# ksahlin/IsoCon

Hardware: AMD Instinct MI355X
Metric: read x candidate alignments/sec (NN-graph build, 50k x 2.5kb reads) (higher is better)
Workload: dtype u64; 1 GPU; C3: 50000 synthetic CCS reads (50000 unique), ~2500 bp, 10 isoforms, seed 30001; 1-set NN graph; edges=78526, graph_digest=65944c838d76a6c9, parallelism=single GPU

## Files before the change

isocon_amd/csrc/isocon_hip.hip:

```cpp
#include <algorithm>
#include <chrono>
#include <cstdio>
#include <cstdlib>
#include <cstring>
#include <numeric>
#include <string>
#include <memory>
#include <mutex>
#include <thread>
#include <vector>

#include "common.hpp"
#include "ed_band.hpp"
#include "ed_full.hpp"
#include "qgram_mm.hpp"
#include "nn.hpp"
#include "nn_list.hpp"
#include "nn_filter.hpp"
#include "nn_finalize.hpp"
#include "nn_finalize_host.hpp"
#include "partition_host.hpp"
#include "sg.hpp"
#include "msa.hpp"
#include "hw.hpp"
#include "hw_tiles.hpp"
#include "hw_full.hpp"
#include "nw_path.hpp"
#include "ed_lanes.hpp"
#include "ed_bytes.hpp"
#include "nn2_depth.hpp"
#include "readtab.hpp"
#include "edgevar.hpp"

namespace isocon {
thread_local std::string g_last_error;
}

using namespace isocon;

static bool variant_lookup(const char *name, std::string *value)
{
    const char *e = getenv("ISOCON_DEBUG_VARIANT");
    if (!e) return false;
    const size_t ln = strlen(name);
    for (const char *p = e; *p;) {
        const char *q = strchr(p, ',');
        const size_t len = q ? (size_t)(q - p) : strlen(p);
        if (len >= ln && strncmp(p, name, ln) == 0 && (len == ln || p[ln] == '=')) {
            if (value) *value = len > ln ? std::string(p + ln + 1, len - ln - 1) : std::string();
            return true;
        }
        p += len + (q ? 1 : 0);
    }
    return false;
}
static bool variant(const char *name) { return variant_lookup(name, nullptr); }
static const char *variant_value(const char *name)
{
    thread_local std::string ring[8];
    thread_local unsigned at = 0;
    std::string &slot = ring[at++ % 8];
    return variant_lookup(name, &slot) ? slot.c_str() : nullptr;
}

struct BoundTag {
    bool valid = false, has_order = false;
    uint64_t serial = 0;
    QMap map = {0, 0, 0, 0};
    uint32_t depth = 0;
    int32_t kcap = 0;
    unsigned long long lb_total = 0;
};
struct MsaBuilt {
    enum By { NONE, SINGLE, BATCH } by = NONE;
    uint64_t serial = 0;
    uint32_t n_parts = 0, n_rows = 0;
    std::vector<uint32_t> ncols, col_base, first_row;
    std::vector<unsigned long long> m_off;
};
struct HeldHits { uint64_t store_serial = 0; uint64_t rows = 0; };

struct ScratchPool {
    struct Slot { void *p = nullptr; size_t cap = 0; };
    Slot slots[160];
    BoundTag bound_tag;
    HeldHits held_hits;
    MsaBuilt msa;
    void *get(int idx, size_t bytes)
    {
        Slot &s = slots[idx];
        if (bytes == 0) bytes = 16;
        if (s.cap < bytes) {
            if (s.p) (void)hipFree(s.p);
            s.p = nullptr; s.cap = 0;
            const size_t want = bytes + bytes / 8;
            if (hipMalloc(&s.p, want) == hipSuccess) s.cap = want;
            else if (hipMalloc(&s.p, bytes) == hipSuccess) s.cap = bytes;
            else { s.p = nullptr; (void)hipGetLastError(); }
        }
        return s.p;
    }
    void release()
    {
        for (Slot &s : slots) { if (s.p) (void)hipFree(s.p); s.p = nullptr; s.cap = 0; }
        bound_tag = BoundTag();
        held_hits = HeldHits();
        msa = MsaBuilt();
    }
};

enum {
    SLOT_ED_TS = 0, SLOT_ED_IDS, SLOT_ED_K, SLOT_ED_OUT, SLOT_FULL_A, SLOT_FULL_B, SLOT_FULL_K, SLOT_FULL_OUT,
    SLOT_NN_BEST, SLOT_NN_QF, SLOT_NN_TF, SLOT_NN_HITS, SLOT_NN_HITCOUNT, SLOT_NN_STATS, SLOT_NN_TS, SLOT_NN_IDS, SLOT_NN_PLANES2, SLOT_NN_PERM, SLOT_NN_IL, SLOT_NN_IL2, SLOT_NN_HITS2, SLOT_NN_HITCOUNT2, SLOT_NN_QPROF, SLOT_NN_QSUM, SLOT_NN_LB, SLOT_NN_LBROW, SLOT_NN_LBLEN, SLOT_NN_SLOTORDER, SLOT_NN_LBCHUNKS, SLOT_NN_ROWMIN, SLOT_NN_COLMIN, SLOT_NN_SEED_A, SLOT_NN_SEED_B, SLOT_NN_SEED_N, SLOT_NN_LBT, SLOT_NN_LBT_OFF, SLOT_NN_LBT_SLO, SLOT_NN_LBT_LEN, SLOT_NN_LBT_PAD, SLOT_NN_SCORE, SLOT_NN_LDEST, SLOT_NN_FIN_HITS, SLOT_NN_FIN_CNT, SLOT_NN_FIN_START, SLOT_NN_FIN_CUR, SLOT_NN_FIN_NB, SLOT_NN_FIN_LEN2, SLOT_NN_FIN_OUT, SLOT_NN_FIN_FLAG, SLOT_NN_FIN_BEST, SLOT_NN_ACC_HITS, SLOT_NN_LTOT, SLOT_NN_LCHUNKS, SLOT_NN_LIST, SLOT_NN_LPA, SLOT_NN_LPB, SLOT_NN_TEXT2, SLOT_NN_LTASKS, SLOT_NN_RECORD,
    SLOT_NN2_STATE, SLOT_NN2_TPOS, SLOT_NN2_EXC, SLOT_NN2_CTR, SLOT_NN2_PAIRS, SLOT_NN2_WIDE,
    SLOT_SG_PAIRS, SLOT_SG_R, SLOT_SG_TRACE, SLOT_SG_END, SLOT_SG_OPS, SLOT_SG_CNT, SLOT_SG_RES, SLOT_SG_OFF, SLOT_SG_DENSE, SLOT_SG_BOUND, SLOT_SG_AOFF, SLOT_SG_ALNA, SLOT_SG_ALNB,
    SLOT_MSA_IN, SLOT_MSA_OUT, SLOT_MSA_DEG, SLOT_MSA_COUNTS, SLOT_MSA_MAJ, SLOT_MSA_FLAGS, SLOT_MSA_TOT, SLOT_MSA_NCAND, SLOT_MSA_LEN, SLOT_MSA_OFF, SLOT_MSA_PACKED, SLOT_MSA_ROWS, SLOT_MSA_OPS, SLOT_MSA_OPTR, SLOT_MSA_LONGEST, SLOT_MSA_WIDTH, SLOT_MSA_CSLOT, SLOT_MSA_LTOT, SLOT_MSA_WIDE, SLOT_MSA_PROW, SLOT_MSA_PCOL, SLOT_MSA_PPTR, SLOT_MSA_PBYTES, SLOT_MSA_PART, SLOT_MSA_FIRST, SLOT_MSA_LM, SLOT_MSA_SBASE, SLOT_MSA_NCOLS, SLOT_MSA_MOFF, SLOT_MSA_CBASE, SLOT_MSA_CBP, SLOT_MSA_CBC, SLOT_MSA_CBR,
    SLOT_HW_Q, SLOT_HW_T, SLOT_HW_K, SLOT_HW_OUT, SLOT_HW_TRACE, SLOT_HW_CTR, SLOT_HW_TILEQ, SLOT_HW_LANES, SLOT_HW_PQ, SLOT_HW_KEY, SLOT_HW_HIST, SLOT_HW_CURSOR, SLOT_HW_TBASE, SLOT_HW_CLS,
    SLOT_PACK_ASCII, SLOT_PACK_OFF, SLOT_PACK_BAD, SLOT_PACK_HIST, SLOT_PACK_FLAGS, SLOT_EB_A, SLOT_EB_B, SLOT_EB_K, SLOT_EB_OUT, SLOT_EB_ROWS, SLOT_SCAN_TMP, SLOT_SCAN_SUMS,
    SLOT_RT_REF, SLOT_RT_IN, SLOT_RT_OUT,
    SLOT_EV_IN, SLOT_EV_OUT, SLOT_EV_SNIP,
    SLOT_NWP_Q, SLOT_NWP_T, SLOT_NWP_ED, SLOT_NWP_TOFF, SLOT_NWP_ROFF, SLOT_NWP_REV, SLOT_NWP_RUNS, SLOT_NWP_FOFF, SLOT_NWP_OPS, SLOT_NWP_START, SLOT_NWP_COLS,
    SLOT_COUNT
};
static_assert(SLOT_COUNT <= 160, "ScratchPool::slots too small");

static ScratchPool g_scratch;

static uint64_t g_store_serial = 0;

struct isocon_store {
    uint64_t serial = ++g_store_serial;
    DevStore dev;
    explicit isocon_store(bool private_scratch = false) : own_pool(private_scratch ? new ScratchPool() : nullptr), pool(own_pool ? *own_pool : g_scratch) {}
    std::unique_ptr<ScratchPool> own_pool;
    ScratchPool &pool;
    std::vector<int32_t> lens;
    uint64_t device_bytes = 0;
    uint64_t *d_planes = nullptr;
    char alphabet[4] = {'A', 'C', 'G', 'T'};
    bool acgt = true;
    uint8_t *d_bytes = nullptr;
    uint64_t *d_boff = nullptr;
    uint64_t bytes_base = 0;
    std::vector<uint8_t> exc;
    std::vector<uint32_t> exc_count;
    uint32_t n_exc = 0;
    bool is_exc(uint32_t i) const { return n_exc != 0 && exc[i] != 0; }
    int32_t *d_lens = nullptr;
    int32_t maxlen = 0;
    uint64_t last_host_waits = 0;
};

namespace {

struct PinnedStage {
    void *p = nullptr;
    size_t cap = 0;
    void *get(size_t bytes)
    {
        if (cap < bytes) {
            if (p) (void)hipHostFree(p);
            p = nullptr; cap = 0;
            if (hipHostMalloc(&p, bytes, hipHostMallocDefault) == hipSuccess) cap = bytes;
            else { p = nullptr; (void)hipGetLastError(); }
        }
        return p;
    }
    void release() { if (p) (void)hipHostFree(p); p = nullptr; cap = 0; }
};
static PinnedStage g_stage;
static constexpr size_t kStageBytes = (size_t)32 << 20;
static constexpr uint64_t kPackWaves = (uint64_t)1 << 25;
static constexpr size_t kStageMin = (size_t)32 << 10;

static std::vector<std::pair<const char *, size_t>> g_pinned;
static bool is_pinned(const void *p, size_t bytes)
{
    for (const auto &r : g_pinned)
        if ((const char *)p >= r.first && (const char *)p + bytes <= r.first + r.second) return true;
    return false;
}

static thread_local uint64_t g_host_waits = 0;
static hipError_t memcpy_wait(void *dst, const void *src, size_t bytes, hipMemcpyKind kind) { ++g_host_waits; return hipMemcpy(dst, src, bytes, kind); }
static hipError_t memset_wait(void *dst, int value, size_t bytes) { ++g_host_waits; return hipMemset(dst, value, bytes); }
static hipError_t device_wait() { ++g_host_waits; return hipDeviceSynchronize(); }

static hipError_t copy_d2h(void *dst, const void *dsrc, size_t bytes)
{
    if (bytes < kStageMin || is_pinned(dst, bytes)) return memcpy_wait(dst, dsrc, bytes, hipMemcpyDeviceToHost);
    char *st = static_cast<char *>(g_stage.get(kStageBytes));
    if (!st) return memcpy_wait(dst, dsrc, bytes, hipMemcpyDeviceToHost);
    for (size_t off = 0; off < bytes; off += kStageBytes) {
        const size_t len = std::min(kStageBytes, bytes - off);
        const hipError_t e = memcpy_wait(st, static_cast<const char *>(dsrc) + off, len, hipMemcpyDeviceToHost);
        if (e != hipSuccess) return e;
        memcpy(static_cast<char *>(dst) + off, st, len);
    }
    return hipSuccess;
}

static hipError_t copy_h2d(void *ddst, const void *src, size_t bytes)
{
    if (bytes < kStageMin || is_pinned(src, bytes)) return memcpy_wait(ddst, src, bytes, hipMemcpyHostToDevice);
    char *st = static_cast<char *>(g_stage.get(kStageBytes));
    if (!st) return memcpy_wait(ddst, src, bytes, hipMemcpyHostToDevice);
    for (size_t off = 0; off < bytes; off += kStageBytes) {
        const size_t len = std::min(kStageBytes, bytes - off);
        memcpy(st, static_cast<const char *>(src) + off, len);
        const hipError_t e = memcpy_wait(static_cast<char *>(ddst) + off, st, len, hipMemcpyHostToDevice);
        if (e != hipSuccess) return e;
    }
    return hipSuccess;
}

struct SideUpload {
    hipStream_t stream = nullptr;
    hipEvent_t before = nullptr, done = nullptr;
    PinnedStage pinned;
    bool in_flight = false;
    bool ready()
    {
        if (stream) return true;
        if (hipStreamCreateWithFlags(&stream, hipStreamNonBlocking) != hipSuccess) { stream = nullptr; (void)hipGetLastError(); return false; }
        if (hipEventCreateWithFlags(&before, hipEventDisableTiming) != hipSuccess || hipEventCreateWithFlags(&done, hipEventDisableTiming) != hipSuccess) {
            (void)hipGetLastError();
            release();
            return false;
        }
        return true;
    }
    void settle()
    {
        if (!in_flight) return;
        if (hipEventQuery(done) != hipSuccess || hipStreamQuery(stream) != hipSuccess) { (void)hipGetLastError(); ++g_host_waits; (void)hipStreamSynchronize(stream); }
        in_flight = false;
    }
    void release()
    {
        if (stream) { (void)hipStreamSynchronize(stream); (void)hipStreamDestroy(stream); }
        if (before) (void)hipEventDestroy(before);
        if (done) (void)hipEventDestroy(done);
        stream = nullptr; before = done = nullptr; in_flight = false;
        pinned.release();
    }
};
static SideUpload g_side;

struct DevBuf {
    void *p = nullptr;
    ScratchPool *pool = nullptr;
    int slot = -1;
    DevBuf() {}
    DevBuf(ScratchPool *pl, int sl) : pool(pl), slot(sl) {}
    DevBuf(const DevBuf &) = delete;
    DevBuf &operator=(const DevBuf &) = delete;
    ~DevBuf() { if (p && !pool) (void)hipFree(p); }
    template <class T> T *as() { return static_cast<T *>(p); }
    int alloc(size_t bytes)
    {
        if (pool) {
            p = pool->get(slot, bytes);
            if (!p) { g_last_error = "hipMalloc(scratch slot " + std::to_string(slot) + ", " + std::to_string(bytes) + " B) failed"; return ISOCON_E_HIP; }
            return ISOCON_OK;
        }
        if (p) { (void)hipFree(p); p = nullptr; }
        ISO_HIP_CHECK(hipMalloc(&p, bytes ? bytes : 16));
        return ISOCON_OK;
    }
};

template <int SHIFT, class OUT>
static int device_exscan(ScratchPool *pl, const uint32_t *d_in, uint32_t n, OUT *d_out)
{
    DevBuf d_tmp(pl, SLOT_SCAN_TMP), d_sums(pl, SLOT_SCAN_SUMS);
    const uint32_t tiles = std::max<uint32_t>(1, (n + SCAN_TILE - 1) / SCAN_TILE);
    int rc;
    if ((rc = d_tmp.alloc((size_t)std::max<uint32_t>(n, 1) * 4)) || (rc = d_sums.alloc((size_t)tiles * 8))) return rc;
    hipLaunchKernelGGL((k_scan_tiles<SHIFT>), dim3(tiles), dim3(256), 0, 0, d_in, n, d_tmp.as<uint32_t>(), d_sums.as<unsigned long long>());
    hipLaunchKernelGGL((k_scan_finish<OUT>), dim3(tiles), dim3(256), 0, 0, d_tmp.as<uint32_t>(), n, d_sums.as<unsigned long long>(), tiles, d_out, (unsigned long long *)nullptr);
    ISO_HIP_CHECK(hipGetLastError());
    return ISOCON_OK;
}

struct EventPool {
    std::mutex mu;
    std::vector<hipEvent_t> idle;
    hipEvent_t get()
    {
        {
            std::lock_guard<std::mutex> g(mu);
            if (!idle.empty()) { hipEvent_t e = idle.back(); idle.pop_back(); return e; }
        }
        hipEvent_t e = nullptr;
        if (hipEventCreate(&e) != hipSuccess) { (void)hipGetLastError(); return nullptr; }
        return e;
    }
    void put(hipEvent_t e)
    {
        if (!e) return;
        std::lock_guard<std::mutex> g(mu);
        idle.push_back(e);
    }
    void release()
    {
        std::lock_guard<std::mutex> g(mu);
        for (hipEvent_t e : idle) (void)hipEventDestroy(e);
        idle.clear();
    }
};
static EventPool g_events;

struct EventTimer {
    struct Interval { hipEvent_t e0, em, e1; float *acc, *marked_acc; };
    std::vector<Interval> pending;
    hipEvent_t e0 = nullptr, em = nullptr;
    float total = 0.f;
    float marked_total = 0.f;
    const bool sync_phases = variant("nn_sync_phases");
    EventTimer() {}
    EventTimer(const EventTimer &) = delete;
    EventTimer &operator=(const EventTimer &) = delete;
    ~EventTimer()
    {
        g_events.put(e0); g_events.put(em);
        for (const Interval &iv : pending) { g_events.put(iv.e0); g_events.put(iv.em); g_events.put(iv.e1); }
    }
    void start()
    {
        g_events.put(em); em = nullptr;
        if (!e0) e0 = g_events.get();
        if (e0) (void)hipEventRecord(e0, 0);
    }
    void mark()
    {
        if (!e0) return;
        if (!em) em = g_events.get();
        if (em) (void)hipEventRecord(em, 0);
    }
    void stop_later(float *acc, float *marked_acc = nullptr)
    {
        if (!e0) return;
        hipEvent_t e1 = g_events.get();
        if (!e1) { g_events.put(e0); g_events.put(em); e0 = em = nullptr; return; }
        (void)hipEventRecord(e1, 0);
        pending.push_back(Interval{e0, em, e1, acc, marked_acc});
        e0 = em = nullptr;
        if (sync_phases) resolve(true);
    }
    void resolve(bool wait_counts = false)
    {
        if (pending.empty()) return;
        hipEvent_t last = pending.back().e1;
        if (wait_counts || hipEventQuery(last) != hipSuccess) { (void)hipGetLastError(); ++g_host_waits; (void)hipEventSynchronize(last); }
        for (const Interval &iv : pending) {
            float ms = 0.f, part = 0.f;
            if (hipEventElapsedTime(&ms, iv.e0, iv.e1) != hipSuccess) { (void)hipGetLastError(); ms = 0.f; }
            total += ms;
            if (iv.acc) *iv.acc += ms;
            if (iv.em) {
                if (hipEventElapsedTime(&part, iv.em, iv.e1) != hipSuccess) { (void)hipGetLastError(); part = 0.f; }
                if (iv.marked_acc) *iv.marked_acc += part; else marked_total += part;
            }
            g_events.put(iv.e0); g_events.put(iv.em); g_events.put(iv.e1);
        }
        pending.clear();
    }
    float stop()
    {
        float ms = 0.f;
        stop_later(&ms);
        resolve(true);
        return ms;
    }
};

struct PackMap { uint8_t sym[4]; };

__global__ __launch_bounds__(256) void k_byte_histogram(const uint8_t *__restrict__ ascii, uint64_t total, unsigned long long *__restrict__ hist)
{
    __shared__ uint32_t h[256];
    h[threadIdx.x] = 0;
    __syncthreads();
    for (uint64_t i = (uint64_t)blockIdx.x * 256 + threadIdx.x; i < total; i += (uint64_t)gridDim.x * 256) atomicAdd(&h[ascii[i]], 1u);
    __syncthreads();
    if (h[threadIdx.x]) atomicAdd(hist + threadIdx.x, (unsigned long long)h[threadIdx.x]);
}

__global__ __launch_bounds__(256) void k_pack_planes(const uint8_t *__restrict__ ascii, const uint64_t *__restrict__ offsets, uint64_t base, uint32_t n,
                                                      uint32_t nchunks, uint64_t *__restrict__ planes, unsigned long long *__restrict__ first_bad, PackMap map,
                                                      uint32_t fold, uint64_t w0)
{
    const uint64_t w = w0 + (uint64_t)blockIdx.x * 4 + (threadIdx.x >> 6);
    if (w >= (uint64_t)nchunks * n) return;
    const uint32_t lane = threadIdx.x & 63;
    const uint32_t chunk = (uint32_t)(w / n), seq = (uint32_t)(w % n);
    const uint64_t off = offsets[seq] - base, len = offsets[seq + 1] - offsets[seq];
    const uint64_t pos = (uint64_t)chunk * 64 + lane;
    int cd = 0;
    bool bad = false;
    if (pos < len) {
        uint8_t ch = ascii[off + pos];
        if (fold && ch >= 'a' && ch <= 'z') ch = (uint8_t)(ch - 32);
        cd = ch == map.sym[0] ? 0 : ch == map.sym[1] ? 1 : ch == map.sym[2] ? 2 : ch == map.sym[3] ? 3 : -1;
        bad = cd < 0 && !fold;
    }
    const unsigned long long lo = __ballot(!bad && (cd & 1)), hi = __ballot(!bad && (cd & 2)), bm = __ballot(bad);
    if (lane == 0) {
        planes[((size_t)chunk * n + seq) * 2] = lo;
        planes[((size_t)chunk * n + seq) * 2 + 1] = hi;
        if (bm) atomicMin(first_bad, ((unsigned long long)seq << 32) | ((unsigned long long)chunk * 64 + (unsigned long long)(__ffsll((long long)bm) - 1)));
    }
}

}

extern "C" {

const char *isocon_strerror(int status)
{
    switch (status) {
    case ISOCON_OK: return "ok";
    case ISOCON_E_ARG: return "bad argument";
    case ISOCON_E_ALPHABET: return "sequence contains a symbol outside ACGT";
    case ISOCON_E_HIP: return "HIP runtime error";
    case ISOCON_E_CAPACITY: return "output buffer too small";
    case ISOCON_E_NODEVICE: return "no usable GPU";
    case ISOCON_E_UNSUPPORTED: return "unsupported request";
    default: return "unknown status";
    }
}

const char *isocon_last_error(void) { return g_last_error.c_str(); }

int isocon_device_count(void)
{
    int n = 0;
    if (hipGetDeviceCount(&n) != hipSuccess) return 0;
    return n;
}

void isocon_release_scratch(void) { g_scratch.release(); g_stage.release(); g_events.release(); g_side.release(); }

int isocon_init(int device_ordinal)
{
    int n = 0;
    if (hipGetDeviceCount(&n) != hipSuccess || n <= 0) { g_last_error = "hipGetDeviceCount: no device"; return ISOCON_E_NODEVICE; }
    if (device_ordinal < 0 || device_ordinal >= n) return ISOCON_E_ARG;
    ISO_HIP_CHECK(hipSetDevice(device_ordinal));
    return ISOCON_OK;
}

static int store_create_impl(const uint8_t *ascii, const uint8_t *const *seq_ptrs, const uint64_t *offsets, uint32_t n, isocon_store **out, bool private_scratch = false)
{
    *out = nullptr;
    int32_t maxlen = 0;
    for (uint32_t i = 0; i < n; ++i) {
        if (offsets[i + 1] < offsets[i] || offsets[i + 1] - offsets[i] > 0x3fffffff) return ISOCON_E_ARG;
        maxlen = std::max<int32_t>(maxlen, (int32_t)(offsets[i + 1] - offsets[i]));
    }
    const uint32_t nchunks = (uint32_t)((maxlen + 63) / 64 + 1);
    const uint32_t nn = std::max<uint32_t>(n, 1);
    std::vector<int32_t> lens(nn, 0);
    for (uint32_t i = 0; i < n; ++i) lens[i] = (int32_t)(offsets[i + 1] - offsets[i]);
    const uint64_t base = n ? offsets[0] : 0, total = n ? offsets[n] - offsets[0] : 0;
    isocon_store *st = new isocon_store(private_scratch);
    st->lens = lens;
    st->maxlen = maxlen;
    const size_t pbytes = (size_t)nchunks * nn * 2 * sizeof(uint64_t), lbytes = lens.size() * sizeof(int32_t);
    if (hipMalloc((void **)&st->d_planes, pbytes) != hipSuccess || hipMalloc((void **)&st->d_lens, lbytes) != hipSuccess) {
        g_last_error = "hipMalloc(store) failed";
        isocon_store_destroy(st);
        return ISOCON_E_HIP;
    }
    {
        DevBuf d_ascii(&g_scratch, SLOT_PACK_ASCII), d_off(&g_scratch, SLOT_PACK_OFF), d_bad(&g_scratch, SLOT_PACK_BAD);
        uint64_t pack_waves = kPackWaves;
        if (const char *e = variant_value("pack_waves")) pack_waves = std::max<uint64_t>(4, strtoull(e, nullptr, 10)) & ~(uint64_t)3;
        const unsigned long long none = ~0ull;
        int rc = ISOCON_OK;
        if ((rc = d_ascii.alloc(total ? total : 16)) || (rc = d_off.alloc((size_t)(nn + 1) * 8)) || (rc = d_bad.alloc(8))) { isocon_store_destroy(st); return rc; }
        bool up = true;
        if (total && ascii) up = copy_h2d(d_ascii.p, ascii + base, total) == hipSuccess;
        else if (total) {
            char *stg = static_cast<char *>(g_stage.get(kStageBytes));
            hipEvent_t ev[2] = {nullptr, nullptr};
            up = stg != nullptr && hipEventCreateWithFlags(&ev[0], hipEventDisableTiming) == hipSuccess && hipEventCreateWithFlags(&ev[1], hipEventDisableTiming) == hipSuccess;
            const size_t half = kStageBytes / 2;
            uint64_t done = 0;
            bool busy[2] = {false, false};
            auto gather = [&](char *dst, uint64_t b0, uint64_t b1) {
                uint32_t i = (uint32_t)(std::upper_bound(offsets, offsets + n + 1, base + b0) - offsets) - 1;
                uint64_t in_seq = base + b0 - offsets[i];
                while (b0 < b1 && i < n) {
                    const uint64_t len = offsets[i + 1] - offsets[i];
                    const size_t take = (size_t)std::min<uint64_t>(len - in_seq, b1 - b0);
                    if (take) memcpy(dst, seq_ptrs[i] + in_seq, take);
                    dst += take; b0 += take; in_seq += take;
                    if (in_seq == len) { ++i; in_seq = 0; }
                }
            };
            const unsigned hc = std::thread::hardware_concurrency();
            const unsigned n_thr = total >= ((uint64_t)8 << 20) ? std::min(4u, hc ? hc : 1u) : 1u;
            for (int h = 0; up && done < total; h ^= 1) {
                if (busy[h]) up = hipEventSynchronize(ev[h]) == hipSuccess;
                const size_t fill = (size_t)std::min<uint64_t>(half, total - done);
                if (n_thr <= 1) gather(stg + h * half, done, done + fill);
                else {
                    std::thread th[4];
                    const size_t part = (fill + n_thr - 1) / n_thr;
                    for (unsigned t = 0; t < n_thr; ++t) {
                        const size_t a = std::min(fill, t * part), b = std::min(fill, (t + 1) * part);
                        th[t] = std::thread([&, a, b, h] { if (b > a) gather(stg + h * half + a, done + a, done + b); });
                    }
                    for (unsigned t = 0; t < n_thr; ++t) th[t].join();
                }
                up = up && hipMemcpyAsync(static_cast<char *>(d_ascii.p) + done, stg + h * half, fill, hipMemcpyHostToDevice, 0) == hipSuccess &&
                     hipEventRecord(ev[h], 0) == hipSuccess;
                busy[h] = true;
                done += fill;
            }
            up = up && hipStreamSynchronize(0) == hipSuccess;
            if (ev[0]) (void)hipEventDestroy(ev[0]);
            if (ev[1]) (void)hipEventDestroy(ev[1]);
        }
        bool ok = up &&
                  (n == 0 || copy_h2d(d_off.p, offsets, (size_t)(n + 1) * 8) == hipSuccess) &&
                  hipMemcpy(d_bad.p, &none, 8, hipMemcpyHostToDevice) == hipSuccess && copy_h2d(st->d_lens, lens.data(), lbytes) == hipSuccess;
        unsigned long long bad = none;
        if (ok) {
            if (n) {
                const uint64_t waves = (uint64_t)nchunks * n;
                for (uint64_t w0 = 0; w0 < waves; w0 += pack_waves)
                    hipLaunchKernelGGL(k_pack_planes, dim3((unsigned)((std::min<uint64_t>(pack_waves, waves - w0) + 3) / 4)), dim3(256), 0, 0, d_ascii.as<uint8_t>(), d_off.as<uint64_t>(), base, n, nchunks,
                                       st->d_planes, d_bad.as<unsigned long long>(), PackMap{{'A', 'C', 'G', 'T'}}, 0u, w0);
            } else {
                ok = hipMemset(st->d_planes, 0, pbytes) == hipSuccess;
            }
            ok = ok && hipGetLastError() == hipSuccess && hipMemcpy(&bad, d_bad.p, 8, hipMemcpyDeviceToHost) == hipSuccess;
        }
        if (!ok) {
            g_last_error = "isocon_store_create: device copy / packing failed";
            (void)hipGetLastError();
            isocon_store_destroy(st);
            return ISOCON_E_HIP;
        }
        if (bad != none) {
            DevBuf d_hist(&g_scratch, SLOT_PACK_HIST);
            unsigned long long hist[256];
            bool hok = d_hist.alloc(256 * 8) == ISOCON_OK && hipMemset(d_hist.p, 0, 256 * 8) == hipSuccess;
            if (hok) {
                hipLaunchKernelGGL(k_byte_histogram, dim3(1024), dim3(256), 0, 0, d_ascii.as<uint8_t>(), (uint64_t)total, d_hist.as<unsigned long long>());
                hok = hipGetLastError() == hipSuccess && hipMemcpy(hist, d_hist.p, sizeof(hist), hipMemcpyDeviceToHost) == hipSuccess;
            }
            int distinct = 0;
            for (int c = 0; hok && c < 256; ++c) distinct += hist[c] != 0;
            if (!hok) {
                g_last_error = "isocon_store_create: symbol histogram failed";
                (void)hipGetLastError();
                isocon_store_destroy(st);
                return ISOCON_E_HIP;
            }
            if (distinct > 4) {
                DevBuf d_flags(&g_scratch, SLOT_PACK_FLAGS);
                st->exc.assign(nn, 0);
                st->exc_count.assign(nn, 0);
                bool eok = d_flags.alloc((size_t)nn * 4) == ISOCON_OK && hipMemset(d_flags.p, 0, (size_t)nn * 4) == hipSuccess &&
                           hipMalloc((void **)&st->d_bytes, total ? total : 16) == hipSuccess && hipMalloc((void **)&st->d_boff, (size_t)(nn + 1) * 8) == hipSuccess;
                if (eok) {
                    const uint64_t waves = (uint64_t)nchunks * n;
                    for (uint64_t w0 = 0; w0 < waves; w0 += pack_waves)
                    hipLaunchKernelGGL(k_pack_planes, dim3((unsigned)((std::min<uint64_t>(pack_waves, waves - w0) + 3) / 4)), dim3(256), 0, 0, d_ascii.as<uint8_t>(), d_off.as<uint64_t>(), base, n, nchunks,
                                       st->d_planes, d_bad.as<unsigned long long>(), PackMap{{'A', 'C', 'G', 'T'}}, 1u, w0);
                    for (uint64_t w0 = 0; w0 < waves; w0 += pack_waves)
                        hipLaunchKernelGGL(k_exception_flags, dim3((unsigned)((std::min<uint64_t>(pack_waves, waves - w0) + 3) / 4)), dim3(256), 0, 0, d_ascii.as<uint8_t>(), d_off.as<uint64_t>(), base, n,
                                           nchunks, d_flags.as<uint32_t>(), (uint32_t)'A' | ((uint32_t)'C' << 8) | ((uint32_t)'G' << 16) | ((uint32_t)'T' << 24), w0);
                    eok = hipGetLastError() == hipSuccess && hipMemcpy(st->exc_count.data(), d_flags.p, (size_t)n * 4, hipMemcpyDeviceToHost) == hipSuccess &&
                          hipMemcpy(st->d_bytes, d_ascii.p, total, hipMemcpyDeviceToDevice) == hipSuccess &&
                          hipMemcpy(st->d_boff, d_off.p, (size_t)(n + 1) * 8, hipMemcpyDeviceToDevice) == hipSuccess;
                }
                if (!eok) {
                    g_last_error = "isocon_store_create: keeping the bytes of a set with more than four symbols failed";
                    (void)hipGetLastError();
                    isocon_store_destroy(st);
                    return ISOCON_E_HIP;
                }
                st->bytes_base = base;
                for (uint32_t i = 0; i < n; ++i) { st->exc[i] = st->exc_count[i] != 0; st->n_exc += st->exc[i]; }
                st->acgt = false;
                st->device_bytes += total + (size_t)(nn + 1) * 8;
            } else {
            PackMap map{{0, 0, 0, 0}};
            bool used[4] = {false, false, false, false};
            const char acgt_sym[4] = {'A', 'C', 'G', 'T'};
            for (int k = 0; k < 4; ++k) if (hist[(uint8_t)acgt_sym[k]]) { map.sym[k] = (uint8_t)acgt_sym[k]; used[k] = true; }
            for (int c = 0; c < 256; ++c) {
                if (!hist[c] || c == 'A' || c == 'C' || c == 'G' || c == 'T') continue;
                for (int k = 0; k < 4; ++k) if (!used[k]) { map.sym[k] = (uint8_t)c; used[k] = true; break; }
            }
            for (int k = 0; k < 4; ++k) if (!used[k]) { for (int c = 1; c < 256; ++c) if (!hist[c] && c != map.sym[0] && c != map.sym[1] && c != map.sym[2] && c != map.sym[3]) { map.sym[k] = (uint8_t)c; break; } }
            bool rok = hipMemcpy(d_bad.p, &none, 8, hipMemcpyHostToDevice) == hipSuccess;
            if (rok) {
                const uint64_t waves = (uint64_t)nchunks * n;
                for (uint64_t w0 = 0; w0 < waves; w0 += pack_waves)
                    hipLaunchKernelGGL(k_pack_planes, dim3((unsigned)((std::min<uint64_t>(pack_waves, waves - w0) + 3) / 4)), dim3(256), 0, 0, d_ascii.as<uint8_t>(), d_off.as<uint64_t>(), base, n, nchunks,
                                       st->d_planes, d_bad.as<unsigned long long>(), map, 0u, w0);
                rok = hipGetLastError() == hipSuccess && hipMemcpy(&bad, d_bad.p, 8, hipMemcpyDeviceToHost) == hipSuccess && bad == none;
            }
            if (!rok) {
                g_last_error = "isocon_store_create: packing under the set's own alphabet failed";
                (void)hipGetLastError();
                isocon_store_destroy(st);
                return ISOCON_E_HIP;
            }
            for (int k = 0; k < 4; ++k) st->alphabet[k] = (char)map.sym[k];
            st->acgt = false;
            }
        }
    }
    st->device_bytes += pbytes + lbytes;
    st->dev.planes = st->d_planes;
    st->dev.il = nullptr;
    st->dev.lens = st->d_lens;
    st->dev.n = n;
    st->dev.nchunks = nchunks;
    st->lens.resize(n);
    *out = st;
    return ISOCON_OK;
}

int isocon_store_create(const uint8_t *ascii, const uint64_t *offsets, uint32_t n, isocon_store **out)
{
    if (!out || (!ascii && n) || !offsets) return ISOCON_E_ARG;
    return store_create_impl(ascii, nullptr, offsets, n, out);
}

int isocon_store_create_ptrs(const uint8_t *const *seq_ptrs, const uint64_t *seq_lens, uint32_t n, isocon_store **out)
{
    if (!out || (n && (!seq_ptrs || !seq_lens))) return ISOCON_E_ARG;
    std::vector<uint64_t> offsets((size_t)n + 1, 0);
    for (uint32_t i = 0; i < n; ++i) {
        if (seq_lens[i] && !seq_ptrs[i]) return ISOCON_E_ARG;
        offsets[i + 1] = offsets[i] + seq_lens[i];
    }
    return store_create_impl(nullptr, seq_ptrs, offsets.data(), n, out);
}

int isocon_store_create_ptrs_ex(const uint8_t *const *seq_ptrs, const uint64_t *seq_lens, uint32_t n, uint32_t flags, isocon_store **out)
{
    if (!out || (n && (!seq_ptrs || !seq_lens)) || (flags & ~(uint32_t)ISOCON_STORE_PRIVATE_SCRATCH)) return ISOCON_E_ARG;
    std::vector<uint64_t> offsets((size_t)n + 1, 0);
    for (uint32_t i = 0; i < n; ++i) {
        if (seq_lens[i] && !seq_ptrs[i]) return ISOCON_E_ARG;
        offsets[i + 1] = offsets[i] + seq_lens[i];
    }
    return store_create_impl(nullptr, seq_ptrs, offsets.data(), n, out, (flags & ISOCON_STORE_PRIVATE_SCRATCH) != 0);
}

void *isocon_host_alloc(uint64_t bytes)
{
    void *p = nullptr;
    if (hipHostMalloc(&p, bytes ? bytes : 16, hipHostMallocDefault) != hipSuccess) { (void)hipGetLastError(); return nullptr; }
    g_pinned.emplace_back((const char *)p, (size_t)(bytes ? bytes : 16));
    return p;
}

void isocon_host_free(void *p)
{
    if (!p) return;
    for (size_t i = 0; i < g_pinned.size(); ++i)
        if (g_pinned[i].first == (const char *)p) { g_pinned.erase(g_pinned.begin() + (long)i); break; }
    (void)hipHostFree(p);
}

void isocon_store_destroy(isocon_store *s)
{
    if (!s) return;
    if (s->d_planes) (void)hipFree(s->d_planes);
    if (s->d_lens) (void)hipFree(s->d_lens);
    if (s->d_bytes) (void)hipFree(s->d_bytes);
    if (s->d_boff) (void)hipFree(s->d_boff);
    if (s->own_pool) s->own_pool->release();
    delete s;
}

uint32_t isocon_store_size(const isocon_store *s) { return s ? s->dev.n : 0; }
uint64_t isocon_nn_last_host_waits(const isocon_store *s) { return s ? s->last_host_waits : 0; }
uint64_t isocon_store_device_bytes(const isocon_store *s) { return s ? s->device_bytes : 0; }

}

namespace {

template <int W>
int launch_band_tiles(isocon_store *st, const DevStore &S, const std::vector<uint32_t> &tile_shared, const std::vector<uint32_t> &lane_ids,
                      const std::vector<int32_t> &lane_k, std::vector<int32_t> &out, EventTimer &tm)
{
    const size_t nt = tile_shared.size();
    out.assign(nt * 64, -1);
    if (!nt) return ISOCON_OK;
    DevBuf d_ts(&st->pool, SLOT_ED_TS), d_ids(&st->pool, SLOT_ED_IDS), d_k(&st->pool, SLOT_ED_K), d_out(&st->pool, SLOT_ED_OUT);
    int rc;
    if ((rc = d_ts.alloc(nt * 4)) || (rc = d_ids.alloc(nt * 64 * 4)) || (rc = d_k.alloc(nt * 64 * 4)) || (rc = d_out.alloc(nt * 64 * 4))) return rc;
    ISO_HIP_CHECK(copy_h2d(d_ts.p, tile_shared.data(), nt * 4));
    ISO_HIP_CHECK(copy_h2d(d_ids.p, lane_ids.data(), nt * 64 * 4));
    ISO_HIP_CHECK(copy_h2d(d_k.p, lane_k.data(), nt * 64 * 4));
    tm.start();
    hipLaunchKernelGGL(k_ed_band_tiles<W>, dim3((unsigned)((nt + 3) / 4)), dim3(256), 0, 0, S, d_ts.as<uint32_t>(),
                       d_ids.as<uint32_t>(), d_k.as<int32_t>(), d_out.as<int32_t>(), (uint32_t)nt);
    ISO_HIP_CHECK(hipGetLastError());
    tm.stop();
    ISO_HIP_CHECK(copy_d2h(out.data(), d_out.p, nt * 64 * 4));
    return ISOCON_OK;
}

int run_band_stage(int W, isocon_store *st, const DevStore &S, const std::vector<uint32_t> &ts, const std::vector<uint32_t> &ids,
                   const std::vector<int32_t> &ks, std::vector<int32_t> &out, EventTimer &tm)
{
    switch (W) {
    case 1: return launch_band_tiles<1>(st, S, ts, ids, ks, out, tm);
    case 2: return launch_band_tiles<2>(st, S, ts, ids, ks, out, tm);
    case 4: return launch_band_tiles<4>(st, S, ts, ids, ks, out, tm);
    case 8: return launch_band_tiles<8>(st, S, ts, ids, ks, out, tm);
    default: return ISOCON_E_ARG;
    }
}

int run_full(isocon_store *st, const std::vector<uint32_t> &a, const std::vector<uint32_t> &b,
             const std::vector<int32_t> &k, std::vector<int32_t> &out, EventTimer &tm)
{
    const size_t np = a.size();
    out.assign(np, -1);
    if (!np) return ISOCON_OK;
    DevBuf d_a(&st->pool, SLOT_FULL_A), d_b(&st->pool, SLOT_FULL_B), d_k(&st->pool, SLOT_FULL_K), d_out(&st->pool, SLOT_FULL_OUT);
    int rc;
    if ((rc = d_a.alloc(np * 4)) || (rc = d_b.alloc(np * 4)) || (rc = d_k.alloc(np * 4)) || (rc = d_out.alloc(np * 4))) return rc;
    ISO_HIP_CHECK(copy_h2d(d_a.p, a.data(), np * 4));
    ISO_HIP_CHECK(copy_h2d(d_b.p, b.data(), np * 4));
    ISO_HIP_CHECK(copy_h2d(d_k.p, k.data(), np * 4));
    bool multipass = false;
    int32_t maxtext = 0;
    for (size_t p = 0; p < np; ++p) {
        const int32_t la = st->lens[a[p]], lb = st->lens[b[p]];
        if (std::min(la, lb) > 4096) multipass = true;
        maxtext = std::max(maxtext, std::max(la, lb));
    }
    const size_t lds = multipass ? (size_t)((maxtext + 15) & ~15) : 0;
    if (lds > 160 * 1024) { g_last_error = "sequence longer than 163840 bases in the un-banded kernel"; return ISOCON_E_UNSUPPORTED; }
    if (lds > 64 * 1024)
        ISO_HIP_CHECK(hipFuncSetAttribute((const void *)k_ed_full, hipFuncAttributeMaxDynamicSharedMemorySize, (int)lds));
    tm.start();
    hipLaunchKernelGGL(k_ed_full, dim3((unsigned)np), dim3(64), lds, 0, st->dev, d_a.as<uint32_t>(), d_b.as<uint32_t>(),
                       d_k.as<int32_t>(), d_out.as<int32_t>(), (uint32_t)np);
    ISO_HIP_CHECK(hipGetLastError());
    tm.stop();
    ISO_HIP_CHECK(copy_d2h(out.data(), d_out.p, np * 4));
    return ISOCON_OK;
}

int run_bytes(isocon_store *st, const std::vector<uint32_t> &a, const std::vector<uint32_t> &b, const std::vector<int32_t> &k, std::vector<int32_t> &out, EventTimer &tm)
{
    const size_t np = a.size();
    out.assign(np, -1);
    if (!np) return ISOCON_OK;
    if (!st->d_bytes) { g_last_error = "internal: byte-wise distances on a store that kept no bytes"; return ISOCON_E_HIP; }
    if (st->maxlen >= (int32_t)EB_INF - 1) { g_last_error = "byte-wise distances: sequences of 8 388 606 bases and more are not supported"; return ISOCON_E_UNSUPPORTED; }
    const uint32_t row_stride = (uint32_t)st->maxlen + 130u;
    size_t waves = std::min<size_t>(np, 8192);
    while (waves > 256 && waves * row_stride * 4 > ((size_t)2 << 30)) waves /= 2;
    DevBuf d_a(&st->pool, SLOT_EB_A), d_b(&st->pool, SLOT_EB_B), d_k(&st->pool, SLOT_EB_K), d_out(&st->pool, SLOT_EB_OUT), d_rows(&st->pool, SLOT_EB_ROWS);
    int rc;
    if ((rc = d_a.alloc(np * 4)) || (rc = d_b.alloc(np * 4)) || (rc = d_k.alloc(np * 4)) || (rc = d_out.alloc(np * 4)) || (rc = d_rows.alloc(waves * row_stride * 4))) return rc;
    ISO_HIP_CHECK(copy_h2d(d_a.p, a.data(), np * 4));
    ISO_HIP_CHECK(copy_h2d(d_b.p, b.data(), np * 4));
    ISO_HIP_CHECK(copy_h2d(d_k.p, k.data(), np * 4));
    tm.start();
    hipLaunchKernelGGL(k_ed_bytes, dim3((unsigned)waves), dim3(64), 0, 0, ByteStore{st->d_bytes, st->d_boff, st->bytes_base, st->d_lens}, d_a.as<uint32_t>(), d_b.as<uint32_t>(),
                       d_k.as<int32_t>(), (unsigned long long)np, d_rows.as<uint32_t>(), row_stride, d_out.as<int32_t>());
    ISO_HIP_CHECK(hipGetLastError());
    tm.stop();
    ISO_HIP_CHECK(copy_d2h(out.data(), d_out.p, np * 4));
    return ISOCON_OK;
}

}

namespace isocon {

int ed_pairs_impl(isocon_store *st, const uint32_t *a, const uint32_t *b, const int32_t *k, uint64_t n_pairs,
                  int32_t *out_ed, float *kernel_ms, uint64_t *full_pairs, bool images)
{
    EventTimer tm;
    const uint32_t n = st->dev.n;
    for (uint64_t p = 0; p < n_pairs; ++p)
        if (a[p] >= n || b[p] >= n) return ISOCON_E_ARG;
    bool swap_roles = false;
    {
        std::vector<uint8_t> seen_a(n, 0), seen_b(n, 0);
        size_t da = 0, db = 0;
        for (uint64_t p = 0; p < n_pairs; ++p) {
            if (!seen_a[a[p]]) { seen_a[a[p]] = 1; ++da; }
            if (!seen_b[b[p]]) { seen_b[b[p]] = 1; ++db; }
        }
        swap_roles = db < da;
    }
    std::vector<uint64_t> pending;
    pending.reserve(n_pairs);
    if (st->n_exc && !images) {
        std::vector<uint64_t> xp;
        for (uint64_t p = 0; p < n_pairs; ++p) (st->exc[a[p]] || st->exc[b[p]] ? xp : pending).push_back(p);
        if (!xp.empty()) {
            std::vector<uint32_t> xa(xp.size()), xb(xp.size());
            std::vector<int32_t> xk(xp.size()), res;
            for (size_t i = 0; i < xp.size(); ++i) { xa[i] = a[xp[i]]; xb[i] = b[xp[i]]; xk[i] = k ? k[xp[i]] : -1; }
            int rc = run_bytes(st, xa, xb, xk, res, tm);
            if (rc) return rc;
            for (size_t i = 0; i < xp.size(); ++i) out_ed[xp[i]] = res[i];
        }
    } else {
        pending.resize(n_pairs);
        std::iota(pending.begin(), pending.end(), 0);
    }
    static const int stages[4] = {1, 2, 4, 8};
    for (int si = 0; si < 4 && !pending.empty(); ++si) {
        const int W = stages[si];
        const int32_t kcap = 64 * W - 1;
        auto sh = [&](uint64_t p) { return swap_roles ? b[p] : a[p]; };
        auto ln = [&](uint64_t p) { return swap_roles ? a[p] : b[p]; };
        std::sort(pending.begin(), pending.end(), [&](uint64_t x, uint64_t y) {
            if (sh(x) != sh(y)) return sh(x) < sh(y);
            const int32_t lx = st->lens[ln(x)], ly = st->lens[ln(y)];
            if (lx != ly) return lx < ly;
            return x < y;
        });
        std::vector<uint64_t> todo = pending, next;
        if (W == 1) {
            const char *e = variant_value("ed_lanes");
            const size_t min_group = e ? (atoi(e) ? (size_t)-1 : 0) : 16;
            std::vector<uint64_t> lanes_p, tiles_p;
            for (size_t i = 0; i < todo.size();) {
                size_t j = i;
                while (j < todo.size() && sh(todo[j]) == sh(todo[i])) ++j;
                std::vector<uint64_t> &dst = (j - i) < min_group ? lanes_p : tiles_p;
                dst.insert(dst.end(), todo.begin() + i, todo.begin() + j);
                i = j;
            }
            if (!lanes_p.empty()) {
                const size_t np = lanes_p.size();
                std::vector<uint32_t> la(np), lb2(np);
                std::vector<int32_t> lk(np), res(np, -1);
                for (size_t i = 0; i < np; ++i) {
                    const uint64_t p = lanes_p[i];
                    la[i] = a[p]; lb2[i] = b[p];
                    const int32_t kr = k ? k[p] : -1;
                    lk[i] = kr < 0 ? kcap : std::min(kr, kcap);
                }
                DevBuf d_a(&st->pool, SLOT_ED_TS), d_b(&st->pool, SLOT_ED_IDS), d_k(&st->pool, SLOT_ED_K), d_out(&st->pool, SLOT_ED_OUT);
                int rc;
                if ((rc = d_a.alloc(np * 4)) || (rc = d_b.alloc(np * 4)) || (rc = d_k.alloc(np * 4)) || (rc = d_out.alloc(np * 4))) return rc;
                ISO_HIP_CHECK(copy_h2d(d_a.p, la.data(), np * 4));
                ISO_HIP_CHECK(copy_h2d(d_b.p, lb2.data(), np * 4));
                ISO_HIP_CHECK(copy_h2d(d_k.p, lk.data(), np * 4));
                NNParams none;
                memset(&none, 0, sizeof(none));
                tm.start();
                hipLaunchKernelGGL(k_ed_lanes<false>, dim3((unsigned)((np + 255) / 256)), dim3(256), 0, 0, st->dev, none, d_a.as<uint32_t>(), d_b.as<uint32_t>(),
                                   d_k.as<int32_t>(), (uint64_t)np, d_out.as<int32_t>());
                ISO_HIP_CHECK(hipGetLastError());
                tm.stop();
                ISO_HIP_CHECK(copy_d2h(res.data(), d_out.p, np * 4));
                for (size_t i = 0; i < np; ++i) {
                    const uint64_t p = lanes_p[i];
                    const int32_t kr = k ? k[p] : -1;
                    if (res[i] >= 0) out_ed[p] = res[i];
                    else if (kr >= 0 && kr <= kcap) out_ed[p] = -1;
                    else next.push_back(p);
                }
            }
            todo.swap(tiles_p);
        }
        for (int round = 0; round < 2 && !todo.empty(); ++round) {
            std::vector<uint32_t> ts, ids;
            std::vector<int32_t> ks;
            std::vector<uint64_t> slot_pair;
            size_t i = 0;
            while (i < todo.size()) {
                size_t j = i;
                const uint32_t s0 = sh(todo[i]);
                const size_t lim = round == 0 ? 64 : 1;
                while (j < todo.size() && j - i < lim && sh(todo[j]) == s0) ++j;
                ts.push_back(s0);
                for (size_t l = 0; l < 64; ++l) {
                    if (i + l < j) {
                        const uint64_t p = todo[i + l];
                        ids.push_back(ln(p));
                        const int32_t kr = k ? k[p] : -1;
                        ks.push_back(kr < 0 ? kcap : std::min(kr, kcap));
                        slot_pair.push_back(p);
                    } else {
                        ids.push_back(0xffffffffu);
                        ks.push_back(-1);
                        slot_pair.push_back(~(uint64_t)0);
                    }
                }
                i = j;
            }
            std::vector<int32_t> res;
            int rc = run_band_stage(W, st, st->dev, ts, ids, ks, res, tm);
            if (rc) return rc;
            std::vector<uint64_t> retry;
            for (size_t sidx = 0; sidx < slot_pair.size(); ++sidx) {
                const uint64_t p = slot_pair[sidx];
                if (p == ~(uint64_t)0) continue;
                const int32_t r = res[sidx];
                const int32_t kr = k ? k[p] : -1;
                if (r >= 0) out_ed[p] = r;
                else if (r == -2) retry.push_back(p);
                else if (kr >= 0 && kr <= kcap) out_ed[p] = -1;
                else next.push_back(p);
            }
            todo.swap(retry);
        }
        if (!todo.empty()) { g_last_error = "internal: single-lane tile undetermined"; return ISOCON_E_HIP; }
        pending.swap(next);
    }
    if (full_pairs) *full_pairs = pending.size();
    if (!pending.empty()) {
        std::vector<uint32_t> fa, fb;
        std::vector<int32_t> fk, res;
        for (uint64_t p : pending) { fa.push_back(a[p]); fb.push_back(b[p]); fk.push_back(k ? k[p] : -1); }
        int rc = run_full(st, fa, fb, fk, res, tm);
        if (rc) return rc;
        for (size_t i = 0; i < pending.size(); ++i) out_ed[pending[i]] = res[i];
    }
    if (kernel_ms) *kernel_ms = tm.total;
    return ISOCON_OK;
}

}

__global__ __launch_bounds__(256) void k_store_digest(const uint64_t *__restrict__ planes, size_t n_words, const int32_t *__restrict__ lens, uint32_t n,
                                                      unsigned long long *__restrict__ out)
{
    unsigned long long acc = 0;
    const size_t stride = (size_t)gridDim.x * blockDim.x;
    for (size_t i = (size_t)blockIdx.x * blockDim.x + threadIdx.x; i < n_words + n; i += stride) {
        unsigned long long v = i < n_words ? planes[i] : (unsigned long long)(uint32_t)lens[i - n_words];
        v ^= (unsigned long long)i * 0xD6E8FEB86659FD93ull;
        v ^= v >> 32; v *= 0x9E3779B97F4A7C15ull; v ^= v >> 29; v *= 0xBF58476D1CE4E5B9ull; v ^= v >> 32;
        acc += v;
    }
    for (int o = 32; o > 0; o >>= 1) acc += __shfl_xor(acc, o, 64);
    if ((threadIdx.x & 63) == 0 && acc) atomicAdd(out, acc);
}

extern "C" int isocon_store_digest(const isocon_store *s, uint64_t *out)
{
    if (!s || !out) return ISOCON_E_ARG;
    DevBuf d_acc;
    int rc;
    if ((rc = d_acc.alloc(8))) return rc;
    ISO_HIP_CHECK(hipMemset(d_acc.p, 0, 8));
    const size_t n_words = (size_t)s->dev.nchunks * std::max<uint32_t>(s->dev.n, 1) * 2;
    hipLaunchKernelGGL(k_store_digest, dim3(1024), dim3(256), 0, 0, s->d_planes, n_words, s->d_lens, s->dev.n, d_acc.as<unsigned long long>());
    ISO_HIP_CHECK(hipGetLastError());
    ISO_HIP_CHECK(hipMemcpy(out, d_acc.p, 8, hipMemcpyDeviceToHost));
    return ISOCON_OK;
}

extern "C" int isocon_ed_pairs(isocon_store *s, const uint32_t *a, const uint32_t *b, const int32_t *k, uint64_t n_pairs,
                               int32_t *out_ed, float *kernel_ms)
{
    if (!s || (n_pairs && (!a || !b || !out_ed))) return ISOCON_E_ARG;
    if (kernel_ms) *kernel_ms = 0.f;
    if (!n_pairs) return ISOCON_OK;
    return ed_pairs_impl(s, a, b, k, n_pairs, out_ed, kernel_ms, nullptr, false);
}

extern "C" int isocon_qgram_params(int32_t *out)
{
    if (out) { out[0] = QG_Q; out[1] = QG_B0; out[2] = QG_B1; out[3] = QG_CAP; }
    return QM_K;
}

namespace isocon {
int qgram_bounds_for_pairs(isocon_store *s, const uint32_t *a, const uint32_t *b, uint64_t n_pairs, int32_t *out_bound, float *kernel_ms)
{
    const uint32_t n = s->dev.n;
    const uint32_t n_pad = std::max<uint32_t>(QM_TILE, ((n + QM_TILE - 1) / QM_TILE) * QM_TILE);
    DevBuf d_prof(&s->pool, SLOT_NN_QPROF), d_sum(&s->pool, SLOT_NN_QSUM), d_a(&s->pool, SLOT_ED_TS), d_b(&s->pool, SLOT_ED_IDS), d_out(&s->pool, SLOT_ED_OUT);
    int rc;
    if ((rc = d_prof.alloc((size_t)n_pad * (QM_K / 2))) || (rc = d_sum.alloc((size_t)n * 4)) || (rc = d_a.alloc(n_pairs * 4)) || (rc = d_b.alloc(n_pairs * 4)) ||
        (rc = d_out.alloc(n_pairs * 4)))
        return rc;
    s->pool.bound_tag.valid = false;
    ISO_HIP_CHECK(copy_h2d(d_a.p, a, n_pairs * 4));
    ISO_HIP_CHECK(copy_h2d(d_b.p, b, n_pairs * 4));
    EventTimer tm;
    tm.start();
    hipLaunchKernelGGL(k_qgram_profile4, dim3((n + QP_SEQS - 1) / QP_SEQS), dim3(256), 0, 0, s->dev, d_prof.as<uint8_t>(), d_sum.as<uint32_t>(), n_pad);
    ISO_HIP_CHECK(hipGetLastError());
    for (uint64_t at = 0; at < n_pairs; at += (uint64_t)1 << 24) {
        const uint64_t cnt = std::min<uint64_t>((uint64_t)1 << 24, n_pairs - at);
        hipLaunchKernelGGL(k_qgram_lb_pairs, dim3((unsigned)((cnt + 3) / 4)), dim3(256), 0, 0, d_prof.as<uint8_t>(), d_sum.as<uint32_t>(), n_pad, d_a.as<uint32_t>() + at,
                           d_b.as<uint32_t>() + at, cnt, d_out.as<int32_t>() + at);
        ISO_HIP_CHECK(hipGetLastError());
    }
    const float ms = tm.stop();
    if (kernel_ms) *kernel_ms = ms;
    ISO_HIP_CHECK(copy_d2h(out_bound, d_out.p, n_pairs * 4));
    return ISOCON_OK;
}
}

extern "C" int isocon_qgram_bound_pairs(isocon_store *s, const uint32_t *a, const uint32_t *b, uint64_t n_pairs, int32_t *out_bound)
{
    if (!s || (n_pairs && (!a || !b || !out_bound))) return ISOCON_E_ARG;
    if (!n_pairs) return ISOCON_OK;
    if (s->n_exc) { g_last_error = "q-gram bounds are defined on the 2-bit planes: the set holds more than four distinct symbols"; return ISOCON_E_ALPHABET; }
    const uint32_t n = s->dev.n;
    for (uint64_t i = 0; i < n_pairs; ++i)
        if (a[i] >= n || b[i] >= n) { g_last_error = "pair index out of range"; return ISOCON_E_ARG; }
    return qgram_bounds_for_pairs(s, a, b, n_pairs, out_bound, nullptr);
}

extern "C" int isocon_block_bound_pairs(isocon_store *s, const uint32_t *owner, const uint32_t *partner, uint64_t n_pairs, int32_t probe_stride, int32_t *out_count)
{
    if (probe_stride != 4 && probe_stride != 2) return ISOCON_E_ARG;
    if (!s || (n_pairs && (!owner || !partner || !out_count))) return ISOCON_E_ARG;
    if (!n_pairs) return ISOCON_OK;
    if (s->n_exc) { g_last_error = "block bounds are defined on the 2-bit planes: the set holds more than four distinct symbols"; return ISOCON_E_ALPHABET; }
    const uint32_t n = s->dev.n;
    if (n_pairs >= ((uint64_t)1 << 31)) return ISOCON_E_ARG;
    for (uint64_t i = 0; i < n_pairs; ++i)
        if (owner[i] >= n || partner[i] >= n) { g_last_error = "pair index out of range"; return ISOCON_E_ARG; }
    const uint32_t stride = nnf_text2_stride(s->maxlen);
    DevBuf d_text(&s->pool, SLOT_NN_TEXT2), d_a(&s->pool, SLOT_ED_TS), d_b(&s->pool, SLOT_ED_IDS), d_out(&s->pool, SLOT_ED_OUT);
    int rc;
    if ((rc = d_text.alloc((size_t)n * stride * 4)) || (rc = d_a.alloc(n_pairs * 4)) || (rc = d_b.alloc(n_pairs * 4)) || (rc = d_out.alloc(n_pairs * 4))) return rc;
    ISO_HIP_CHECK(copy_h2d(d_a.p, owner, n_pairs * 4));
    ISO_HIP_CHECK(copy_h2d(d_b.p, partner, n_pairs * 4));
    hipLaunchKernelGGL(k_build_text2, dim3(n), dim3(256), 0, 0, s->dev, d_text.as<uint32_t>(), stride);
    hipLaunchKernelGGL(k_nn_block_count_pairs, dim3((unsigned)n_pairs), dim3(256), 0, 0, d_text.as<uint32_t>(), stride, s->dev.lens, d_a.as<uint32_t>(), d_b.as<uint32_t>(), d_out.as<int32_t>(), probe_stride);
    ISO_HIP_CHECK(hipGetLastError());
    ISO_HIP_CHECK(copy_d2h(out_count, d_out.p, n_pairs * 4));
    return ISOCON_OK;
}

#include "nn_context.inc"
#include "nn_bounds.inc"
#include "nn_lists.inc"
#include "nn_main.inc"
#include "nn_wide.inc"
#include "nn_images.inc"
#include "nn_entry.inc"
#include "nn2_depth.inc"
#include "sg_host.inc"
#include "msa_host.inc"
#include "hw_host.inc"
#include "hw_full_host.inc"
#include "nw_path_host.inc"
#include "hw_path_host.inc"
#include "readtab_host.inc"
#include "edgevar_host.inc"

extern "C" int isocon_partition_ids(uint32_t n, const int32_t *degree, uint64_t n_edges, const uint32_t *edge_a, const uint32_t *edge_b,
                                    const uint32_t *rank, int32_t nbr_tiebreak, uint32_t *out_centre, int64_t *out_weight,
                                    uint64_t *out_member_ptr, uint32_t *out_members, uint32_t *n_parts)
{
    if (!out_member_ptr || !n_parts || (n && (!degree || !rank || !out_centre || !out_weight || !out_members)) || (n_edges && (!edge_a || !edge_b))) return ISOCON_E_ARG;
    return partition_ids_impl(n, degree, n_edges, edge_a, edge_b, rank, nbr_tiebreak, out_centre, out_weight, out_member_ptr, out_members, n_parts);
}
```

isocon_amd/csrc/nn_bounds.inc:

```

namespace {

int NNContext::build_bounds(const QMap &Q, int32_t kcap, NNParams &P, bool want_seeds)
{
    const uint32_t q_begin = Q.begin, q_end = Q.end;
    P.lb = nullptr;
    P.lb_row = nullptr;
    P.slot_order = nullptr;
    if (variant("nn_no_qgram") || n < 2 || n >= (1u << 30) || q_begin >= q_end) return ISOCON_OK;
    if (!want_seeds && st->pool.bound_tag.valid && st->pool.bound_tag.serial == st->serial && st->pool.bound_tag.map.same(Q) &&
        st->pool.bound_tag.depth == depth && st->pool.bound_tag.kcap == kcap) {
        P.lb = static_cast<const uint8_t *>(st->pool.slots[SLOT_NN_LB].p);
        P.lb_row = static_cast<const unsigned long long *>(st->pool.slots[SLOT_NN_LBROW].p);
        if (st->pool.bound_tag.has_order && use_slot_order(Q.count())) P.slot_order = static_cast<const uint32_t *>(st->pool.slots[SLOT_NN_SLOTORDER].p);
        lb_total = st->pool.bound_tag.lb_total;
        return ISOCON_OK;
    }
    st->pool.bound_tag.valid = false;
    const uint32_t nq = Q.count();
    const std::vector<int32_t> &lens = st->lens;
    const uint32_t n_pad = std::max<uint32_t>(QM_TILE, ((n + QM_TILE - 1) / QM_TILE) * QM_TILE);
    const size_t prof_bytes = (size_t)n_pad * (QM_K / 2);
    d_qprof.pool = d_qsum.pool = &st->pool;
    d_qprof.slot = SLOT_NN_QPROF; d_qsum.slot = SLOT_NN_QSUM;
    HostClock bclk;
    {
        size_t free_b = 0;
        if (!free_mem(free_b) || prof_bytes > free_b / 2 + st->pool.slots[SLOT_NN_QPROF].cap) return ISOCON_OK;
        if (d_qprof.alloc(prof_bytes) || d_qsum.alloc((size_t)n * 4)) return ISOCON_OK;
    }
    bclk.lap("bounds: memory check + profile buffers");
    const bool side = !variant("nn_sync_uploads") && g_side.ready() && hipEventRecord(g_side.before, 0) == hipSuccess;
    tm.start();
    hipLaunchKernelGGL(k_qgram_profile4, dim3((n + QP_SEQS - 1) / QP_SEQS), dim3(256), 0, 0, st->dev, d_qprof.as<uint8_t>(), d_qsum.as<uint32_t>(), n_pad);
    ISO_HIP_CHECK(hipGetLastError());
    struct StopTimer { NNContext &c; bool armed = true; ~StopTimer() { if (armed) c.tm.stop_later(&c.stats.bound_kernel_ms); } } stop_timer{*this};
    std::vector<unsigned long long> &off = lb_off_host;
    std::vector<uint32_t> &rlen = lb_len_host;
    off.assign(nq, 0);
    rlen.assign(nq, 0);
    unsigned long long total = 0, sum_rlen = 0;
    uint64_t hi = 0;
    const uint32_t nrb = (nq + QM_TILE - 1) / QM_TILE;
    std::vector<uint64_t> rb_lo(nrb, ~(uint64_t)0), rb_hi(nrb, 0);
    for (uint32_t s = 0; s < nq; ++s) {
        const uint64_t q = Q.entry(s);
        if (hi < q + 1) hi = q + 1;
        while (hi < n && lens[hi] - lens[q] <= kcap) ++hi;
        uint64_t len = hi - q - 1;
        if (len > depth) len = depth;
        const uint64_t pal = (q + 1) & ~(uint64_t)15;
        off[s] = total + (q + 1 - pal);
        rlen[s] = (uint32_t)len;
        sum_rlen += len;
        if (len) {
            total += ((q + 1 + len + 15) & ~(uint64_t)15) - pal;
            rb_lo[s / QM_TILE] = std::min<uint64_t>(rb_lo[s / QM_TILE], q + 1);
            rb_hi[s / QM_TILE] = std::max<uint64_t>(rb_hi[s / QM_TILE], q + len);
        }
    }
    if (total == 0) return ISOCON_OK;
    bclk.lap("bounds: profile launch + rows (host)");
    const unsigned long long totalT = sum_rlen + 30ull * n;
    bclk.lap("bounds: transposed rows (host)");
    size_t free_b = 0;
    const size_t need = (size_t)total + (size_t)totalT + prof_bytes + (size_t)n * 24 + (size_t)nq * 12;
    if (!free_mem(free_b) || need > free_b / 2 + st->pool.slots[SLOT_NN_LB].cap + st->pool.slots[SLOT_NN_QPROF].cap) return ISOCON_OK;
    bclk.lap("bounds: memory check 2");
    std::vector<uint2> tiles;
    for (uint32_t g = 0; g * 4 < nrb; ++g) {
        uint64_t jmin = ~(uint64_t)0, jmax = 0;
        bool any = false;
        for (uint32_t I = g * 4; I < std::min(nrb, g * 4 + 4); ++I)
            if (rb_lo[I] != ~(uint64_t)0) { any = true; jmin = std::min(jmin, rb_lo[I] / QM_TILE); jmax = std::max(jmax, rb_hi[I] / QM_TILE); }
        if (!any) continue;
        for (uint64_t j0 = jmin; j0 <= jmax; j0 += 8)
            for (uint32_t ri = 0; ri < 4; ++ri)
                for (uint32_t cj = 0; cj < 8; ++cj) {
                    const uint32_t I = g * 4 + ri;
                    const uint64_t J = j0 + cj;
                    const bool have = I < nrb && rb_lo[I] != ~(uint64_t)0 && J >= rb_lo[I] / QM_TILE && J <= rb_hi[I] / QM_TILE;
                    tiles.push_back(have ? make_uint2(I, (uint32_t)J) : make_uint2(0xffffffffu, 0xffffffffu));
                }
    }
    while (tiles.size() % 256) tiles.push_back(make_uint2(0xffffffffu, 0xffffffffu));
    if (tiles.size() > 0x7fffffffull) return ISOCON_OK;
    bclk.lap("bounds: tile table (host)");
    d_lb.pool = d_lbrow.pool = d_lblen.pool = &st->pool;
    d_lb.slot = SLOT_NN_LB; d_lbrow.slot = SLOT_NN_LBROW; d_lblen.slot = SLOT_NN_LBLEN;
    int rc;
    if ((rc = d_lb.alloc((size_t)total + 16)) ||
        (rc = d_lbrow.alloc((size_t)nq * 8)) || (rc = d_lblen.alloc((size_t)nq * 4)))
        return ISOCON_OK;
    d_lbt.pool = d_offT.pool = d_sloT.pool = d_lenT.pool = d_score.pool = &st->pool;
    d_lbt.slot = SLOT_NN_LBT; d_offT.slot = SLOT_NN_LBT_OFF; d_sloT.slot = SLOT_NN_LBT_SLO; d_lenT.slot = SLOT_NN_LBT_LEN; d_score.slot = SLOT_NN_SCORE;
    DevBuf d_padT(&st->pool, SLOT_NN_LBT_PAD);
    if (d_lbt.alloc((size_t)totalT + 16) || d_offT.alloc(((size_t)n + 1) * 8) || d_sloT.alloc((size_t)n * 4) || d_lenT.alloc((size_t)n * 4) || d_score.alloc((size_t)n * 4) ||
        d_padT.alloc((size_t)n * 4))
        return ISOCON_OK;
    ISO_HIP_CHECK(hipMemsetAsync(d_score.p, 0, (size_t)n * 4, 0));
    d_chunks.pool = &st->pool;
    d_chunks.slot = SLOT_NN_LBCHUNKS;
    if (d_chunks.alloc(tiles.size() * sizeof(uint2))) return ISOCON_OK;
    const size_t b_tiles = (tiles.size() * sizeof(uint2) + 15) & ~(size_t)15, b_off = ((size_t)nq * 8 + 15) & ~(size_t)15, b_len = (size_t)nq * 4;
    char *pin = nullptr;
    if (side) { g_side.settle(); pin = static_cast<char *>(g_side.pinned.get(b_tiles + b_off + b_len)); }
    if (pin) {
        memcpy(pin, tiles.data(), tiles.size() * sizeof(uint2));
        memcpy(pin + b_tiles, off.data(), (size_t)nq * 8);
        memcpy(pin + b_tiles + b_off, rlen.data(), (size_t)nq * 4);
        g_side.in_flight = true;
        ISO_HIP_CHECK(hipStreamWaitEvent(g_side.stream, g_side.before, 0));
        ISO_HIP_CHECK(hipMemcpyAsync(d_chunks.p, pin, tiles.size() * sizeof(uint2), hipMemcpyHostToDevice, g_side.stream));
        ISO_HIP_CHECK(hipMemcpyAsync(d_lbrow.p, pin + b_tiles, (size_t)nq * 8, hipMemcpyHostToDevice, g_side.stream));
        ISO_HIP_CHECK(hipMemcpyAsync(d_lblen.p, pin + b_tiles + b_off, (size_t)nq * 4, hipMemcpyHostToDevice, g_side.stream));
        ISO_HIP_CHECK(hipEventRecord(g_side.done, g_side.stream));
        ISO_HIP_CHECK(hipStreamWaitEvent(0, g_side.done, 0));
    } else {
        ISO_HIP_CHECK(copy_h2d(d_chunks.p, tiles.data(), tiles.size() * sizeof(uint2)));
        ISO_HIP_CHECK(copy_h2d(d_lbrow.p, off.data(), (size_t)nq * 8));
        ISO_HIP_CHECK(copy_h2d(d_lblen.p, rlen.data(), (size_t)nq * 4));
    }
    hipLaunchKernelGGL(k_lbt_rows, dim3((n + 255) / 256), dim3(256), 0, 0, Q, nq, d_lblen.as<uint32_t>(), n, d_sloT.as<uint32_t>(), d_lenT.as<uint32_t>(), d_padT.as<uint32_t>());
    if ((rc = device_exscan<0, unsigned long long>(&st->pool, d_padT.as<uint32_t>(), n, d_offT.as<unsigned long long>()))) return ISOCON_OK;
    hipLaunchKernelGGL(k_lbt_offsets, dim3((n + 255) / 256), dim3(256), 0, 0, n, d_sloT.as<uint32_t>(), d_offT.as<unsigned long long>());
    ISO_HIP_CHECK(hipGetLastError());
    bclk.lap("bounds: alloc + uploads");
    if (use_slot_order(nq)) {
        std::vector<uint32_t> order(nq);
        std::iota(order.begin(), order.end(), 0u);
        std::stable_sort(order.begin(), order.end(), [&](uint32_t x, uint32_t y) { return rlen[x] > rlen[y]; });
        d_order.pool = &st->pool;
        d_order.slot = SLOT_NN_SLOTORDER;
        if (d_order.alloc((size_t)nq * 4)) return ISOCON_OK;
        ISO_HIP_CHECK(copy_h2d(d_order.p, order.data(), (size_t)nq * 4));
    }
    unsigned long long *rowmin = nullptr, *colmin = nullptr;
    if (want_seeds) {
        d_rowmin.pool = d_colmin.pool = d_seed_a.pool = d_seed_b.pool = &st->pool;
        d_rowmin.slot = SLOT_NN_ROWMIN; d_colmin.slot = SLOT_NN_COLMIN; d_seed_a.slot = SLOT_NN_SEED_A; d_seed_b.slot = SLOT_NN_SEED_B;
        if (!(d_rowmin.alloc((size_t)nq * 8 * QM_SEEDS) || d_colmin.alloc((size_t)n_pad * 8 * QM_SEEDS) || d_seed_a.alloc((size_t)n * 8 * QM_SEEDS) || d_seed_b.alloc((size_t)n * 8 * QM_SEEDS))) {
            ISO_HIP_CHECK(hipMemsetAsync(d_rowmin.p, 0xff, (size_t)nq * 8 * QM_SEEDS, 0));
            ISO_HIP_CHECK(hipMemsetAsync(d_colmin.p, 0xff, (size_t)n_pad * 8 * QM_SEEDS, 0));
            rowmin = d_rowmin.as<unsigned long long>();
            colmin = d_colmin.as<unsigned long long>();
        }
    }
    bclk.lap("bounds: slot order + seed buffers");
    static bool lds_attr_set = false;
    if (!lds_attr_set) {
        ISO_HIP_CHECK(hipFuncSetAttribute((const void *)k_qgram_mm, hipFuncAttributeMaxDynamicSharedMemorySize, (int)QM_LDS_BYTES));
        lds_attr_set = true;
    }
    tm.mark();
    hipLaunchKernelGGL(k_qgram_mm, dim3((unsigned)tiles.size()), dim3(512), QM_LDS_BYTES, 0, d_qprof.as<uint8_t>(), d_qsum.as<uint32_t>(), n, n_pad,
                       d_chunks.as<uint2>(), d_lbrow.as<unsigned long long>(), d_lblen.as<uint32_t>(), d_lb.as<uint8_t>(), Q, nq,
                       d_qf.as<uint8_t>(), d_tf.as<uint8_t>(), rowmin, colmin, d_offT.as<unsigned long long>(), d_sloT.as<uint32_t>(), d_lenT.as<uint32_t>(),
                       d_lbt.as<uint8_t>(), d_score.as<uint32_t>());
    ISO_HIP_CHECK(hipGetLastError());
    stop_timer.armed = false;
    tm.stop_later(&stats.bound_kernel_ms, &stats.mm_kernel_ms);
    bclk.lap("bounds: k_qgram_mm (enqueued)");
#ifdef ISOCON_QM_TIMELINE
    {
        const size_t nt = std::min<size_t>(tiles.size(), 16384);
        std::vector<unsigned long long> tl(nt * 8);
        ISO_HIP_CHECK(hipMemcpyFromSymbol(tl.data(), HIP_SYMBOL(g_qm_timeline), nt * 64));
        double sum[5] = {0, 0, 0, 0, 0};
        unsigned long long t_min = ~0ull, t_max = 0;
        size_t cnt = 0;
        for (size_t b = 0; b < nt; ++b) {
            if (tiles[b].x == 0xffffffffu) continue;
            const unsigned long long *t = tl.data() + b * 8;
            for (int k = 0; k < 5; ++k) sum[k] += (double)(t[k + 1] - t[k]);
            t_min = std::min(t_min, t[0]); t_max = std::max(t_max, t[5]);
            ++cnt;
        }
        fprintf(stderr, "[qm timeline] %zu tiles: prologue %.2f us, K loop %.2f us, E1 %.2f us, E2 %.2f us, E3 %.2f us per tile; first start to last end %.3f ms\n", cnt,
                sum[0] / cnt / 100.0, sum[1] / cnt / 100.0, sum[2] / cnt / 100.0, sum[3] / cnt / 100.0, sum[4] / cnt / 100.0, (double)(t_max - t_min) / 1e5);
    }
#endif
    for (const uint2 &t : tiles) stats.bound_tiles += t.x != 0xffffffffu;
    P.lb = d_lb.as<uint8_t>();
    P.lb_row = d_lbrow.as<unsigned long long>();
    if (use_slot_order(nq)) P.slot_order = d_order.as<uint32_t>();
    seeds_ready = rowmin != nullptr;
    seed_nq = nq;
    lb_total = total;
    st->pool.bound_tag.valid = true;
    st->pool.bound_tag.lb_total = total;
    st->pool.bound_tag.has_order = use_slot_order(nq);
    st->pool.bound_tag.serial = st->serial;
    st->pool.bound_tag.map = Q; st->pool.bound_tag.depth = depth; st->pool.bound_tag.kcap = kcap;
    return ISOCON_OK;
}

int NNContext::run_bound_seeds(const QMap &Q)
{
    if (!seeds_ready) return ISOCON_OK;
    tm.start();
    const uint64_t np = (uint64_t)2 * QM_SEEDS * n;
    const uint32_t ranks = std::max<uint32_t>(1u, Q.stride >> Q.block_log2);
    uint32_t col_classes = QM_SEEDS;
    while (col_classes > 1 && col_classes * ranks > (uint32_t)QM_SEEDS) col_classes >>= 1;
    if (const char *e = variant_value("nn_seed_classes")) { const int v = atoi(e); if (v == 1 || v == 2 || v == QM_SEEDS) col_classes = (uint32_t)v; }
    DevBuf d_seed_n(&st->pool, SLOT_NN_SEED_N);
    int rc;
    if ((rc = d_seed_n.alloc(8))) return rc;
    ISO_HIP_CHECK(hipMemsetAsync(d_seed_n.p, 0, 8, 0));
    ISO_HIP_CHECK(hipMemsetAsync(d_seed_a.p, 0xff, (size_t)np * 4, 0));
    ISO_HIP_CHECK(hipMemsetAsync(d_seed_b.p, 0xff, (size_t)np * 4, 0));
    hipLaunchKernelGGL(k_qgram_seed_pairs, dim3((n + 255) / 256), dim3(256), 0, 0, d_rowmin.as<unsigned long long>(), d_colmin.as<unsigned long long>(),
                       n, Q, seed_nq, col_classes, d_seed_a.as<uint32_t>(), d_seed_b.as<uint32_t>(), d_seed_n.as<unsigned long long>());
    ISO_HIP_CHECK(hipGetLastError());
    hipLaunchKernelGGL(k_ed_lanes<true>, dim3((unsigned)((np + 255) / 256)), dim3(256), 0, 0, st->dev, params(63), d_seed_a.as<uint32_t>(), d_seed_b.as<uint32_t>(),
                       (const int32_t *)nullptr, np, (int32_t *)nullptr);
    ISO_HIP_CHECK(hipGetLastError());
    tm.stop_later(&stats.seed_kernel_ms);
    return ISOCON_OK;
}

}
```

isocon_amd/csrc/nn_context.inc:

```

namespace {

struct HostClock {
    std::chrono::steady_clock::time_point t0 = std::chrono::steady_clock::now();
    const bool on = getenv("ISOCON_DEBUG") != nullptr;
    void lap(const char *what)
    {
        if (!on) return;
        const auto t1 = std::chrono::steady_clock::now();
        fprintf(stderr, "[isocon] %-28s %8.2f ms\n", what, std::chrono::duration<double, std::milli>(t1 - t0).count());
        t0 = t1;
    }
};

struct NNContext {
    isocon_store *st = nullptr;
    uint32_t n = 0;
    std::vector<uint8_t> qflag, tflag;
    bool two_set = false;
    bool depth_binds = false;
    std::vector<uint8_t> wide_mask;
    int32_t min_d = 1;
    uint32_t depth = 0x7fffffffu;
    DevBuf d_best, d_qf, d_tf, d_hits, d_hit_count, d_stats;
    DevBuf d_text;
    uint32_t text_stride = 0;
    bool text_ready = false;
    DevBuf d_qprof, d_qsum, d_lb, d_lbrow, d_lblen;
    DevBuf d_chunks;
    DevBuf d_lbt, d_offT, d_sloT, d_lenT, d_score;
    DevBuf d_order;
    DevBuf d_rowmin, d_colmin, d_seed_a, d_seed_b;
    uint64_t hits_cap = 0;
    std::vector<int32_t> best;
    std::vector<int32_t> hits;
    isocon_nn_stats stats;
    EventTimer tm;

    size_t free_bytes = 0;
    int free_state = 0;
    bool free_mem(size_t &free_b)
    {
        if (free_state == 0) {
            size_t total_b = 0;
            free_state = hipMemGetInfo(&free_bytes, &total_b) == hipSuccess ? 1 : -1;
            if (free_state < 0) (void)hipGetLastError();
        }
        free_b = free_bytes;
        return free_state > 0;
    }
    bool text_room = false;
    bool text_affordable()
    {
        if (text_ready || text_room) return true;
        text_stride = (uint32_t)NN_TEXT_PAD_FRONT + (uint32_t)((st->maxlen + 7) / 8) + (uint32_t)NN_TEXT_PAD_BACK;
        size_t free_b = 0;
        if (!free_mem(free_b) || (size_t)n * text_stride * 4 > free_b / 2) return false;
        d_text.pool = &st->pool;
        d_text.slot = SLOT_NN_IL;
        if (d_text.alloc((size_t)std::max<uint32_t>(n, 1) * text_stride * 4) != ISOCON_OK) return false;
        text_room = true;
        return true;
    }
    bool build_text()
    {
        if (text_ready) return true;
        if (!text_room) return false;
        hipLaunchKernelGGL(k_build_nibble_text, dim3(std::max<uint32_t>(n, 1)), dim3(256), 0, 0, st->dev, d_text.as<uint32_t>(), text_stride);
        if (hipGetLastError() != hipSuccess) { g_last_error = "k_build_nibble_text: launch failed"; return false; }
        text_ready = true;
        return true;
    }
    bool ensure_text() { return text_affordable() && build_text(); }
    DevBuf d_text2;
    uint32_t text2_stride = 0;
    bool text2_ready = false;
    bool ensure_text2()
    {
        if (text2_ready) return true;
        text2_stride = nnf_text2_stride(st->maxlen);
        size_t free_b = 0;
        if (!free_mem(free_b) || (size_t)n * text2_stride * 4 > free_b / 2 + st->pool.slots[SLOT_NN_TEXT2].cap) return false;
        d_text2.pool = &st->pool;
        d_text2.slot = SLOT_NN_TEXT2;
        if (d_text2.alloc((size_t)std::max<uint32_t>(n, 1) * text2_stride * 4) != ISOCON_OK) return false;
        hipLaunchKernelGGL(k_build_text2, dim3(std::max<uint32_t>(n, 1)), dim3(256), 0, 0, st->dev, d_text2.as<uint32_t>(), text2_stride);
        if (hipGetLastError() != hipSuccess) return false;
        text2_ready = true;
        return true;
    }
    static bool use_slot_order(uint32_t nq)
    {
        if (const char *e = variant_value("nn_order")) return atoi(e) != 0;
        return nq <= 16384;
    }
    int build_bounds(const QMap &Q, int32_t kcap, NNParams &P, bool want_seeds = false);
    std::vector<unsigned long long> lb_off_host;
    std::vector<uint32_t> lb_len_host;
    unsigned long long lb_total = 0;
    bool seeds_ready = false;
    uint32_t seed_nq = 0;
    int run_bound_seeds(const QMap &Q);
    DevBuf d_ltot, d_lchunks, d_list, d_lpa, d_lpb, d_lmeta, d_ltasks;
    struct ListPlan {
        bool listed = false;
        unsigned long long n_chunks = 0, n_chunks_narrow = 0, n_small = 0;
        unsigned long long conv_a = 0, conv_b = 0, conv_pairs = 0;
        NNChunk *a = nullptr, *b = nullptr, *sorted_a = nullptr, *sorted_b = nullptr;
    };
    int plan_lists(const QMap &Q, uint32_t nq, const NNParams &PR, ListPlan &L);
    NNParams params(int32_t kcap)
    {
        NNParams P;
        P.best = d_best.as<int32_t>();
        P.qflag = d_qf.as<uint8_t>();
        P.tflag = d_tf.as<uint8_t>();
        P.hits = d_hits.as<int32_t>();
        P.hit_count = d_hit_count.as<unsigned long long>();
        P.stats = d_stats.as<unsigned long long>();
        P.hits_cap = hits_cap;
        P.kcap = kcap;
        P.min_d = image_pass ? 0 : min_d;
        P.depth = depth;
        P.fixed = fixed ? 1 : 0;
        P.q_list = nullptr;
        P.own = QMap{0u, n, 1u, 0u};
        P.lb = nullptr;
        P.lb_row = nullptr;
        P.slot_order = nullptr;
        P.wg_base = 0;
        P.chunks = nullptr;
        P.list = nullptr;
        return P;
    }

    bool fill_best = false;
    bool best_on_host = true;
    int upload_best()
    {
        if (fill_best) {
            fill_best = false;
            if (n) ISO_HIP_CHECK(hipMemsetD32Async((hipDeviceptr_t)d_best.p, NN_INF, n, 0));
            return ISOCON_OK;
        }
        ISO_HIP_CHECK(copy_h2d(d_best.p, best.data(), (size_t)n * 4));
        return ISOCON_OK;
    }
    int download_best() { ISO_HIP_CHECK(copy_d2h(best.data(), d_best.p, (size_t)n * 4)); best_on_host = true; return ISOCON_OK; }
    static constexpr uint32_t N_COUNTERS = 2 * (NN_COUNTER_SLOTS * 4 + 1);
    int reset_counters()
    {
        ISO_HIP_CHECK(hipMemsetAsync(d_hit_count.p, 0, 8, 0));
        ISO_HIP_CHECK(hipMemsetAsync(d_stats.p, 0, N_COUNTERS * 8, 0));
        return ISOCON_OK;
    }
    void add_counters(const unsigned long long *sc2)
    {
        for (int blk = 0; blk < 2; ++blk) {
            const unsigned long long *sc = sc2 + blk * (NN_COUNTER_SLOTS * 4 + 1);
            stats.pairs_prefiltered += sc[NN_COUNTER_SLOTS * 4];
            for (int i = 0; i < NN_COUNTER_SLOTS; ++i) {
                stats.pairs_evaluated += sc[i * 4 + 0];
                stats.cells_columns += sc[i * 4 + 1];
                stats.tiles += sc[i * 4 + 2];
                stats.live_columns += sc[i * 4 + 3];
                if (blk == 1) stats.narrow_columns += sc[i * 4 + 1];
            }
        }
    }
    bool keep_dev = false;
    const int32_t *dev_hits = nullptr;
    uint64_t dev_hit_count = 0;
    int collect(std::vector<int32_t> &out, uint64_t *needed, bool filter = false, bool to_device = false)
    {
        unsigned long long cnt = 0;
        ISO_HIP_CHECK(memcpy_wait(&cnt, d_hit_count.p, 8, hipMemcpyDeviceToHost));
        unsigned long long sc2[N_COUNTERS];
        ISO_HIP_CHECK(memcpy_wait(sc2, d_stats.p, sizeof(sc2), hipMemcpyDeviceToHost));
        add_counters(sc2);
        if (needed) *needed = cnt;
        if (cnt > hits_cap) return ISOCON_E_CAPACITY;
        stats.hits += cnt;
        const void *src = d_hits.p;
        if (filter && cnt > 4096 && dev_hit_count == 0) {
            DevBuf d_h2(&st->pool, SLOT_NN_HITS2), d_c2(&st->pool, SLOT_NN_HITCOUNT2);
            int rc;
            if ((rc = d_h2.alloc((size_t)cnt * 12)) || (rc = d_c2.alloc(8))) return rc;
            ISO_HIP_CHECK(hipMemsetAsync(d_c2.p, 0, 8, 0));
            const unsigned blocks = (unsigned)std::min<unsigned long long>((cnt + 255) / 256, 4096);
            hipLaunchKernelGGL(k_filter_hits, dim3(blocks), dim3(256), 0, 0, d_hits.as<int32_t>(), cnt, d_best.as<int32_t>(), d_h2.as<int32_t>(),
                               d_c2.as<unsigned long long>());
            ISO_HIP_CHECK(hipGetLastError());
            ISO_HIP_CHECK(memcpy_wait(&cnt, d_c2.p, 8, hipMemcpyDeviceToHost));
            src = d_h2.p;
        }
        if (to_device) {
            dev_hits = static_cast<const int32_t *>(src);
            dev_hit_count = cnt;
            return ISOCON_OK;
        }
        const size_t base = out.size();
        out.resize(base + (size_t)cnt * 3);
        if (cnt) ISO_HIP_CHECK(copy_d2h(out.data() + base, src, (size_t)cnt * 12));
        return ISOCON_OK;
    }
    bool csr_follows = false;
    bool wide_needed = false;
    int collect_record(uint64_t *needed)
    {
        DevBuf d_rec(&st->pool, SLOT_NN_RECORD);
        int rc;
        if ((rc = d_rec.alloc((2 + N_COUNTERS) * 8))) return rc;
        ISO_HIP_CHECK(hipMemsetAsync(d_rec.p, 0, 16, 0));
        hipLaunchKernelGGL(k_nn_step_record, dim3(std::max<uint32_t>(1, (n + 255) / 256)), dim3(256), 0, 0, d_hit_count.as<unsigned long long>(), d_stats.as<unsigned long long>(),
                           N_COUNTERS, d_best.as<int32_t>(), d_qf.as<uint8_t>(), st->dev.lens, n, d_rec.as<unsigned long long>());
        ISO_HIP_CHECK(hipGetLastError());
        unsigned long long rec[2 + N_COUNTERS];
        ISO_HIP_CHECK(memcpy_wait(rec, d_rec.p, sizeof(rec), hipMemcpyDeviceToHost));
        add_counters(rec + 2);
        if (needed) *needed = rec[0];
        if (rec[0] > hits_cap) return ISOCON_E_CAPACITY;
        stats.hits += rec[0];
        wide_needed = rec[1] != 0;
        dev_hits = d_hits.as<int32_t>();
        dev_hit_count = rec[0];
        best_on_host = false;
        return ISOCON_OK;
    }
    int pull_dev_hits()
    {
        if (dev_hit_count) {
            const size_t base = hits.size();
            hits.resize(base + (size_t)dev_hit_count * 3);
            ISO_HIP_CHECK(copy_d2h(hits.data() + base, dev_hits, (size_t)dev_hit_count * 12));
        }
        dev_hits = nullptr;
        dev_hit_count = 0;
        return ISOCON_OK;
    }
    bool is_exc(uint32_t q) const { return st->n_exc != 0 && st->exc[q] != 0; }
    bool mask_exc = true;
    bool image_pass = false;
    bool fixed = false;
    bool dev_excluded(uint32_t q) const { return mask_exc && is_exc(q); }
    bool flags_dirty = false;
    bool roles_uniform = false;
    int upload_flags(bool fresh = false)
    {
        if (!n) return ISOCON_OK;
        if (fresh && roles_uniform && !st->n_exc) {
            ISO_HIP_CHECK(hipMemsetAsync(d_qf.p, 1, n, 0));
            ISO_HIP_CHECK(hipMemsetAsync(d_tf.p, 1, n, 0));
            return ISOCON_OK;
        }
        if (!st->n_exc || !mask_exc) {
            ISO_HIP_CHECK(copy_h2d(d_qf.p, qflag.data(), n));
            ISO_HIP_CHECK(copy_h2d(d_tf.p, tflag.data(), n));
            return ISOCON_OK;
        }
        std::vector<uint8_t> q2(qflag), t2(tflag);
        for (uint32_t i = 0; i < n; ++i)
            if (st->exc[i]) q2[i] = t2[i] = 0;
        ISO_HIP_CHECK(copy_h2d(d_qf.p, q2.data(), n));
        ISO_HIP_CHECK(copy_h2d(d_tf.p, t2.data(), n));
        return ISOCON_OK;
    }
    bool admissible(uint32_t x, uint32_t y) const { return qflag[x] && tflag[y]; }
    void apply(uint32_t s, uint32_t p, int32_t d)
    {
        if (d < min_d) return;
        const int32_t ls = st->lens[s], lp = st->lens[p];
        if (admissible(s, p) && d <= ls && d <= best[s]) { if (!fixed) best[s] = d; hits.push_back((int32_t)s); hits.push_back((int32_t)p); hits.push_back(d); }
        if (admissible(p, s) && d <= lp && d <= best[p]) { if (!fixed) best[p] = d; hits.push_back((int32_t)p); hits.push_back((int32_t)s); hits.push_back(d); }
    }
};

template <int W>
int launch_nn_tiles(NNContext &C, const std::vector<uint32_t> &ts, const std::vector<uint32_t> &ids, int32_t kcap, float *ms_out)
{
    const size_t nt = ts.size();
    if (!nt) return ISOCON_OK;
    DevBuf d_ts(&C.st->pool, SLOT_NN_TS), d_ids(&C.st->pool, SLOT_NN_IDS);
    int rc;
    if ((rc = d_ts.alloc(nt * 4)) || (rc = d_ids.alloc(nt * 64 * 4))) return rc;
    ISO_HIP_CHECK(copy_h2d(d_ts.p, ts.data(), nt * 4));
    ISO_HIP_CHECK(copy_h2d(d_ids.p, ids.data(), nt * 64 * 4));
    C.tm.start();
    hipLaunchKernelGGL(k_nn_tiles<W>, dim3((unsigned)((nt + 3) / 4)), dim3(256), 0, 0, C.st->dev, C.params(kcap),
                       d_ts.as<uint32_t>(), d_ids.as<uint32_t>(), (uint32_t)nt);
    ISO_HIP_CHECK(hipGetLastError());
    const float ms = C.tm.stop();
    if (ms_out) *ms_out += ms;
    return ISOCON_OK;
}

int run_nn_tiles(int W, NNContext &C, const std::vector<uint32_t> &ts, const std::vector<uint32_t> &ids, float *ms_out)
{
    switch (W) {
    case 1: return launch_nn_tiles<1>(C, ts, ids, 63, ms_out);
    case 2: return launch_nn_tiles<2>(C, ts, ids, 127, ms_out);
    case 4: return launch_nn_tiles<4>(C, ts, ids, 255, ms_out);
    case 8: return launch_nn_tiles<8>(C, ts, ids, 511, ms_out);
    default: return ISOCON_E_ARG;
    }
}

void push_tiles(std::vector<uint32_t> &ts, std::vector<uint32_t> &ids, uint32_t shared, const std::vector<uint32_t> &lanes)
{
    for (size_t i = 0; i < lanes.size(); i += 64) {
        ts.push_back(shared);
        for (size_t l = 0; l < 64; ++l) ids.push_back(i + l < lanes.size() ? lanes[i + l] : 0xffffffffu);
    }
}

void length_window(const std::vector<int32_t> &lens, uint32_t x, int32_t w, uint32_t &lo, uint32_t &hi)
{
    const int32_t L = lens[x];
    lo = (uint32_t)(std::lower_bound(lens.begin(), lens.end(), L - w) - lens.begin());
    hi = (uint32_t)(std::upper_bound(lens.begin(), lens.end(), L + w) - lens.begin());
}

int nn_setup(NNContext &C, isocon_store *s, const uint8_t *is_converged, const uint8_t *is_target, uint64_t depth,
             const int32_t *best_in, bool depth_walk = false)
{
    C.st = s;
    C.n = s->dev.n;
    C.d_best.pool = C.d_qf.pool = C.d_tf.pool = C.d_hits.pool = C.d_hit_count.pool = C.d_stats.pool = &s->pool;
    C.d_best.slot = SLOT_NN_BEST; C.d_qf.slot = SLOT_NN_QF; C.d_tf.slot = SLOT_NN_TF; C.d_hits.slot = SLOT_NN_HITS;
    C.d_hit_count.slot = SLOT_NN_HITCOUNT; C.d_stats.slot = SLOT_NN_STATS;
    const uint32_t n = C.n;
    for (uint32_t i = 1; i < n; ++i)
        if (s->lens[i] < s->lens[i - 1]) { g_last_error = "nearest-neighbour entry points need a length-sorted store"; return ISOCON_E_ARG; }
    C.two_set = is_target != nullptr;
    C.roles_uniform = !C.two_set && !is_converged;
    C.min_d = C.two_set ? 0 : 1;
    C.qflag.assign(n, 0);
    C.tflag.assign(n, 0);
    uint64_t n_targets = 0;
    for (uint32_t i = 0; i < n; ++i) {
        if (C.two_set) { C.tflag[i] = is_target[i] ? 1 : 0; C.qflag[i] = is_target[i] ? 0 : 1; n_targets += C.tflag[i]; }
        else { C.tflag[i] = 1; C.qflag[i] = (is_converged && is_converged[i]) ? 0 : 1; }
    }
    if (C.two_set) {
        C.depth_binds = depth < n_targets;
        if (C.depth_binds && !depth_walk) { g_last_error = "2-set search with neighbor_search_depth < number of targets is not supported"; return ISOCON_E_UNSUPPORTED; }
        C.depth = 0x7fffffffu;
    } else {
        if (depth == 0) { g_last_error = "neighbor_search_depth must be >= 1"; return ISOCON_E_ARG; }
        C.depth = depth > 0x7fffffffull ? 0x7fffffffu : (uint32_t)depth;
    }
    HostClock clk;
    C.best.assign(std::max<uint32_t>(n, 1), NN_INF);
    if (best_in) std::copy(best_in, best_in + n, C.best.begin());
    clk.lap("setup: host arrays");
    memset(&C.stats, 0, sizeof(C.stats));
    C.hits_cap = ((uint64_t)1 << 20) + (uint64_t)n * 48;
    if (const char *e = variant_value("hits_cap")) C.hits_cap = std::max<uint64_t>(16, strtoull(e, nullptr, 10));
    int rc;
    if ((rc = C.d_best.alloc((size_t)std::max<uint32_t>(n, 1) * 4)) || (rc = C.d_qf.alloc(std::max<uint32_t>(n, 1))) ||
        (rc = C.d_tf.alloc(std::max<uint32_t>(n, 1))) || (rc = C.d_hits.alloc(C.hits_cap * 12)) || (rc = C.d_hit_count.alloc(8)) ||
        (rc = C.d_stats.alloc(2 * (NN_COUNTER_SLOTS * 4 + 1) * 8)))
        return rc;
    clk.lap("setup: pool");
    if ((rc = C.upload_flags(true))) return rc;
    clk.lap("setup: role flags");
    return ISOCON_OK;
}

bool qmap_args_ok(uint32_t q_stride, uint32_t q_block) { return q_stride != 0 && q_block != 0 && (q_block & (q_block - 1)) == 0 && q_block <= q_stride; }
QMap qmap_of(uint32_t q_begin, uint32_t q_end, uint32_t q_stride, uint32_t q_block)
{
    uint32_t lg = 0;
    while ((1u << lg) < q_block) ++lg;
    return QMap{q_begin, q_end, q_stride, lg};
}

}
```

isocon_amd/csrc/nn_entry.inc:

```

namespace {

int nn_phase_a(NNContext &C, const QMap &Q, bool allow_regroup = false, bool do_seed = true, bool do_main = true, bool seeded_before = false)
{
    if (!C.st->n_exc || !do_main) return nn_phase_a_planes(C, Q, allow_regroup, do_seed, do_main, seeded_before);
    return nn_phase_a_images(C, Q, allow_regroup, do_seed, seeded_before);
}

int nn_phase_b(NNContext &C, const QMap &Q)
{
    return C.st->n_exc ? nn_phase_b_images(C, Q) : nn_phase_b_planes(C, Q);
}


struct WaitScope {
    isocon_store *s;
    explicit WaitScope(isocon_store *st) : s(st) { g_host_waits = 0; }
    ~WaitScope() { if (s) s->last_host_waits = g_host_waits; }
};

int nn_finalize_device_core(ScratchPool *pl, uint32_t n, const int32_t *d_best, const int32_t *best_host, const int32_t *d_hits, uint64_t n_hits,
                            int32_t *out_best, uint64_t *out_row_ptr, uint32_t *out_cols, uint64_t cols_cap, uint64_t *n_cols_needed)
{
    DevBuf d_cnt(pl, SLOT_NN_FIN_CNT), d_start(pl, SLOT_NN_FIN_START), d_cur(pl, SLOT_NN_FIN_CUR), d_nb(pl, SLOT_NN_FIN_NB),
        d_len2(pl, SLOT_NN_FIN_LEN2), d_out(pl, SLOT_NN_FIN_OUT), d_rec(pl, SLOT_NN_FIN_FLAG);
    static_assert(sizeof(unsigned long long) == sizeof(uint64_t), "row pointers travel as they are");
    const size_t rp_bytes = (((size_t)n + 1) * 8 + 15) & ~(size_t)15, best_bytes = best_host ? 0 : ((size_t)n * 4 + 15) & ~(size_t)15;
    const size_t cols_off = rp_bytes + best_bytes;
    int rc;
    if ((rc = d_cnt.alloc((size_t)n * 4)) || (rc = d_start.alloc(((size_t)n + 1) * 8)) || (rc = d_cur.alloc((size_t)n * 4)) ||
        (rc = d_nb.alloc((size_t)n_hits * 4 + 16)) || (rc = d_len2.alloc((size_t)n * 4)) || (rc = d_out.alloc(cols_off + (size_t)n_hits * 4 + 16)) ||
        (rc = d_rec.alloc(16)))
        return rc;
    unsigned long long *d_rowptr = d_out.as<unsigned long long>();
    int32_t *d_best_out = best_host ? nullptr : reinterpret_cast<int32_t *>(d_out.as<char>() + rp_bytes);
    uint32_t *d_cols = reinterpret_cast<uint32_t *>(d_out.as<char>() + cols_off);
    ISO_HIP_CHECK(hipMemsetAsync(d_cnt.p, 0, (size_t)n * 4, 0));
    ISO_HIP_CHECK(hipMemsetAsync(d_cur.p, 0, (size_t)n * 4, 0));
    ISO_HIP_CHECK(hipMemsetAsync(d_rec.p, 0, 16, 0));
    const unsigned hb = (unsigned)std::max<uint64_t>(1, (n_hits + 255) / 256), nb_ = (n + 255) / 256;
    hipLaunchKernelGGL(k_fin_count, dim3(hb), dim3(256), 0, 0, d_hits, (unsigned long long)n_hits, d_best, n, d_cnt.as<uint32_t>());
    if ((rc = device_exscan<0, unsigned long long>(pl, d_cnt.as<uint32_t>(), n, d_start.as<unsigned long long>()))) return rc;
    hipLaunchKernelGGL(k_fin_scatter, dim3(hb), dim3(256), 0, 0, d_hits, (unsigned long long)n_hits, d_best, n,
                       d_start.as<unsigned long long>(), d_cur.as<uint32_t>(), d_nb.as<uint32_t>());
    hipLaunchKernelGGL(k_fin_rows, dim3(nb_), dim3(256), 0, 0, n, d_start.as<unsigned long long>(), d_nb.as<uint32_t>(), d_len2.as<uint32_t>(), d_rec.as<uint32_t>());
    if ((rc = device_exscan<0, unsigned long long>(pl, d_len2.as<uint32_t>(), n, d_rowptr))) return rc;
    hipLaunchKernelGGL(k_fin_gather, dim3(nb_), dim3(256), 0, 0, n, d_start.as<unsigned long long>(), d_nb.as<uint32_t>(), d_rowptr, d_cols);
    hipLaunchKernelGGL(k_fin_pack, dim3(std::max(1u, nb_)), dim3(256), 0, 0, n, d_rowptr, d_rec.as<unsigned long long>(), d_best, d_best_out);
    ISO_HIP_CHECK(hipGetLastError());
    unsigned long long rec[2] = {0, 0};
    ISO_HIP_CHECK(memcpy_wait(rec, d_rec.p, sizeof(rec), hipMemcpyDeviceToHost));
    if (rec[0]) return ISOCON_E_UNSUPPORTED;
    const uint64_t total = rec[1];
    if (n_cols_needed) *n_cols_needed = total;
    if (total > cols_cap) return ISOCON_E_CAPACITY;
    const size_t bytes = cols_off + (size_t)total * 4;
    char *stg = bytes <= kStageBytes ? static_cast<char *>(g_stage.get(kStageBytes)) : nullptr;
    const int32_t *best_src = best_host;
    std::vector<int32_t> best_tmp;
    if (stg) {
        ISO_HIP_CHECK(memcpy_wait(stg, d_out.p, bytes, hipMemcpyDeviceToHost));
        memcpy(out_row_ptr, stg, ((size_t)n + 1) * 8);
        if (total) memcpy(out_cols, stg + cols_off, (size_t)total * 4);
        if (!best_src) best_src = reinterpret_cast<const int32_t *>(stg + rp_bytes);
    } else {
        ISO_HIP_CHECK(copy_d2h(out_row_ptr, d_rowptr, ((size_t)n + 1) * 8));
        if (total) ISO_HIP_CHECK(copy_d2h(out_cols, d_cols, (size_t)total * 4));
        if (!best_src) {
            best_tmp.resize(std::max<uint32_t>(n, 1));
            if (n) ISO_HIP_CHECK(copy_d2h(best_tmp.data(), d_best_out, (size_t)n * 4));
            best_src = best_tmp.data();
        }
    }
    for (uint32_t i = 0; i < n; ++i) out_best[i] = out_row_ptr[i + 1] > out_row_ptr[i] ? best_src[i] : -1;
    return ISOCON_OK;
}

int nn_finalize_device(isocon_store *st, uint32_t n, const int32_t *best, const int32_t *hits, uint64_t n_hits, int32_t *out_best,
                       uint64_t *out_row_ptr, uint32_t *out_cols, uint64_t cols_cap, uint64_t *n_cols_needed)
{
    ScratchPool *pl = &st->pool;
    DevBuf d_hits(pl, SLOT_NN_FIN_HITS), d_best(pl, SLOT_NN_FIN_BEST);
    int rc;
    if ((rc = d_hits.alloc((size_t)n_hits * 12)) || (rc = d_best.alloc((size_t)n * 4))) return rc;
    ISO_HIP_CHECK(copy_h2d(d_hits.p, hits, (size_t)n_hits * 12));
    ISO_HIP_CHECK(copy_h2d(d_best.p, best, (size_t)n * 4));
    return nn_finalize_device_core(pl, n, d_best.as<int32_t>(), best, d_hits.as<int32_t>(), n_hits, out_best, out_row_ptr, out_cols, cols_cap, n_cols_needed);
}

int nn2_depth_graph(NNContext &C, uint64_t depth, int32_t *out_best, uint64_t *out_row_ptr, uint32_t *out_cols, uint64_t cols_cap,
                    uint64_t *n_cols_needed, isocon_nn_stats *stats);


}

extern "C" int isocon_nn_partial(isocon_store *s, const uint8_t *is_converged, const uint8_t *is_target, uint64_t depth,
                                 uint32_t q_begin, uint32_t q_end, uint32_t q_stride, uint32_t q_block, int32_t phase, int32_t *best_inout,
                                 int32_t *out_hits, uint64_t hits_cap, uint64_t *n_hits, isocon_nn_stats *stats, const uint8_t *wide_queries)
{
    if (!s || !best_inout || !n_hits || (hits_cap && !out_hits) || phase < 0 || phase > 3 || !qmap_args_ok(q_stride, q_block)) return ISOCON_E_ARG;
    const uint32_t n = s->dev.n;
    if (q_end > n) q_end = n;
    const QMap Q = qmap_of(q_begin, q_end, q_stride, q_block);
    WaitScope waits(s);
    NNContext C;
    int rc = nn_setup(C, s, is_converged, is_target, depth, best_inout);
    if (rc) return rc;
    if (phase == 2 && wide_queries) C.wide_mask.assign(wide_queries, wide_queries + n);
    rc = phase == 2 ? nn_phase_b(C, Q) : nn_phase_a(C, Q, false, phase == 0 || phase == 3, phase == 1 || phase == 3, phase == 1);
    if (rc) return rc;
    C.tm.resolve();
    C.stats.kernel_ms = C.tm.total; C.stats.narrow_kernel_ms = C.tm.marked_total;
    if (stats) *stats = C.stats;
    std::copy(C.best.begin(), C.best.begin() + n, best_inout);
    *n_hits = C.hits.size() / 3;
    if (*n_hits > hits_cap) return ISOCON_E_CAPACITY;
    if (!C.hits.empty()) memcpy(out_hits, C.hits.data(), C.hits.size() * 4);
    return ISOCON_OK;
}

extern "C" int isocon_nn_finalize(uint32_t n, const int32_t *best, const int32_t *hits, uint64_t n_hits,
                                  int32_t *out_best, uint64_t *out_row_ptr, uint32_t *out_cols, uint64_t cols_cap,
                                  uint64_t *n_cols_needed)
{
    if ((n && (!best || !out_best)) || !out_row_ptr || (n_hits && !hits) || (cols_cap && !out_cols)) return ISOCON_E_ARG;
    return nn_finalize_impl(n, best, hits, n_hits, out_best, out_row_ptr, out_cols, cols_cap, n_cols_needed);
}

extern "C" int isocon_nn_partial_dev(isocon_store *s, const uint8_t *is_converged, const uint8_t *is_target, uint64_t depth,
                                     uint32_t q_begin, uint32_t q_end, uint32_t q_stride, uint32_t q_block, int32_t phase, int32_t *best_inout_dev,
                                     int32_t keep_hits, uint64_t *n_hits_held, isocon_nn_stats *stats, const uint8_t *wide_queries)
{
    if (!s || !best_inout_dev || !n_hits_held || phase < 0 || phase > 3 || !qmap_args_ok(q_stride, q_block)) return ISOCON_E_ARG;
    const uint32_t n = s->dev.n;
    if (q_end > n) q_end = n;
    const QMap Q = qmap_of(q_begin, q_end, q_stride, q_block);
    WaitScope waits(s);
    std::vector<int32_t> best(std::max<uint32_t>(n, 1), NN_INF);
    if (n) ISO_HIP_CHECK(copy_d2h(best.data(), best_inout_dev, (size_t)n * 4));
    NNContext C;
    int rc = nn_setup(C, s, is_converged, is_target, depth, best.data());
    if (rc) return rc;
    if (phase == 2 && wide_queries) C.wide_mask.assign(wide_queries, wide_queries + n);
    C.keep_dev = phase != 2;
    rc = phase == 2 ? nn_phase_b(C, Q) : nn_phase_a(C, Q, false, phase == 0 || phase == 3, phase == 1 || phase == 3, phase == 1);
    if (rc) return rc;
    C.tm.resolve();
    C.stats.kernel_ms = C.tm.total; C.stats.narrow_kernel_ms = C.tm.marked_total;
    if (stats) *stats = C.stats;
    if (n) ISO_HIP_CHECK(copy_h2d(best_inout_dev, C.best.data(), (size_t)n * 4));
    if (!keep_hits || s->pool.held_hits.store_serial != s->serial) s->pool.held_hits = HeldHits{s->serial, 0};
    const uint64_t add_host = C.hits.size() / 3, add = add_host + C.dev_hit_count, have = s->pool.held_hits.rows;
    ScratchPool::Slot &slot = s->pool.slots[SLOT_NN_ACC_HITS];
    if ((have + add) * 12 > slot.cap) {
        void *bigger = nullptr;
        const size_t want = (size_t)(have + add) * 12 * 2 + ((size_t)1 << 20);
        ISO_HIP_CHECK(hipMalloc(&bigger, want));
        if (have) ISO_HIP_CHECK(memcpy_wait(bigger, slot.p, (size_t)have * 12, hipMemcpyDeviceToDevice));
        if (slot.p) (void)hipFree(slot.p);
        slot.p = bigger; slot.cap = want;
    }
    if (add_host) ISO_HIP_CHECK(copy_h2d(static_cast<char *>(slot.p) + (size_t)have * 12, C.hits.data(), (size_t)add_host * 12));
    if (C.dev_hit_count)
        ISO_HIP_CHECK(memcpy_wait(static_cast<char *>(slot.p) + (size_t)(have + add_host) * 12, C.dev_hits, (size_t)C.dev_hit_count * 12, hipMemcpyDeviceToDevice));
    s->pool.held_hits.rows = have + add;
    *n_hits_held = s->pool.held_hits.rows;
    return ISOCON_OK;
}

extern "C" int isocon_nn_hits_dev(isocon_store *s, const int32_t *best_dev, int32_t *out_hits_dev, uint64_t cap_rows, uint64_t *n_kept)
{
    if (!s || !best_dev || (cap_rows && !out_hits_dev)) return ISOCON_E_ARG;
    uint64_t rows = s->pool.held_hits.store_serial == s->serial ? s->pool.held_hits.rows : 0;
    if (s->pool.slots[SLOT_NN_ACC_HITS].cap < rows * 12) rows = 0;
    if (rows > cap_rows) return ISOCON_E_CAPACITY;
    if (cap_rows) ISO_HIP_CHECK(hipMemsetAsync(out_hits_dev, 0xff, (size_t)cap_rows * 12, 0));
    unsigned long long kept = 0;
    if (rows) {
        DevBuf d_c(&s->pool, SLOT_NN_HITCOUNT2);
        int rc;
        if ((rc = d_c.alloc(8))) return rc;
        ISO_HIP_CHECK(hipMemsetAsync(d_c.p, 0, 8, 0));
        const unsigned blocks = (unsigned)std::min<unsigned long long>((rows + 255) / 256, 4096);
        hipLaunchKernelGGL(k_filter_hits, dim3(blocks), dim3(256), 0, 0, static_cast<const int32_t *>(s->pool.slots[SLOT_NN_ACC_HITS].p), (unsigned long long)rows,
                           best_dev, out_hits_dev, d_c.as<unsigned long long>());
        ISO_HIP_CHECK(hipGetLastError());
        if (n_kept) ISO_HIP_CHECK(memcpy_wait(&kept, d_c.p, 8, hipMemcpyDeviceToHost));
    }
    if (n_kept) *n_kept = kept;
    return ISOCON_OK;
}

extern "C" int isocon_nn_finalize_dev(isocon_store *s, const int32_t *best_dev, const int32_t *hits_dev, uint64_t n_rows,
                                      int32_t *out_best, uint64_t *out_row_ptr, uint32_t *out_cols, uint64_t cols_cap, uint64_t *n_cols_needed)
{
    if (!s || !out_row_ptr || (n_rows && !hits_dev) || (cols_cap && !out_cols)) return ISOCON_E_ARG;
    const uint32_t n = s->dev.n;
    if (n && (!best_dev || !out_best)) return ISOCON_E_ARG;
    std::vector<int32_t> best(std::max<uint32_t>(n, 1));
    if (n) ISO_HIP_CHECK(copy_d2h(best.data(), best_dev, (size_t)n * 4));
    int rc = nn_finalize_device_core(&s->pool, n, best_dev, best.data(), hits_dev, n_rows, out_best, out_row_ptr, out_cols, cols_cap, n_cols_needed);
    if (rc != ISOCON_E_UNSUPPORTED) return rc;
    std::vector<int32_t> hits((size_t)n_rows * 3);
    if (n_rows) ISO_HIP_CHECK(copy_d2h(hits.data(), hits_dev, (size_t)n_rows * 12));
    return nn_finalize_impl(n, best.data(), hits.data(), n_rows, out_best, out_row_ptr, out_cols, cols_cap, n_cols_needed);
}

extern "C" int isocon_nn_graph(isocon_store *s, const uint8_t *is_converged, const uint8_t *is_target, uint64_t depth,
                               int32_t *out_best, uint64_t *out_row_ptr, uint32_t *out_cols, uint64_t cols_cap,
                               uint64_t *n_cols_needed, isocon_nn_stats *stats)
{
    if (!s || !out_best || !out_row_ptr || (cols_cap && !out_cols)) return ISOCON_E_ARG;
    const uint32_t n = s->dev.n;
    HostClock clk0;
    if (getenv("ISOCON_DEBUG")) { (void)hipDeviceSynchronize(); clk0.lap("sync at entry"); }
    struct Total { std::chrono::steady_clock::time_point t = std::chrono::steady_clock::now();
                   ~Total() { if (getenv("ISOCON_DEBUG")) fprintf(stderr, "[isocon] %-28s %8.2f ms\n", "isocon_nn_graph total", std::chrono::duration<double, std::milli>(std::chrono::steady_clock::now() - t).count()); } } total;
    WaitScope waits(s);
    NNContext C;
    int rc = nn_setup(C, s, is_converged, is_target, depth, nullptr, true);
    if (rc) return rc;
    clk0.lap("setup");
    if (getenv("ISOCON_DEBUG")) { (void)hipDeviceSynchronize(); clk0.lap("sync after setup"); }
    if (C.two_set && (C.depth_binds || variant("nn_2set_walk"))) return nn2_depth_graph(C, depth, out_best, out_row_ptr, out_cols, cols_cap, n_cols_needed, stats);
    C.keep_dev = n >= 1024 && !variant("nn_host_finalize");
    C.csr_follows = C.keep_dev;
    C.fill_best = !s->n_exc;
    if ((rc = nn_phase_a(C, QMap{0u, n, 1u, 0u}, true, true, true))) return rc;
    HostClock clk;
    C.keep_dev = C.csr_follows = C.fill_best = false;
    bool run_b = true;
    if (!C.best_on_host) {
        if (C.wide_needed || !C.dev_hit_count) {
            if ((rc = C.download_best()) || (rc = C.pull_dev_hits())) return rc;
        } else run_b = false;
    }
    if (run_b && (rc = nn_phase_b(C, QMap{0u, n, 1u, 0u}))) return rc;
    clk.lap("phaseB");
    C.tm.resolve();
    if (C.dev_hit_count) {
        if (C.hits.empty()) {
            C.stats.kernel_ms = C.tm.total; C.stats.narrow_kernel_ms = C.tm.marked_total;
            if (stats) *stats = C.stats;
            rc = nn_finalize_device_core(&s->pool, n, C.d_best.as<int32_t>(), C.best_on_host ? C.best.data() : nullptr, C.dev_hits, C.dev_hit_count, out_best, out_row_ptr, out_cols, cols_cap, n_cols_needed);
            clk.lap("finalize (device hits)");
            if (rc != ISOCON_E_UNSUPPORTED && rc != ISOCON_E_HIP) return rc;
        }
        if (!C.best_on_host && (rc = C.download_best())) return rc;
        if ((rc = C.pull_dev_hits())) return rc;
    }
    C.stats.kernel_ms = C.tm.total; C.stats.narrow_kernel_ms = C.tm.marked_total;
    if (stats) *stats = C.stats;
    struct Lap { HostClock &c; ~Lap() { c.lap("finalize"); } } lap{clk};
    if (C.hits.size() / 3 >= 4096 && n >= 1024 && !variant("nn_host_finalize")) {
        rc = nn_finalize_device(s, n, C.best.data(), C.hits.data(), C.hits.size() / 3, out_best, out_row_ptr, out_cols, cols_cap, n_cols_needed);
        if (rc != ISOCON_E_UNSUPPORTED && rc != ISOCON_E_HIP) return rc;
    }
    return nn_finalize_impl(n, C.best.data(), C.hits.data(), C.hits.size() / 3, out_best, out_row_ptr, out_cols, cols_cap, n_cols_needed);
}

extern "C" int isocon_qgram_bound_matrix(isocon_store *s, uint32_t q_begin, uint32_t q_end, uint32_t q_stride, uint32_t q_block, uint64_t depth,
                                         uint64_t *out_row_ptr, uint8_t *out_bounds, uint64_t bounds_cap, uint64_t *n_bounds_needed)
{
    if (!s || !out_row_ptr || !qmap_args_ok(q_stride, q_block) || (bounds_cap && !out_bounds)) return ISOCON_E_ARG;
    if (s->n_exc) { g_last_error = "q-gram bounds are defined on the 2-bit planes: the set holds more than four distinct symbols"; return ISOCON_E_ALPHABET; }
    const uint32_t n = s->dev.n;
    if (q_end > n) q_end = n;
    NNContext C;
    int rc = nn_setup(C, s, nullptr, nullptr, depth, nullptr);
    if (rc) return rc;
    NNParams P = C.params(63);
    s->pool.bound_tag.valid = false;
    const QMap Q = qmap_of(q_begin, q_end, q_stride, q_block);
    const uint32_t nq = Q.count();
    if ((rc = C.build_bounds(Q, 63, P))) return rc;
    ISO_HIP_CHECK(device_wait());
    C.tm.resolve();
    s->pool.bound_tag.valid = false;
    uint64_t total = 0;
    if (P.lb == nullptr) {
        for (uint32_t r = 0; r <= nq; ++r) out_row_ptr[r] = 0;
        if (n_bounds_needed) *n_bounds_needed = 0;
        bool any = false;
        for (uint32_t r = 0; r < C.lb_len_host.size(); ++r) any = any || C.lb_len_host[r] != 0;
        if (any) { g_last_error = "bound matrix not built (memory)"; return ISOCON_E_UNSUPPORTED; }
        return ISOCON_OK;
    }
    for (uint32_t r = 0; r < nq; ++r) { out_row_ptr[r] = total; total += C.lb_len_host[r]; }
    out_row_ptr[nq] = total;
    if (n_bounds_needed) *n_bounds_needed = total;
    if (total > bounds_cap) return ISOCON_E_CAPACITY;
    std::vector<uint8_t> raw((size_t)C.lb_total);
    ISO_HIP_CHECK(copy_d2h(raw.data(), P.lb, (size_t)C.lb_total));
    for (uint32_t r = 0; r < nq; ++r)
        if (C.lb_len_host[r]) memcpy(out_bounds + out_row_ptr[r], raw.data() + C.lb_off_host[r], C.lb_len_host[r]);
    if (C.d_lbt.p != nullptr) {
        std::vector<unsigned long long> offT(n);
        std::vector<uint32_t> sloT(n), lenT(n);
        ISO_HIP_CHECK(copy_d2h(offT.data(), C.d_offT.p, (size_t)n * 8));
        ISO_HIP_CHECK(copy_d2h(sloT.data(), C.d_sloT.p, (size_t)n * 4));
        ISO_HIP_CHECK(copy_d2h(lenT.data(), C.d_lenT.p, (size_t)n * 4));
        unsigned long long endT = 0, cells = 0;
        for (uint32_t p = 0; p < n; ++p) if (lenT[p]) endT = std::max(endT, offT[p] + lenT[p]);
        std::vector<uint8_t> rawT((size_t)endT + 1);
        if (endT) ISO_HIP_CHECK(copy_d2h(rawT.data(), C.d_lbt.p, (size_t)endT));
        for (uint32_t p = 0; p < n; ++p)
            for (uint32_t i = 0; i < lenT[p]; ++i) {
                const uint32_t r = sloT[p] + i;
                const uint64_t q = Q.entry(r);
                if (r >= nq || q >= p || p - q - 1 >= C.lb_len_host[r] || rawT[offT[p] + i] != raw[C.lb_off_host[r] + (p - q - 1)]) {
                    g_last_error = "transposed bound matrix differs from the matrix at entry " + std::to_string(p) + ", slot " + std::to_string(r);
                    return ISOCON_E_HIP;
                }
                ++cells;
            }
        if (cells != total) { g_last_error = "transposed bound matrix holds " + std::to_string(cells) + " cells, the matrix " + std::to_string(total); return ISOCON_E_HIP; }
    }
    return ISOCON_OK;
}
```

isocon_amd/csrc/nn_finalize.hpp:

```cpp
#pragma once
#include "nn_list.hpp"

namespace isocon {

static constexpr uint32_t NN_FIN_MAX_ROW = 256;

__device__ __forceinline__ bool nn_fin_valid(const int32_t *__restrict__ hits, unsigned long long h, const int32_t *__restrict__ best, uint32_t n,
                                             uint32_t &e, uint32_t &o)
{
    const int32_t a = hits[h * 3], b = hits[h * 3 + 1], d = hits[h * 3 + 2];
    if (a < 0 || b < 0 || (uint32_t)a >= n || (uint32_t)b >= n || d < 0 || d != best[a]) return false;
    e = (uint32_t)a; o = (uint32_t)b;
    return true;
}

__global__ __launch_bounds__(256) void k_fin_count(const int32_t *__restrict__ hits, unsigned long long n_hits, const int32_t *__restrict__ best, uint32_t n,
                                                    uint32_t *__restrict__ cnt)
{
    const unsigned long long h = (unsigned long long)blockIdx.x * 256u + threadIdx.x;
    uint32_t e, o;
    if (h < n_hits && nn_fin_valid(hits, h, best, n, e, o)) atomicAdd(cnt + e, 1u);
}

__global__ __launch_bounds__(256) void k_fin_scatter(const int32_t *__restrict__ hits, unsigned long long n_hits, const int32_t *__restrict__ best, uint32_t n,
                                                      const unsigned long long *__restrict__ start, uint32_t *__restrict__ cursor, uint32_t *__restrict__ nb)
{
    const unsigned long long h = (unsigned long long)blockIdx.x * 256u + threadIdx.x;
    uint32_t e, o;
    if (h < n_hits && nn_fin_valid(hits, h, best, n, e, o)) nb[start[e] + atomicAdd(cursor + e, 1u)] = o;
}

__global__ __launch_bounds__(256) void k_fin_rows(uint32_t n, const unsigned long long *__restrict__ start, uint32_t *__restrict__ nb, uint32_t *__restrict__ len2,
                                                   uint32_t *__restrict__ too_long)
{
    const uint32_t i = blockIdx.x * 256u + threadIdx.x;
    if (i >= n) return;
    uint32_t *b = nb + start[i];
    const uint32_t len = (uint32_t)(start[i + 1] - start[i]);
    if (len > NN_FIN_MAX_ROW) { atomicOr(too_long, 1u); len2[i] = len; return; }
    auto before = [i](uint32_t x, uint32_t y) {
        const uint32_t ox = x > i ? x - i : i - x, oy = y > i ? y - i : i - y;
        return ox != oy ? ox < oy : x < y;
    };
    for (uint32_t a = 1; a < len; ++a) {
        const uint32_t v = b[a];
        uint32_t c = a;
        while (c > 0 && before(v, b[c - 1])) { b[c] = b[c - 1]; --c; }
        b[c] = v;
    }
    uint32_t w = 0;
    for (uint32_t a = 0; a < len; ++a)
        if (a == 0 || b[a] != b[a - 1]) b[w++] = b[a];
    len2[i] = w;
}

__global__ __launch_bounds__(256) void k_fin_gather(uint32_t n, const unsigned long long *__restrict__ start, const uint32_t *__restrict__ nb,
                                                     const unsigned long long *__restrict__ row_ptr, uint32_t *__restrict__ cols)
{
    const uint32_t i = blockIdx.x * 256u + threadIdx.x;
    if (i >= n) return;
    const uint32_t len = (uint32_t)(row_ptr[i + 1] - row_ptr[i]);
    const uint32_t *src = nb + start[i];
    uint32_t *dst = cols + row_ptr[i];
    for (uint32_t a = 0; a < len; ++a) dst[a] = src[a];
}

__global__ __launch_bounds__(256) void k_fin_pack(uint32_t n, const unsigned long long *__restrict__ row_ptr, unsigned long long *__restrict__ rec,
                                                   const int32_t *__restrict__ best, int32_t *__restrict__ best_out)
{
    const uint32_t i = blockIdx.x * 256u + threadIdx.x;
    if (i == 0) rec[1] = row_ptr[n];
    if (best_out != nullptr && i < n) best_out[i] = best[i];
}

__global__ __launch_bounds__(256) void k_nn_step_record(const unsigned long long *__restrict__ hit_count, const unsigned long long *__restrict__ stats, uint32_t n_stats,
                                                         const int32_t *__restrict__ best, const uint8_t *__restrict__ qflag, const int32_t *__restrict__ lens,
                                                         uint32_t n, unsigned long long *__restrict__ rec)
{
    const uint32_t i = blockIdx.x * 256u + threadIdx.x;
    if (blockIdx.x == 0) {
        if (threadIdx.x == 0) rec[0] = *hit_count;
        for (uint32_t k = threadIdx.x; k < n_stats; k += 256u) rec[2 + k] = stats[k];
    }
    const bool wide = i < n && qflag[i] != 0 && best[i] == NN_INF && lens[i] > 63;
    if (__ballot(wide) != 0 && (threadIdx.x & 63u) == 0) atomicOr(rec + 1, 1ull);
}

}
```

isocon_amd/csrc/nn_lists.inc:

```

namespace {

int NNContext::plan_lists(const QMap &Q, uint32_t nq, const NNParams &PR, ListPlan &L)
{
    L = ListPlan();
    if (PR.lb == nullptr || nq == 0 || variant("nn_no_list") || st->pool.slots[SLOT_NN_LBT].p == nullptr || st->maxlen >= 16384) return ISOCON_OK;
    unsigned long long pairs_cap = std::min<unsigned long long>(lb_total, std::max<unsigned long long>(1ull << 22, lb_total / 8));
    if (const char *e = variant_value("nn_list_cap")) pairs_cap = std::max<unsigned long long>(1, strtoull(e, nullptr, 10));
    const bool filter = !variant("nn_no_block_filter") && ensure_text2();
    uint32_t list_min = NN_LIST_MIN;
    if (const char *e = variant_value("nn_list_min")) list_min = (uint32_t)std::max(1, atoi(e));
    const uint32_t build_min = filter ? std::min<uint32_t>(list_min, NNF_LIST_MIN) : list_min;
    const unsigned long long cap_in = pairs_cap / build_min + 1, cap_out = filter ? pairs_cap / list_min + 1 : cap_in;
    size_t free_b = 0;
    if (!free_mem(free_b) || pairs_cap * 12 > free_b / 2 + st->pool.slots[SLOT_NN_LIST].cap * 3) return ISOCON_OK;
    DevBuf *bufs[] = {&d_ltot, &d_lchunks, &d_list, &d_lpa, &d_lpb, &d_lmeta, &d_ltasks};
    const int slots[] = {SLOT_NN_LTOT, SLOT_NN_LCHUNKS, SLOT_NN_LIST, SLOT_NN_LPA, SLOT_NN_LPB, SLOT_NN_LDEST, SLOT_NN_LTASKS};
    for (int i = 0; i < 7; ++i) { bufs[i]->pool = &st->pool; bufs[i]->slot = slots[i]; }
    const bool second = filter && !variant("nn_filter_one_pass");
    const unsigned long long tasks_cap = second ? 2 * cap_in + pairs_cap / 64 + 1 : 0;
    if (second && d_ltasks.alloc((size_t)tasks_cap * sizeof(NNFTask))) return ISOCON_OK;
    const size_t n_records = (size_t)(filter ? 2 * cap_in : 0) + 4 * (size_t)cap_out;
    if (d_lmeta.alloc(((size_t)n + NN_META_PAD) * 4) || d_ltot.alloc(sizeof(NNPlanTotals)) || d_lchunks.alloc(n_records * sizeof(NNChunk)) || d_list.alloc((size_t)pairs_cap * 4) ||
        d_lpa.alloc((size_t)pairs_cap * 4) || d_lpb.alloc((size_t)pairs_cap * 4))
        return ISOCON_OK;
    NNChunk *built = d_lchunks.as<NNChunk>();
    L.a = built + (filter ? 2 * cap_in : 0);
    L.b = L.a + cap_out;
    L.sorted_a = L.b + cap_out;
    L.sorted_b = L.sorted_a + cap_out;
    ISO_HIP_CHECK(hipMemsetAsync(d_ltot.p, 0, sizeof(NNPlanTotals), 0));
    NNBoundRows B;
    B.lb = PR.lb; B.row_off = PR.lb_row; B.row_len = static_cast<const uint32_t *>(st->pool.slots[SLOT_NN_LBLEN].p);
    B.lbT = static_cast<const uint8_t *>(st->pool.slots[SLOT_NN_LBT].p);
    B.offT = static_cast<const unsigned long long *>(st->pool.slots[SLOT_NN_LBT_OFF].p);
    B.sloT = static_cast<const uint32_t *>(st->pool.slots[SLOT_NN_LBT_SLO].p);
    B.lenT = static_cast<const uint32_t *>(st->pool.slots[SLOT_NN_LBT_LEN].p);
    B.score = static_cast<const uint32_t *>(st->pool.slots[SLOT_NN_SCORE].p);
    tm.start();
    int32_t class_mode = 0;
    if (const char *e = variant_value("nn_narrow")) class_mode = atoi(e) > 0 ? 1 : -1;
    hipLaunchKernelGGL(k_nn_entry_meta, dim3((n + NN_META_PAD + 255) / 256), dim3(256), 0, 0, st->dev, PR, B.score, d_lmeta.as<uint32_t>(), d_ltot.as<NNPlanTotals>());
    ISO_HIP_CHECK(hipGetLastError());
    hipLaunchKernelGGL(k_nn_survivors, dim3((n + NN_SURV_WAVES - 1) / NN_SURV_WAVES), dim3(64 * NN_SURV_WAVES), 0, 0, st->dev, PR, B, d_lmeta.as<uint32_t>(), Q, nq, d_list.as<uint32_t>(), pairs_cap,
                       filter ? built : L.a, cap_in, d_lpa.as<uint32_t>(), d_lpb.as<uint32_t>(), pairs_cap, d_ltot.as<NNPlanTotals>(), build_min, class_mode);
    ISO_HIP_CHECK(hipGetLastError());
    if (filter) {
        tm.mark();
        hipLaunchKernelGGL(k_nn_block_filter, dim3(NNF_GRID), dim3(256), 0, 0, d_text2.as<uint32_t>(), text2_stride, st->dev.lens, d_lmeta.as<uint32_t>(), PR.kcap, d_list.as<uint32_t>(),
                           built, cap_in, L.a, cap_out, d_lpa.as<uint32_t>(), d_lpb.as<uint32_t>(), pairs_cap, d_ltot.as<NNPlanTotals>(), list_min,
                           second ? d_ltasks.as<NNFTask>() : (NNFTask *)nullptr, tasks_cap);
        ISO_HIP_CHECK(hipGetLastError());
        if (second) {
            hipLaunchKernelGGL(k_nn_block_filter2, dim3(NNF_GRID2), dim3(256), 0, 0, d_text2.as<uint32_t>(), text2_stride, st->dev.lens, d_lmeta.as<uint32_t>(), PR.kcap,
                               d_list.as<uint32_t>(), d_ltasks.as<NNFTask>(), tasks_cap, d_lpa.as<uint32_t>(), d_lpb.as<uint32_t>(), pairs_cap, d_ltot.as<NNPlanTotals>());
            ISO_HIP_CHECK(hipGetLastError());
        }
    }
    tm.stop_later(&stats.list_kernel_ms, &stats.filter_kernel_ms);
    NNPlanTotals tot;
    ISO_HIP_CHECK(memcpy_wait(&tot, d_ltot.p, sizeof(tot), hipMemcpyDeviceToHost));
    if (tot.overflow) return ISOCON_OK;
    stats.pairs_prefiltered += tot.n_filtered;
    stats.pairs_block_rejected += tot.f_rejected + tot.f_rejected2;
    L.listed = true;
    L.n_chunks = filter ? tot.f_chunks : tot.n_chunks;
    L.n_chunks_narrow = filter ? tot.f_chunks_narrow : tot.n_chunks_narrow;
    L.n_small = tot.n_small;
    stats.pairs_wide_to_lanes += tot.n_wide_pairs;
    unsigned long long table_chunks = NNF_TABLE_CHUNKS;
    if (const char *e = variant_value("nn_table_chunks")) table_chunks = strtoull(e, nullptr, 10);
    if (filter && L.n_chunks + L.n_chunks_narrow > 0 && L.n_chunks + L.n_chunks_narrow < table_chunks) {
        if (tot.n_small + tot.f_listed > pairs_cap) return ISOCON_OK;
        L.conv_a = L.n_chunks; L.conv_b = L.n_chunks_narrow; L.conv_pairs = tot.f_listed;
        L.n_chunks = L.n_chunks_narrow = 0;
        return ISOCON_OK;
    }
    stats.pairs_narrow += filter ? tot.f_narrow_listed : tot.n_narrow_listed;
    return ISOCON_OK;
}

}
```

isocon_amd/csrc/nn_main.inc:

```

namespace {

template <int NW, bool HALF>
int launch_refill_as(NNContext &C, const NNRefillShape &sh, unsigned grid, const NNParams &P, const QMap &Q, int32_t first_tile)
{
    if (sh.raise_limit) ISO_HIP_CHECK(hipFuncSetAttribute((const void *)k_nn_scan_refill<NW, 1, HALF>, hipFuncAttributeMaxDynamicSharedMemorySize, (int)sh.lds));
    hipLaunchKernelGGL((k_nn_scan_refill<NW, 1, HALF>), dim3(grid), dim3(NW * 64), sh.lds, 0, C.st->dev, P, C.d_text.as<uint32_t>(), C.text_stride, Q, first_tile);
    ISO_HIP_CHECK(hipGetLastError());
    return ISOCON_OK;
}

int launch_refill(NNContext &C, const NNRefillShape &sh, bool half, unsigned grid, const NNParams &P, const QMap &Q, int32_t first_tile)
{
    switch (sh.waves) {
    case 4: return half ? launch_refill_as<4, true>(C, sh, grid, P, Q, first_tile) : launch_refill_as<4, false>(C, sh, grid, P, Q, first_tile);
    case 8: return half ? launch_refill_as<8, true>(C, sh, grid, P, Q, first_tile) : launch_refill_as<8, false>(C, sh, grid, P, Q, first_tile);
    default: return half ? launch_refill_as<16, true>(C, sh, grid, P, Q, first_tile) : launch_refill_as<16, false>(C, sh, grid, P, Q, first_tile);
    }
}

struct Regrouped {
    std::vector<uint32_t> perm;
    std::vector<int32_t> seed_got;
    bool seed_collected = false;
    const std::vector<int32_t> *best_at_entry = nullptr;
    const uint64_t *planes = nullptr;

    int unpermute(NNContext &C, std::vector<int32_t> &got) const
    {
        std::vector<int32_t> b(C.n);
        for (uint32_t i = 0; i < C.n; ++i) b[perm[i]] = C.best[i];
        std::copy(b.begin(), b.end(), C.best.begin());
        for (size_t i = 0; i + 2 < got.size(); i += 3) { got[i] = (int32_t)perm[got[i]]; got[i + 1] = (int32_t)perm[got[i + 1]]; }
        return C.upload_flags();
    }
};

struct PhaseAPass {
    bool do_seed, do_main, seeded_before;
    bool refill_main = false;
    bool bounds_wanted = false;
    NNParams PR;
    bool bound_seeded = false, bounds_built = false;
    bool seeds_clean;
    bool no_markers = false;
    Regrouped G;
    PhaseAPass(bool seed, bool main_, bool before) : do_seed(seed), do_main(main_), seeded_before(before), seeds_clean(!seed) {}
};

int phase_a_seeds(NNContext &C, const QMap &Q, PhaseAPass &P, HostClock &clk)
{
    int rc;
    if (P.bounds_wanted && !variant("nn_old_seed")) {
        if ((rc = C.build_bounds(Q, 63, P.PR, true))) return rc;
        P.bounds_built = true;
        clk.lap("phaseA: q-gram bounds");
        if (C.seeds_ready) {
            if ((rc = C.run_bound_seeds(Q))) return rc;
            P.bound_seeded = P.seeds_clean = true;
            clk.lap("phaseA: seed pairs");
            return ISOCON_OK;
        }
    }
    C.tm.start();
    hipLaunchKernelGGL(k_nn_scan_up<1>, dim3((Q.count() + 3) / 4), dim3(256), 0, 0, C.st->dev, C.params(63), Q, 0, 1, 1);
    ISO_HIP_CHECK(hipGetLastError());
    C.tm.stop_later(&C.stats.seed_kernel_ms);
    clk.lap("phaseA: seed kernel");
    return ISOCON_OK;
}

int regroup_by_seed_hits(NNContext &C, const std::vector<int32_t> &best_at_entry, Regrouped &G, HostClock &clk)
{
    const uint32_t n = C.n;
    uint64_t needed0 = 0;
    std::vector<int32_t> seed_hits;
    int rc = C.collect(seed_hits, &needed0);
    if (rc == ISOCON_E_CAPACITY) return ISOCON_OK;
    if (rc || (rc = C.download_best())) return rc;
    G.seed_got.swap(seed_hits);
    std::vector<uint32_t> parent(n);
    std::iota(parent.begin(), parent.end(), 0u);
    auto find = [&](uint32_t x) { while (parent[x] != x) { parent[x] = parent[parent[x]]; x = parent[x]; } return x; };
    for (size_t i = 0; i + 2 < G.seed_got.size(); i += 3) {
        if (G.seed_got[i + 2] < 0) continue;
        const uint32_t a = find((uint32_t)G.seed_got[i]), b = find((uint32_t)G.seed_got[i + 1]);
        if (a != b) parent[a < b ? b : a] = a < b ? a : b;
    }
    std::vector<uint32_t> &perm = G.perm;
    perm.resize(n);
    std::iota(perm.begin(), perm.end(), 0u);
    std::vector<uint32_t> root(n);
    for (uint32_t i = 0; i < n; ++i) root[i] = find(i);
    const std::vector<int32_t> &lens = C.st->lens;
    std::sort(perm.begin(), perm.end(), [&](uint32_t x, uint32_t y) {
        if (lens[x] != lens[y]) return lens[x] < lens[y];
        if (root[x] != root[y]) return root[x] < root[y];
        if (C.best[x] != C.best[y]) return C.best[x] < C.best[y];
        return x < y;
    });
    if (clk.on) {
        std::vector<uint8_t> seen(n, 0);
        bool okp = true;
        for (uint32_t i = 0; i < n; ++i) { if (seen[perm[i]]) okp = false; seen[perm[i]] = 1; }
        size_t ncomp = 0, moved = 0;
        for (uint32_t i = 0; i < n; ++i) { ncomp += root[i] == i; moved += perm[i] != i; }
        bool lens_ok = true;
        for (uint32_t i = 0; i < n; ++i) lens_ok = lens_ok && lens[perm[i]] == lens[i];
        fprintf(stderr, "[isocon] regroup: n=%u components=%zu moved=%zu perm_valid=%d lens_preserved=%d seed_hits=%zu\n",
                n, ncomp, moved, (int)okp, (int)lens_ok, G.seed_got.size() / 3);
    }
    bool identity = true;
    for (uint32_t i = 0; i < n && identity; ++i) identity = perm[i] == i;
    if (identity) perm.clear();
    else {
        DevBuf d_planes2(&C.st->pool, SLOT_NN_PLANES2), d_perm(&C.st->pool, SLOT_NN_PERM);
        const size_t pbytes = (size_t)n * C.st->dev.nchunks * 16;
        if ((rc = d_planes2.alloc(pbytes)) || (rc = d_perm.alloc((size_t)n * 4))) return rc;
        ISO_HIP_CHECK(copy_h2d(d_perm.p, perm.data(), (size_t)n * 4));
        C.tm.start();
        hipLaunchKernelGGL(k_permute_planes, dim3(2048), dim3(256), 0, 0, reinterpret_cast<const ulonglong2 *>(C.st->dev.planes),
                           d_planes2.as<ulonglong2>(), d_perm.as<uint32_t>(), n, C.st->dev.nchunks);
        ISO_HIP_CHECK(hipGetLastError());
        C.tm.stop();
        G.planes = d_planes2.as<uint64_t>();
        G.best_at_entry = &best_at_entry;
        std::vector<int32_t> b2(n);
        std::vector<uint8_t> q2(n), t2(n);
        for (uint32_t i = 0; i < n; ++i) { b2[i] = C.best[perm[i]]; q2[i] = C.dev_excluded(perm[i]) ? 0 : C.qflag[perm[i]]; t2[i] = C.dev_excluded(perm[i]) ? 0 : C.tflag[perm[i]]; }
        ISO_HIP_CHECK(copy_h2d(C.d_best.p, b2.data(), (size_t)n * 4));
        ISO_HIP_CHECK(copy_h2d(C.d_qf.p, q2.data(), n));
        ISO_HIP_CHECK(copy_h2d(C.d_tf.p, t2.data(), n));
    }
    if ((rc = C.reset_counters())) return rc;
    G.seed_collected = true;
    clk.lap("phaseA: regroup (host+permute)");
    return ISOCON_OK;
}

int run_listed_pass(NNContext &C, const QMap &Q, const NNParams &PR, const NNContext::ListPlan &LP)
{
    int rc;
    NNParams PL = PR;
    PL.list = C.d_list.as<uint32_t>();
    PL.slot_order = nullptr;
    const char *lw = variant_value("nn_list_waves");
    if ((LP.n_chunks || LP.n_chunks_narrow) && !C.build_text()) return ISOCON_E_HIP;
    if (LP.n_chunks) {
        hipLaunchKernelGGL(k_nn_sort_chunks, dim3(1), dim3(1024), 0, 0, LP.a, (uint32_t)LP.n_chunks, LP.sorted_a);
        ISO_HIP_CHECK(hipGetLastError());
        PL.chunks = LP.sorted_a;
        const char *pad = variant_value("nn_lds_pad");
        const NNRefillShape sh = pad ? nn_refill_shape_padded(C.st->maxlen, atoi(pad)) : nn_refill_shape(C.st->maxlen, lw ? atoi(lw) : 4, false);
        if ((rc = launch_refill(C, sh, false, (unsigned)LP.n_chunks, PL, Q, 0))) return rc;
    }
    if (LP.n_chunks_narrow) {
        C.tm.mark();
        hipLaunchKernelGGL(k_nn_sort_chunks, dim3(1), dim3(1024), 0, 0, LP.b, (uint32_t)LP.n_chunks_narrow, LP.sorted_b);
        ISO_HIP_CHECK(hipGetLastError());
        PL.chunks = LP.sorted_b;
        PL.stats = C.d_stats.as<unsigned long long>() + (NN_COUNTER_SLOTS * 4 + 1);
        if ((rc = launch_refill(C, nn_refill_shape(C.st->maxlen, lw ? atoi(lw) : 8, true), true, (unsigned)LP.n_chunks_narrow, PL, Q, 0))) return rc;
    }
    const unsigned long long n_small = LP.n_small + LP.conv_pairs;
    if (n_small) {
        C.tm.stop_later(&C.stats.scan_kernel_ms);
        C.tm.start();
        const unsigned long long pairs_cap = C.st->pool.slots[SLOT_NN_LPA].cap / 4;
        if (LP.conv_a) hipLaunchKernelGGL(k_nn_chunks_to_pairs, dim3((unsigned)LP.conv_a), dim3(256), 0, 0, LP.a, C.d_list.as<uint32_t>(), C.d_lpa.as<uint32_t>(), C.d_lpb.as<uint32_t>(), pairs_cap, C.d_ltot.as<NNPlanTotals>());
        if (LP.conv_b) hipLaunchKernelGGL(k_nn_chunks_to_pairs, dim3((unsigned)LP.conv_b), dim3(256), 0, 0, LP.b, C.d_list.as<uint32_t>(), C.d_lpa.as<uint32_t>(), C.d_lpb.as<uint32_t>(), pairs_cap, C.d_ltot.as<NNPlanTotals>());
        hipLaunchKernelGGL(k_ed_lanes<true>, dim3((unsigned)((n_small + 255) / 256)), dim3(256), 0, 0, C.st->dev, C.params(63), C.d_lpa.as<uint32_t>(), C.d_lpb.as<uint32_t>(),
                           (const int32_t *)nullptr, (uint64_t)n_small, (int32_t *)nullptr);
        ISO_HIP_CHECK(hipGetLastError());
        C.tm.stop_later(&C.stats.lanes_kernel_ms);
        C.stats.pairs_evaluated += n_small;
        C.stats.pairs_lanes += n_small;
        C.tm.start();
    }
    return ISOCON_OK;
}

int run_unlisted_pass(NNContext &C, const QMap &Q, const PhaseAPass &P, bool refill)
{
    const uint32_t nq = Q.count();
    const int32_t first_tile = (P.G.perm.empty() && ((P.do_seed && !P.bound_seeded) || (P.seeded_before && !P.bounds_wanted))) ? 1 : 0;
    if (refill) {
        if (!C.build_text()) return ISOCON_E_HIP;
        const char *wv = variant_value("nn_waves");
        const bool four = wv ? atoi(wv) == 4 : P.PR.lb != nullptr;
        return launch_refill(C, nn_refill_shape(C.st->maxlen, four ? 4 : 8, false), false, nq, P.PR, Q, first_tile);
    }
    DevStore S = C.st->dev;
    if (P.G.planes) S.planes = P.G.planes;
    const NNTileScan kernel = nn_tile_scan(C.st->maxlen);
    const size_t lds = nn_tile_scan_lds(C.st->maxlen);
    if (kernel == NN_SCAN_WINDOW) {
        hipLaunchKernelGGL(k_nn_scan_up<1>, dim3(nq), dim3(256), 0, 0, S, C.params(63), Q, first_tile, 0x7fffffff, 4);
        return ISOCON_OK;
    }
    DevBuf d_il(&C.st->pool, SLOT_NN_IL2);
    const size_t total = (size_t)C.n * C.st->dev.nchunks;
    int rc;
    if ((rc = d_il.alloc(total * 16))) return rc;
    hipLaunchKernelGGL(k_interleave_planes, dim3(2048), dim3(256), 0, 0, reinterpret_cast<const ulonglong2 *>(S.planes), d_il.as<ulonglong2>(), total);
    S.il = d_il.as<uint64_t>();
    if (kernel == NN_SCAN_LDS8) {
        hipLaunchKernelGGL(k_nn_scan_lds<8>, dim3(nq), dim3(512), lds, 0, S, C.params(63), Q, first_tile, 0x7fffffff);
    } else {
        ISO_HIP_CHECK(hipFuncSetAttribute((const void *)k_nn_scan_lds<16>, hipFuncAttributeMaxDynamicSharedMemorySize, (int)lds));
        hipLaunchKernelGGL(k_nn_scan_lds<16>, dim3(nq), dim3(1024), lds, 0, S, C.params(63), Q, first_tile, 0x7fffffff);
    }
    return ISOCON_OK;
}

int phase_a_main(NNContext &C, const QMap &Q, PhaseAPass &P, HostClock &clk)
{
    int rc;
    if (C.n >= (1u << 30)) { g_last_error = "store too large for the packed neighbour queue"; return ISOCON_E_ARG; }
    C.tm.start();
    const bool refill = P.refill_main && P.G.perm.empty() && C.text_affordable();
    NNParams &PR = P.PR;
    if (refill && P.bounds_wanted && !P.bounds_built) {
        C.tm.stop_later(&C.stats.scan_kernel_ms);
        if ((rc = C.build_bounds(Q, 63, PR))) return rc;
        clk.lap("phaseA: q-gram bounds");
        C.tm.start();
    }
    if (!refill) { PR.lb = nullptr; PR.lb_row = nullptr; PR.slot_order = nullptr; }
    NNContext::ListPlan LP;
    if (refill && PR.lb != nullptr) {
        C.tm.stop_later(&C.stats.scan_kernel_ms);
        if ((rc = C.plan_lists(Q, Q.count(), PR, LP))) return rc;
        clk.lap("phaseA: survivor lists");
        C.tm.start();
    }
    P.no_markers = LP.listed && P.seeds_clean;
    if ((rc = LP.listed ? run_listed_pass(C, Q, PR, LP) : run_unlisted_pass(C, Q, P, refill))) return rc;
    ISO_HIP_CHECK(hipGetLastError());
    C.tm.stop_later(&C.stats.scan_kernel_ms);
    C.stats.scan_launches += 1;
    return ISOCON_OK;
}

int phase_a_two_set_unbounded(NNContext &C, const QMap &Q)
{
    C.tm.start();
    if (!C.build_text()) return ISOCON_E_HIP;
    int rc;
    if ((rc = launch_refill(C, nn_refill_shape(C.st->maxlen, 8, false), false, Q.count(), C.params(63), Q, 0))) return rc;
    C.tm.stop_later(&C.stats.scan_kernel_ms);
    C.stats.scan_launches += 1;
    return ISOCON_OK;
}

int phase_a_two_set_tiles(NNContext &C, const QMap &Q, bool do_main)
{
    std::vector<uint32_t> ts, ids, lanes;
    for (uint32_t c = 0; c < C.n && do_main; ++c) {
        if (!C.tflag[c] || C.dev_excluded(c)) continue;
        uint32_t lo, hi;
        length_window(C.st->lens, c, 63, lo, hi);
        lo = std::max(lo, Q.begin);
        hi = std::min(hi, Q.end);
        lanes.clear();
        for (uint32_t p = lo; p < hi; ++p)
            if (C.qflag[p] && !C.dev_excluded(p) && Q.owns(p)) lanes.push_back(p);
        push_tiles(ts, ids, c, lanes);
    }
    float ms = 0.f;
    int rc;
    if ((rc = run_nn_tiles(1, C, ts, ids, &ms))) return rc;
    C.stats.scan_launches += 1;
    C.stats.scan_kernel_ms += ms;
    return ISOCON_OK;
}

int nn_end_pass(NNContext &C, int32_t kcap, bool no_markers, const Regrouped &G, HostClock *clk, bool &again)
{
    auto lap = [&](const char *what) { if (clk) clk->lap(what); };
    again = false;
    uint64_t needed = 0;
    std::vector<int32_t> got;
    const bool in_place = G.perm.empty();
    const bool dev_ok = C.keep_dev && no_markers && in_place && !G.seed_collected && C.hits.empty();
    const bool one_record = dev_ok && C.csr_follows && !C.st->n_exc && !C.flags_dirty;
    int rc = one_record ? C.collect_record(&needed) : C.collect(got, &needed, in_place, dev_ok);
    C.tm.resolve();
    if (rc == ISOCON_E_CAPACITY) {
        C.hits_cap = needed + needed / 2 + 1024;
        if ((rc = C.d_hits.alloc(C.hits_cap * 12))) return rc;
        again = true;
        if (in_place) return C.download_best();
        C.best = *G.best_at_entry;
        return C.upload_flags();
    }
    if (rc) return rc;
    if (one_record) { lap("phaseA: hits and bounds stay on the device"); return ISOCON_OK; }
    if ((rc = C.download_best())) return rc;
    if (dev_ok) { lap("phaseA: hits stay on the device"); return ISOCON_OK; }
    if (!in_place && (rc = G.unpermute(C, got))) return rc;
    if (G.seed_collected) got.insert(got.end(), G.seed_got.begin(), G.seed_got.end());
    lap("phaseA: collect+unpermute");
    std::vector<uint32_t> ra, rb;
    for (size_t i = 0; i + 2 < got.size(); i += 3) {
        if (got[i + 2] == -2) { ra.push_back((uint32_t)got[i]); rb.push_back((uint32_t)got[i + 1]); }
        else C.hits.insert(C.hits.end(), got.begin() + i, got.begin() + i + 3);
    }
    if (!ra.empty()) {
        std::vector<int32_t> kk(ra.size(), kcap), dd(ra.size(), -1);
        float ems = 0.f;
        if ((rc = ed_pairs_impl(C.st, ra.data(), rb.data(), kk.data(), ra.size(), dd.data(), &ems, nullptr, C.image_pass))) return rc;
        C.tm.total += ems;
        for (size_t i = 0; i < ra.size(); ++i)
            if (dd[i] >= 0) C.apply(ra[i], rb[i], dd[i]);
    }
    lap("phaseA: markers");
    return ISOCON_OK;
}

int nn_phase_a_planes(NNContext &C, const QMap &Q, bool allow_regroup = false,
                      bool do_seed = true, bool do_main = true, bool seeded_before = false)
{
    const uint32_t n = C.n;
    if (Q.begin >= Q.end) return ISOCON_OK;
    const std::vector<int32_t> best0 = C.best;
    HostClock clk;
    const bool fits = nn_refill64_fits(C.st->maxlen);
    const bool two_set_many = C.two_set && do_main && !variant("nn_tiles") && n < (1u << 30) && fits &&
                              (size_t)std::count(C.tflag.begin(), C.tflag.end(), (uint8_t)1) > 512;
    const bool two_set_lists = two_set_many && !variant("nn_no_qgram");
    const bool whole_set = Q.begin == 0 && Q.end == n && Q.stride == 1 && Q.block_log2 == 0 && C.depth >= n;
    for (;;) {
        int rc;
        if ((rc = C.upload_best()) || (rc = C.reset_counters())) return rc;
        clk.lap("phaseA: upload/reset");
        PhaseAPass P(do_seed, do_main, seeded_before);
        if (!C.two_set || two_set_lists) {
            P.refill_main = !variant("nn_tiles") && fits;
            P.bounds_wanted = P.refill_main && !variant("nn_no_qgram");
            P.PR = C.params(63);
            if (do_seed && (rc = phase_a_seeds(C, Q, P, clk))) return rc;
            if (allow_regroup && !P.refill_main && do_seed && do_main && whole_set && n > 128 && (rc = regroup_by_seed_hits(C, best0, P.G, clk))) return rc;
            if (do_main && (rc = phase_a_main(C, Q, P, clk))) return rc;
            if (!do_main) P.no_markers = do_seed && P.seeds_clean;
            clk.lap("phaseA: main kernel");
        } else if (two_set_many && C.text_affordable()) {
            if ((rc = phase_a_two_set_unbounded(C, Q))) return rc;
        } else if ((rc = phase_a_two_set_tiles(C, Q, do_main))) return rc;
        bool again = false;
        if ((rc = nn_end_pass(C, 63, P.no_markers, P.G, &clk, again))) return rc;
        if (!again) return ISOCON_OK;
    }
}

}
```

Measured before the change: 79.06 billion alignments/s.

## Run bounds prep and list setup on a forked side stream lane

Replaces the single-event side upload with a fork/join side lane backed by an event ring. Bounds prep kernels (scan, row offsets, memsets for seed and min buffers) and list/text2 preparation can now run on the side stream, overlapping with the q-gram profile kernel on the main stream. It also fuses the finalize pack into the gather kernel, makes the count and scatter kernels grid-stride over a device-side hit count, and adds a fused step-reset kernel. The cost is more complex stream ordering with join points that must cover every consumer, which raises the risk of races.

After: 79.58 billion alignments/s, median of 6. About the same (+0.7%).

```diff
diff --git a/isocon_amd/csrc/isocon_hip.hip b/isocon_amd/csrc/isocon_hip.hip
--- a/isocon_amd/csrc/isocon_hip.hip
+++ b/isocon_amd/csrc/isocon_hip.hip
@@ -169,6 +169,8 @@
     void release() { if (p) (void)hipHostFree(p); p = nullptr; cap = 0; }
 };
 static PinnedStage g_stage;
+static PinnedStage g_csr_stage;
+static bool g_csr_stage_busy = false;
 static constexpr size_t kStageBytes = (size_t)32 << 20;
 static constexpr uint64_t kPackWaves = (uint64_t)1 << 25;
 static constexpr size_t kStageMin = (size_t)32 << 10;
@@ -214,38 +216,67 @@
     return hipSuccess;
 }
 
-struct SideUpload {
+struct SideLane {
+    static constexpr unsigned N_EVENTS = 8;
     hipStream_t stream = nullptr;
-    hipEvent_t before = nullptr, done = nullptr;
+    hipEvent_t ring[N_EVENTS] = {};
+    unsigned at = 0;
+    bool open = false;
     PinnedStage pinned;
     bool in_flight = false;
     bool ready()
     {
         if (stream) return true;
         if (hipStreamCreateWithFlags(&stream, hipStreamNonBlocking) != hipSuccess) { stream = nullptr; (void)hipGetLastError(); return false; }
-        if (hipEventCreateWithFlags(&before, hipEventDisableTiming) != hipSuccess || hipEventCreateWithFlags(&done, hipEventDisableTiming) != hipSuccess) {
-            (void)hipGetLastError();
-            release();
-            return false;
-        }
+        for (hipEvent_t &e : ring)
+            if (hipEventCreateWithFlags(&e, hipEventDisableTiming) != hipSuccess) {
+                e = nullptr;
+                (void)hipGetLastError();
+                release();
+                return false;
+            }
         return true;
     }
+    hipEvent_t forked = nullptr;
+    bool fork()
+    {
+        hipEvent_t e = ring[at++ % N_EVENTS];
+        if (hipEventRecord(e, 0) != hipSuccess) { (void)hipGetLastError(); return false; }
+        forked = e;
+        open = true;
+        return true;
+    }
+    hipError_t enter()
+    {
+        if (!forked) return hipSuccess;
+        hipEvent_t e = forked;
+        forked = nullptr;
+        return hipStreamWaitEvent(stream, e, 0);
+    }
+    hipError_t join()
+    {
+        open = false;
+        forked = nullptr;
+        hipEvent_t e = ring[at++ % N_EVENTS];
+        const hipError_t err = hipEventRecord(e, stream);
+        return err != hipSuccess ? err : hipStreamWaitEvent(0, e, 0);
+    }
     void settle()
     {
         if (!in_flight) return;
-        if (hipEventQuery(done) != hipSuccess || hipStreamQuery(stream) != hipSuccess) { (void)hipGetLastError(); ++g_host_waits; (void)hipStreamSynchronize(stream); }
+        if (hipStreamQuery(stream) != hipSuccess) { (void)hipGetLastError(); ++g_host_waits; (void)hipStreamSynchronize(stream); }
         in_flight = false;
     }
     void release()
     {
         if (stream) { (void)hipStreamSynchronize(stream); (void)hipStreamDestroy(stream); }
-        if (before) (void)hipEventDestroy(before);
-        if (done) (void)hipEventDestroy(done);
-        stream = nullptr; before = done = nullptr; in_flight = false;
+        for (hipEvent_t &e : ring) { if (e) (void)hipEventDestroy(e); e = nullptr; }
+        stream = nullptr; forked = nullptr; in_flight = open = false;
         pinned.release();
     }
 };
-static SideUpload g_side;
+static SideLane g_side;
+struct SideJoinGuard { ~SideJoinGuard() { if (g_side.open) (void)g_side.join(); } };
 
 struct DevBuf {
     void *p = nullptr;
@@ -271,14 +302,14 @@
 };
 
 template <int SHIFT, class OUT>
-static int device_exscan(ScratchPool *pl, const uint32_t *d_in, uint32_t n, OUT *d_out)
+static int device_exscan(ScratchPool *pl, const uint32_t *d_in, uint32_t n, OUT *d_out, hipStream_t stream = 0)
 {
     DevBuf d_tmp(pl, SLOT_SCAN_TMP), d_sums(pl, SLOT_SCAN_SUMS);
     const uint32_t tiles = std::max<uint32_t>(1, (n + SCAN_TILE - 1) / SCAN_TILE);
     int rc;
     if ((rc = d_tmp.alloc((size_t)std::max<uint32_t>(n, 1) * 4)) || (rc = d_sums.alloc((size_t)tiles * 8))) return rc;
-    hipLaunchKernelGGL((k_scan_tiles<SHIFT>), dim3(tiles), dim3(256), 0, 0, d_in, n, d_tmp.as<uint32_t>(), d_sums.as<unsigned long long>());
-    hipLaunchKernelGGL((k_scan_finish<OUT>), dim3(tiles), dim3(256), 0, 0, d_tmp.as<uint32_t>(), n, d_sums.as<unsigned long long>(), tiles, d_out, (unsigned long long *)nullptr);
+    hipLaunchKernelGGL((k_scan_tiles<SHIFT>), dim3(tiles), dim3(256), 0, stream, d_in, n, d_tmp.as<uint32_t>(), d_sums.as<unsigned long long>());
+    hipLaunchKernelGGL((k_scan_finish<OUT>), dim3(tiles), dim3(256), 0, stream, d_tmp.as<uint32_t>(), n, d_sums.as<unsigned long long>(), tiles, d_out, (unsigned long long *)nullptr);
     ISO_HIP_CHECK(hipGetLastError());
     return ISOCON_OK;
 }
@@ -440,7 +471,7 @@
     return n;
 }
 
-void isocon_release_scratch(void) { g_scratch.release(); g_stage.release(); g_events.release(); g_side.release(); }
+void isocon_release_scratch(void) { g_scratch.release(); g_stage.release(); g_csr_stage.release(); g_csr_stage_busy = false; g_events.release(); g_side.release(); }
 
 int isocon_init(int device_ordinal)
 {
diff --git a/isocon_amd/csrc/nn_bounds.inc b/isocon_amd/csrc/nn_bounds.inc
--- a/isocon_amd/csrc/nn_bounds.inc
+++ b/isocon_amd/csrc/nn_bounds.inc
@@ -30,11 +30,14 @@
         if (d_qprof.alloc(prof_bytes) || d_qsum.alloc((size_t)n * 4)) return ISOCON_OK;
     }
     bclk.lap("bounds: memory check + profile buffers");
-    const bool side = !variant("nn_sync_uploads") && g_side.ready() && hipEventRecord(g_side.before, 0) == hipSuccess;
+    const bool side = !variant("nn_sync_uploads") && g_side.ready() && (g_side.settle(), g_side.fork());
+    const bool lanes = side && !variant("nn_serial_prep");
+    const hipStream_t prep = lanes ? g_side.stream : (hipStream_t)0;
     tm.start();
     hipLaunchKernelGGL(k_qgram_profile4, dim3((n + QP_SEQS - 1) / QP_SEQS), dim3(256), 0, 0, st->dev, d_qprof.as<uint8_t>(), d_qsum.as<uint32_t>(), n_pad);
     ISO_HIP_CHECK(hipGetLastError());
     struct StopTimer { NNContext &c; bool armed = true; ~StopTimer() { if (armed) c.tm.stop_later(&c.stats.bound_kernel_ms); } } stop_timer{*this};
+    SideJoinGuard join_guard;
     std::vector<unsigned long long> &off = lb_off_host;
     std::vector<uint32_t> &rlen = lb_len_host;
     off.assign(nq, 0);
@@ -98,32 +101,35 @@
     if (d_lbt.alloc((size_t)totalT + 16) || d_offT.alloc(((size_t)n + 1) * 8) || d_sloT.alloc((size_t)n * 4) || d_lenT.alloc((size_t)n * 4) || d_score.alloc((size_t)n * 4) ||
         d_padT.alloc((size_t)n * 4))
         return ISOCON_OK;
-    ISO_HIP_CHECK(hipMemsetAsync(d_score.p, 0, (size_t)n * 4, 0));
+    if (!lanes) ISO_HIP_CHECK(hipMemsetAsync(d_score.p, 0, (size_t)n * 4, 0));
     d_chunks.pool = &st->pool;
     d_chunks.slot = SLOT_NN_LBCHUNKS;
     if (d_chunks.alloc(tiles.size() * sizeof(uint2))) return ISOCON_OK;
     const size_t b_tiles = (tiles.size() * sizeof(uint2) + 15) & ~(size_t)15, b_off = ((size_t)nq * 8 + 15) & ~(size_t)15, b_len = (size_t)nq * 4;
     char *pin = nullptr;
-    if (side) { g_side.settle(); pin = static_cast<char *>(g_side.pinned.get(b_tiles + b_off + b_len)); }
+    if (side) { pin = static_cast<char *>(g_side.pinned.get(b_tiles + b_off + b_len)); }
     if (pin) {
         memcpy(pin, tiles.data(), tiles.size() * sizeof(uint2));
         memcpy(pin + b_tiles, off.data(), (size_t)nq * 8);
         memcpy(pin + b_tiles + b_off, rlen.data(), (size_t)nq * 4);
         g_side.in_flight = true;
-        ISO_HIP_CHECK(hipStreamWaitEvent(g_side.stream, g_side.before, 0));
+        ISO_HIP_CHECK(g_side.enter());
         ISO_HIP_CHECK(hipMemcpyAsync(d_chunks.p, pin, tiles.size() * sizeof(uint2), hipMemcpyHostToDevice, g_side.stream));
         ISO_HIP_CHECK(hipMemcpyAsync(d_lbrow.p, pin + b_tiles, (size_t)nq * 8, hipMemcpyHostToDevice, g_side.stream));
         ISO_HIP_CHECK(hipMemcpyAsync(d_lblen.p, pin + b_tiles + b_off, (size_t)nq * 4, hipMemcpyHostToDevice, g_side.stream));
-        ISO_HIP_CHECK(hipEventRecord(g_side.done, g_side.stream));
-        ISO_HIP_CHECK(hipStreamWaitEvent(0, g_side.done, 0));
+        if (!lanes) ISO_HIP_CHECK(g_side.join());
     } else {
+        if (lanes) ISO_HIP_CHECK(g_side.join());
+
         ISO_HIP_CHECK(copy_h2d(d_chunks.p, tiles.data(), tiles.size() * sizeof(uint2)));
         ISO_HIP_CHECK(copy_h2d(d_lbrow.p, off.data(), (size_t)nq * 8));
         ISO_HIP_CHECK(copy_h2d(d_lblen.p, rlen.data(), (size_t)nq * 4));
     }
-    hipLaunchKernelGGL(k_lbt_rows, dim3((n + 255) / 256), dim3(256), 0, 0, Q, nq, d_lblen.as<uint32_t>(), n, d_sloT.as<uint32_t>(), d_lenT.as<uint32_t>(), d_padT.as<uint32_t>());
-    if ((rc = device_exscan<0, unsigned long long>(&st->pool, d_padT.as<uint32_t>(), n, d_offT.as<unsigned long long>()))) return ISOCON_OK;
-    hipLaunchKernelGGL(k_lbt_offsets, dim3((n + 255) / 256), dim3(256), 0, 0, n, d_sloT.as<uint32_t>(), d_offT.as<unsigned long long>());
+    const hipStream_t lane = pin ? prep : (hipStream_t)0;
+    if (lanes) ISO_HIP_CHECK(hipMemsetAsync(d_score.p, 0, (size_t)n * 4, lane));
+    hipLaunchKernelGGL(k_lbt_rows, dim3((n + 255) / 256), dim3(256), 0, lane, Q, nq, d_lblen.as<uint32_t>(), n, d_sloT.as<uint32_t>(), d_lenT.as<uint32_t>(), d_padT.as<uint32_t>());
+    if ((rc = device_exscan<0, unsigned long long>(&st->pool, d_padT.as<uint32_t>(), n, d_offT.as<unsigned long long>(), lane))) return ISOCON_OK;
+    hipLaunchKernelGGL(k_lbt_offsets, dim3((n + 255) / 256), dim3(256), 0, lane, n, d_sloT.as<uint32_t>(), d_offT.as<unsigned long long>());
     ISO_HIP_CHECK(hipGetLastError());
     bclk.lap("bounds: alloc + uploads");
     if (use_slot_order(nq)) {
@@ -140,11 +146,35 @@
         d_rowmin.pool = d_colmin.pool = d_seed_a.pool = d_seed_b.pool = &st->pool;
         d_rowmin.slot = SLOT_NN_ROWMIN; d_colmin.slot = SLOT_NN_COLMIN; d_seed_a.slot = SLOT_NN_SEED_A; d_seed_b.slot = SLOT_NN_SEED_B;
         if (!(d_rowmin.alloc((size_t)nq * 8 * QM_SEEDS) || d_colmin.alloc((size_t)n_pad * 8 * QM_SEEDS) || d_seed_a.alloc((size_t)n * 8 * QM_SEEDS) || d_seed_b.alloc((size_t)n * 8 * QM_SEEDS))) {
-            ISO_HIP_CHECK(hipMemsetAsync(d_rowmin.p, 0xff, (size_t)nq * 8 * QM_SEEDS, 0));
-            ISO_HIP_CHECK(hipMemsetAsync(d_colmin.p, 0xff, (size_t)n_pad * 8 * QM_SEEDS, 0));
+            ISO_HIP_CHECK(hipMemsetAsync(d_rowmin.p, 0xff, (size_t)nq * 8 * QM_SEEDS, lane));
+            ISO_HIP_CHECK(hipMemsetAsync(d_colmin.p, 0xff, (size_t)n_pad * 8 * QM_SEEDS, lane));
             rowmin = d_rowmin.as<unsigned long long>();
             colmin = d_colmin.as<unsigned long long>();
-        }
+            d_seed_n.pool = &st->pool;
+            d_seed_n.slot = SLOT_NN_SEED_N;
+            if (g_side.open && !d_seed_n.alloc(8)) {
+                ISO_HIP_CHECK(hipMemsetAsync(d_seed_n.p, 0, 8, lane));
+                ISO_HIP_CHECK(hipMemsetAsync(d_seed_a.p, 0xff, (size_t)n * 8 * QM_SEEDS, lane));
+                ISO_HIP_CHECK(hipMemsetAsync(d_seed_b.p, 0xff, (size_t)n * 8 * QM_SEEDS, lane));
+                seed_lists_filled = true;
+            }
+        }
+    }
+    const char *t2_lane = variant_value("nn_text2_lane");
+    const bool lists_by_seeds = t2_lane && strcmp(t2_lane, "seeds") == 0;
+    auto prepare_lists = [&](hipStream_t stream) -> int {
+        if (!variant("nn_no_list") && !variant("nn_no_block_filter") && st->maxlen < 16384) (void)ensure_text2(stream);
+        d_ltot.pool = &st->pool;
+        d_ltot.slot = SLOT_NN_LTOT;
+        if (!d_ltot.alloc(sizeof(NNPlanTotals))) {
+            ISO_HIP_CHECK(hipMemsetAsync(d_ltot.p, 0, sizeof(NNPlanTotals), stream));
+            ltot_zeroed = true;
+        }
+        return ISOCON_OK;
+    };
+    if (g_side.open) {
+        if (lists_follow && !lists_by_seeds && (rc = prepare_lists(lane))) return rc;
+        ISO_HIP_CHECK(g_side.join());
     }
     bclk.lap("bounds: slot order + seed buffers");
     static bool lds_attr_set = false;
@@ -160,6 +190,7 @@
     ISO_HIP_CHECK(hipGetLastError());
     stop_timer.armed = false;
     tm.stop_later(&stats.bound_kernel_ms, &stats.mm_kernel_ms);
+    if (lanes && pin && lists_follow && lists_by_seeds && g_side.fork() && g_side.enter() == hipSuccess && (rc = prepare_lists(g_side.stream))) return rc;
     bclk.lap("bounds: k_qgram_mm (enqueued)");
 #ifdef ISOCON_QM_TIMELINE
     {
@@ -204,12 +235,16 @@
     uint32_t col_classes = QM_SEEDS;
     while (col_classes > 1 && col_classes * ranks > (uint32_t)QM_SEEDS) col_classes >>= 1;
     if (const char *e = variant_value("nn_seed_classes")) { const int v = atoi(e); if (v == 1 || v == 2 || v == QM_SEEDS) col_classes = (uint32_t)v; }
-    DevBuf d_seed_n(&st->pool, SLOT_NN_SEED_N);
+    d_seed_n.pool = &st->pool;
+    d_seed_n.slot = SLOT_NN_SEED_N;
     int rc;
     if ((rc = d_seed_n.alloc(8))) return rc;
-    ISO_HIP_CHECK(hipMemsetAsync(d_seed_n.p, 0, 8, 0));
-    ISO_HIP_CHECK(hipMemsetAsync(d_seed_a.p, 0xff, (size_t)np * 4, 0));
-    ISO_HIP_CHECK(hipMemsetAsync(d_seed_b.p, 0xff, (size_t)np * 4, 0));
+    if (!seed_lists_filled) {
+        ISO_HIP_CHECK(hipMemsetAsync(d_seed_n.p, 0, 8, 0));
+        ISO_HIP_CHECK(hipMemsetAsync(d_seed_a.p, 0xff, (size_t)np * 4, 0));
+        ISO_HIP_CHECK(hipMemsetAsync(d_seed_b.p, 0xff, (size_t)np * 4, 0));
+    }
+    seed_lists_filled = false;
     hipLaunchKernelGGL(k_qgram_seed_pairs, dim3((n + 255) / 256), dim3(256), 0, 0, d_rowmin.as<unsigned long long>(), d_colmin.as<unsigned long long>(),
                        n, Q, seed_nq, col_classes, d_seed_a.as<uint32_t>(), d_seed_b.as<uint32_t>(), d_seed_n.as<unsigned long long>());
     ISO_HIP_CHECK(hipGetLastError());
diff --git a/isocon_amd/csrc/nn_context.inc b/isocon_amd/csrc/nn_context.inc
--- a/isocon_amd/csrc/nn_context.inc
+++ b/isocon_amd/csrc/nn_context.inc
@@ -12,6 +12,60 @@
         t0 = t1;
     }
 };
+
+struct CsrJob {
+    uint32_t n = 0;
+    size_t rp_bytes = 0, best_bytes = 0, cols_off = 0;
+    char *d_out = nullptr;
+    unsigned long long *d_rec = nullptr;
+    bool live = false;
+    hipEvent_t ev_rec = nullptr;
+    char *pin = nullptr;
+    static constexpr size_t PIN_REC = 0, PIN_FIXED = 16;
+    CsrJob() {}
+    CsrJob(const CsrJob &) = delete;
+    CsrJob &operator=(const CsrJob &) = delete;
+    ~CsrJob() { drop(); }
+    void drop() { g_events.put(ev_rec); ev_rec = nullptr; live = false; }
+};
+
+int csr_enqueue(ScratchPool *pl, uint32_t n, const int32_t *d_best, bool best_travels, const int32_t *d_hits, const unsigned long long *d_hit_count,
+                uint64_t rows, bool zeroed, CsrJob &J)
+{
+    DevBuf d_cnt(pl, SLOT_NN_FIN_CNT), d_start(pl, SLOT_NN_FIN_START), d_cur(pl, SLOT_NN_FIN_CUR), d_nb(pl, SLOT_NN_FIN_NB),
+        d_len2(pl, SLOT_NN_FIN_LEN2), d_out(pl, SLOT_NN_FIN_OUT), d_rec(pl, SLOT_NN_FIN_FLAG);
+    static_assert(sizeof(unsigned long long) == sizeof(uint64_t), "row pointers travel as they are");
+    J.n = n;
+    J.rp_bytes = (((size_t)n + 1) * 8 + 15) & ~(size_t)15;
+    J.best_bytes = best_travels ? ((size_t)n * 4 + 15) & ~(size_t)15 : 0;
+    J.cols_off = J.rp_bytes + J.best_bytes;
+    int rc;
+    if ((rc = d_cnt.alloc((size_t)n * 4)) || (rc = d_start.alloc(((size_t)n + 1) * 8)) || (rc = d_cur.alloc((size_t)n * 4)) ||
+        (rc = d_nb.alloc((size_t)rows * 4 + 16)) || (rc = d_len2.alloc((size_t)n * 4)) || (rc = d_out.alloc(J.cols_off + (size_t)rows * 4 + 16)) ||
+        (rc = d_rec.alloc(16)))
+        return rc;
+    J.d_out = d_out.as<char>();
+    J.d_rec = d_rec.as<unsigned long long>();
+    unsigned long long *d_rowptr = d_out.as<unsigned long long>();
+    int32_t *d_best_out = best_travels ? reinterpret_cast<int32_t *>(J.d_out + J.rp_bytes) : nullptr;
+    uint32_t *d_cols = reinterpret_cast<uint32_t *>(J.d_out + J.cols_off);
+    if (!zeroed) {
+        ISO_HIP_CHECK(hipMemsetAsync(d_cnt.p, 0, (size_t)n * 4, 0));
+        ISO_HIP_CHECK(hipMemsetAsync(d_cur.p, 0, (size_t)n * 4, 0));
+        ISO_HIP_CHECK(hipMemsetAsync(d_rec.p, 0, 16, 0));
+    }
+    const unsigned hb = (unsigned)std::min<uint64_t>(NN_FIN_GRID, std::max<uint64_t>(1, (rows + 255) / 256)), nb_ = std::max(1u, (n + 255) / 256);
+    hipLaunchKernelGGL(k_fin_count, dim3(hb), dim3(256), 0, 0, d_hits, d_hit_count, (unsigned long long)rows, d_best, n, d_cnt.as<uint32_t>());
+    if ((rc = device_exscan<0, unsigned long long>(pl, d_cnt.as<uint32_t>(), n, d_start.as<unsigned long long>()))) return rc;
+    hipLaunchKernelGGL(k_fin_scatter, dim3(hb), dim3(256), 0, 0, d_hits, d_hit_count, (unsigned long long)rows, d_best, n,
+                       d_start.as<unsigned long long>(), d_cur.as<uint32_t>(), d_nb.as<uint32_t>());
+    hipLaunchKernelGGL(k_fin_rows, dim3(nb_), dim3(256), 0, 0, n, d_start.as<unsigned long long>(), d_nb.as<uint32_t>(), d_len2.as<uint32_t>(), d_rec.as<uint32_t>());
+    if ((rc = device_exscan<0, unsigned long long>(pl, d_len2.as<uint32_t>(), n, d_rowptr))) return rc;
+    hipLaunchKernelGGL(k_fin_gather, dim3(nb_), dim3(256), 0, 0, n, d_start.as<unsigned long long>(), d_nb.as<uint32_t>(), d_rowptr, d_cols,
+                       d_rec.as<unsigned long long>(), d_best, d_best_out);
+    ISO_HIP_CHECK(hipGetLastError());
+    return ISOCON_OK;
+}
 
 struct NNContext {
     isocon_store *st = nullptr;
@@ -75,7 +129,7 @@
     DevBuf d_text2;
     uint32_t text2_stride = 0;
     bool text2_ready = false;
-    bool ensure_text2()
+    bool ensure_text2(hipStream_t stream = 0)
     {
         if (text2_ready) return true;
         text2_stride = nnf_text2_stride(st->maxlen);
@@ -84,7 +138,7 @@
         d_text2.pool = &st->pool;
         d_text2.slot = SLOT_NN_TEXT2;
         if (d_text2.alloc((size_t)std::max<uint32_t>(n, 1) * text2_stride * 4) != ISOCON_OK) return false;
-        hipLaunchKernelGGL(k_build_text2, dim3(std::max<uint32_t>(n, 1)), dim3(256), 0, 0, st->dev, d_text2.as<uint32_t>(), text2_stride);
+        hipLaunchKernelGGL(k_build_text2, dim3(std::max<uint32_t>(n, 1)), dim3(256), 0, stream, st->dev, d_text2.as<uint32_t>(), text2_stride);
         if (hipGetLastError() != hipSuccess) return false;
         text2_ready = true;
         return true;
@@ -100,6 +154,10 @@
     unsigned long long lb_total = 0;
     bool seeds_ready = false;
     uint32_t seed_nq = 0;
+    DevBuf d_seed_n;
+    bool lists_follow = false;
+    bool seed_lists_filled = false;
+    bool ltot_zeroed = false;
     int run_bound_seeds(const QMap &Q);
     DevBuf d_ltot, d_lchunks, d_list, d_lpa, d_lpb, d_lmeta, d_ltasks;
     struct ListPlan {
@@ -146,6 +204,33 @@
         ISO_HIP_CHECK(copy_h2d(d_best.p, best.data(), (size_t)n * 4));
         return ISOCON_OK;
     }
+    bool roles_pending = false;
+    bool rec_zeroed = false, fin_zeroed = false;
+    int begin_pass()
+    {
+        int rc;
+        if (fill_best && roles_pending && n) {
+            uint32_t *cnt = nullptr, *cur = nullptr;
+            unsigned long long *rec = nullptr, *fin_rec = nullptr;
+            DevBuf d_cnt(&st->pool, SLOT_NN_FIN_CNT), d_cur(&st->pool, SLOT_NN_FIN_CUR), d_rec(&st->pool, SLOT_NN_RECORD), d_frec(&st->pool, SLOT_NN_FIN_FLAG);
+            if (csr_follows && !d_cnt.alloc((size_t)n * 4) && !d_cur.alloc((size_t)n * 4) && !d_rec.alloc((2 + N_COUNTERS) * 8) && !d_frec.alloc(16)) {
+                cnt = d_cnt.as<uint32_t>(); cur = d_cur.as<uint32_t>();
+                rec = d_rec.as<unsigned long long>(); fin_rec = d_frec.as<unsigned long long>();
+            }
+            hipLaunchKernelGGL(k_nn_step_reset, dim3((n + 255) / 256), dim3(256), 0, 0, n, d_best.as<int32_t>(), d_qf.as<uint8_t>(), d_tf.as<uint8_t>(),
+                               d_hit_count.as<unsigned long long>(), d_stats.as<unsigned long long>(), N_COUNTERS, cnt, cur, rec, fin_rec);
+            ISO_HIP_CHECK(hipGetLastError());
+            fill_best = roles_pending = false;
+            rec_zeroed = fin_zeroed = cnt != nullptr;
+            return ISOCON_OK;
+        }
+        if (roles_pending) {
+            roles_pending = false;
+            if ((rc = upload_flags(true))) return rc;
+        }
+        if ((rc = upload_best()) || (rc = reset_counters())) return rc;
+        return ISOCON_OK;
+    }
     int download_best() { ISO_HIP_CHECK(copy_d2h(best.data(), d_best.p, (size_t)n * 4)); best_on_host = true; return ISOCON_OK; }
     static constexpr uint32_t N_COUNTERS = 2 * (NN_COUNTER_SLOTS * 4 + 1);
     int reset_counters()
@@ -206,25 +291,57 @@
     }
     bool csr_follows = false;
     bool wide_needed = false;
+    CsrJob csr;
     int collect_record(uint64_t *needed)
     {
         DevBuf d_rec(&st->pool, SLOT_NN_RECORD);
         int rc;
         if ((rc = d_rec.alloc((2 + N_COUNTERS) * 8))) return rc;
-        ISO_HIP_CHECK(hipMemsetAsync(d_rec.p, 0, 16, 0));
+        if (!rec_zeroed) ISO_HIP_CHECK(hipMemsetAsync(d_rec.p, 0, 16, 0));
+        rec_zeroed = false;
         hipLaunchKernelGGL(k_nn_step_record, dim3(std::max<uint32_t>(1, (n + 255) / 256)), dim3(256), 0, 0, d_hit_count.as<unsigned long long>(), d_stats.as<unsigned long long>(),
                            N_COUNTERS, d_best.as<int32_t>(), d_qf.as<uint8_t>(), st->dev.lens, n, d_rec.as<unsigned long long>());
         ISO_HIP_CHECK(hipGetLastError());
         unsigned long long rec[2 + N_COUNTERS];
-        ISO_HIP_CHECK(memcpy_wait(rec, d_rec.p, sizeof(rec), hipMemcpyDeviceToHost));
+        csr.drop();
+        const size_t rec_bytes = (sizeof(rec) + 15) & ~(size_t)15;
+        const size_t rp_bytes = (((size_t)n + 1) * 8 + 15) & ~(size_t)15, best_bytes = ((size_t)n * 4 + 15) & ~(size_t)15;
+        const size_t pin_bytes = CsrJob::PIN_FIXED + rp_bytes + best_bytes + rec_bytes;
+        char *pin = nullptr;
+        hipEvent_t ev_step = nullptr;
+        if (!variant("nn_serial_prep") && pin_bytes <= kStageBytes) {
+            if (g_csr_stage.cap < pin_bytes && g_csr_stage_busy) { ISO_HIP_CHECK(device_wait()); g_csr_stage_busy = false; }
+            pin = static_cast<char *>(g_csr_stage.get(std::max<size_t>(pin_bytes, (size_t)1 << 20)));
+            if (pin) { ev_step = g_events.get(); csr.ev_rec = g_events.get(); }
+            if (!ev_step || !csr.ev_rec) { g_events.put(ev_step); ev_step = nullptr; csr.drop(); pin = nullptr; }
+        }
+        if (pin) {
+            char *pin_step = pin + CsrJob::PIN_FIXED + rp_bytes + best_bytes;
+            g_csr_stage_busy = true;
+            ISO_HIP_CHECK(hipMemcpyAsync(pin_step, d_rec.p, sizeof(rec), hipMemcpyDeviceToHost, 0));
+            ISO_HIP_CHECK(hipEventRecord(ev_step, 0));
+            if (csr_enqueue(&st->pool, n, d_best.as<int32_t>(), true, d_hits.as<int32_t>(), d_hit_count.as<unsigned long long>(), hits_cap, fin_zeroed, csr) == ISOCON_OK &&
+                hipMemcpyAsync(pin + CsrJob::PIN_REC, csr.d_rec, 16, hipMemcpyDeviceToHost, 0) == hipSuccess && hipEventRecord(csr.ev_rec, 0) == hipSuccess &&
+                hipMemcpyAsync(pin + CsrJob::PIN_FIXED, csr.d_out, csr.cols_off, hipMemcpyDeviceToHost, 0) == hipSuccess) {
+                csr.live = true;
+                csr.pin = pin;
+            } else { (void)hipGetLastError(); csr.drop(); }
+            fin_zeroed = false;
+            ++g_host_waits;
+            const hipError_t e = hipEventSynchronize(ev_step);
+            g_events.put(ev_step);
+            ISO_HIP_CHECK(e);
+            memcpy(rec, pin_step, sizeof(rec));
+        } else ISO_HIP_CHECK(memcpy_wait(rec, d_rec.p, sizeof(rec), hipMemcpyDeviceToHost));
         add_counters(rec + 2);
         if (needed) *needed = rec[0];
-        if (rec[0] > hits_cap) return ISOCON_E_CAPACITY;
+        if (rec[0] > hits_cap) { csr.drop(); return ISOCON_E_CAPACITY; }
         stats.hits += rec[0];
         wide_needed = rec[1] != 0;
         dev_hits = d_hits.as<int32_t>();
         dev_hit_count = rec[0];
         best_on_host = false;
+        if (wide_needed || !dev_hit_count) csr.drop();
         return ISOCON_OK;
     }
     int pull_dev_hits()
@@ -321,7 +438,7 @@
 }
 
 int nn_setup(NNContext &C, isocon_store *s, const uint8_t *is_converged, const uint8_t *is_target, uint64_t depth,
-             const int32_t *best_in, bool depth_walk = false)
+             const int32_t *best_in, bool depth_walk = false, bool defer_roles = false)
 {
     C.st = s;
     C.n = s->dev.n;
@@ -362,7 +479,8 @@
         (rc = C.d_stats.alloc(2 * (NN_COUNTER_SLOTS * 4 + 1) * 8)))
         return rc;
     clk.lap("setup: pool");
-    if ((rc = C.upload_flags(true))) return rc;
+    if (defer_roles && n && C.roles_uniform && !s->n_exc && !variant("nn_serial_prep")) C.roles_pending = true;
+    else if ((rc = C.upload_flags(true))) return rc;
     clk.lap("setup: role flags");
     return ISOCON_OK;
 }
diff --git a/isocon_amd/csrc/nn_entry.inc b/isocon_amd/csrc/nn_entry.inc
--- a/isocon_amd/csrc/nn_entry.inc
+++ b/isocon_amd/csrc/nn_entry.inc
@@ -20,36 +20,14 @@
 };
 
 int nn_finalize_device_core(ScratchPool *pl, uint32_t n, const int32_t *d_best, const int32_t *best_host, const int32_t *d_hits, uint64_t n_hits,
-                            int32_t *out_best, uint64_t *out_row_ptr, uint32_t *out_cols, uint64_t cols_cap, uint64_t *n_cols_needed)
-{
-    DevBuf d_cnt(pl, SLOT_NN_FIN_CNT), d_start(pl, SLOT_NN_FIN_START), d_cur(pl, SLOT_NN_FIN_CUR), d_nb(pl, SLOT_NN_FIN_NB),
-        d_len2(pl, SLOT_NN_FIN_LEN2), d_out(pl, SLOT_NN_FIN_OUT), d_rec(pl, SLOT_NN_FIN_FLAG);
-    static_assert(sizeof(unsigned long long) == sizeof(uint64_t), "row pointers travel as they are");
-    const size_t rp_bytes = (((size_t)n + 1) * 8 + 15) & ~(size_t)15, best_bytes = best_host ? 0 : ((size_t)n * 4 + 15) & ~(size_t)15;
-    const size_t cols_off = rp_bytes + best_bytes;
+                            int32_t *out_best, uint64_t *out_row_ptr, uint32_t *out_cols, uint64_t cols_cap, uint64_t *n_cols_needed, bool zeroed = false)
+{
+    CsrJob J;
     int rc;
-    if ((rc = d_cnt.alloc((size_t)n * 4)) || (rc = d_start.alloc(((size_t)n + 1) * 8)) || (rc = d_cur.alloc((size_t)n * 4)) ||
-        (rc = d_nb.alloc((size_t)n_hits * 4 + 16)) || (rc = d_len2.alloc((size_t)n * 4)) || (rc = d_out.alloc(cols_off + (size_t)n_hits * 4 + 16)) ||
-        (rc = d_rec.alloc(16)))
-        return rc;
-    unsigned long long *d_rowptr = d_out.as<unsigned long long>();
-    int32_t *d_best_out = best_host ? nullptr : reinterpret_cast<int32_t *>(d_out.as<char>() + rp_bytes);
-    uint32_t *d_cols = reinterpret_cast<uint32_t *>(d_out.as<char>() + cols_off);
-    ISO_HIP_CHECK(hipMemsetAsync(d_cnt.p, 0, (size_t)n * 4, 0));
-    ISO_HIP_CHECK(hipMemsetAsync(d_cur.p, 0, (size_t)n * 4, 0));
-    ISO_HIP_CHECK(hipMemsetAsync(d_rec.p, 0, 16, 0));
-    const unsigned hb = (unsigned)std::max<uint64_t>(1, (n_hits + 255) / 256), nb_ = (n + 255) / 256;
-    hipLaunchKernelGGL(k_fin_count, dim3(hb), dim3(256), 0, 0, d_hits, (unsigned long long)n_hits, d_best, n, d_cnt.as<uint32_t>());
-    if ((rc = device_exscan<0, unsigned long long>(pl, d_cnt.as<uint32_t>(), n, d_start.as<unsigned long long>()))) return rc;
-    hipLaunchKernelGGL(k_fin_scatter, dim3(hb), dim3(256), 0, 0, d_hits, (unsigned long long)n_hits, d_best, n,
-                       d_start.as<unsigned long long>(), d_cur.as<uint32_t>(), d_nb.as<uint32_t>());
-    hipLaunchKernelGGL(k_fin_rows, dim3(nb_), dim3(256), 0, 0, n, d_start.as<unsigned long long>(), d_nb.as<uint32_t>(), d_len2.as<uint32_t>(), d_rec.as<uint32_t>());
-    if ((rc = device_exscan<0, unsigned long long>(pl, d_len2.as<uint32_t>(), n, d_rowptr))) return rc;
-    hipLaunchKernelGGL(k_fin_gather, dim3(nb_), dim3(256), 0, 0, n, d_start.as<unsigned long long>(), d_nb.as<uint32_t>(), d_rowptr, d_cols);
-    hipLaunchKernelGGL(k_fin_pack, dim3(std::max(1u, nb_)), dim3(256), 0, 0, n, d_rowptr, d_rec.as<unsigned long long>(), d_best, d_best_out);
-    ISO_HIP_CHECK(hipGetLastError());
+    if ((rc = csr_enqueue(pl, n, d_best, best_host == nullptr, d_hits, nullptr, n_hits, zeroed, J))) return rc;
+    const size_t rp_bytes = J.rp_bytes, cols_off = J.cols_off;
     unsigned long long rec[2] = {0, 0};
-    ISO_HIP_CHECK(memcpy_wait(rec, d_rec.p, sizeof(rec), hipMemcpyDeviceToHost));
+    ISO_HIP_CHECK(memcpy_wait(rec, J.d_rec, sizeof(rec), hipMemcpyDeviceToHost));
     if (rec[0]) return ISOCON_E_UNSUPPORTED;
     const uint64_t total = rec[1];
     if (n_cols_needed) *n_cols_needed = total;
@@ -59,19 +37,41 @@
     const int32_t *best_src = best_host;
     std::vector<int32_t> best_tmp;
     if (stg) {
-        ISO_HIP_CHECK(memcpy_wait(stg, d_out.p, bytes, hipMemcpyDeviceToHost));
+        ISO_HIP_CHECK(memcpy_wait(stg, J.d_out, bytes, hipMemcpyDeviceToHost));
         memcpy(out_row_ptr, stg, ((size_t)n + 1) * 8);
         if (total) memcpy(out_cols, stg + cols_off, (size_t)total * 4);
         if (!best_src) best_src = reinterpret_cast<const int32_t *>(stg + rp_bytes);
     } else {
-        ISO_HIP_CHECK(copy_d2h(out_row_ptr, d_rowptr, ((size_t)n + 1) * 8));
-        if (total) ISO_HIP_CHECK(copy_d2h(out_cols, d_cols, (size_t)total * 4));
+        ISO_HIP_CHECK(copy_d2h(out_row_ptr, J.d_out, ((size_t)n + 1) * 8));
+        if (total) ISO_HIP_CHECK(copy_d2h(out_cols, J.d_out + cols_off, (size_t)total * 4));
         if (!best_src) {
             best_tmp.resize(std::max<uint32_t>(n, 1));
-            if (n) ISO_HIP_CHECK(copy_d2h(best_tmp.data(), d_best_out, (size_t)n * 4));
+            if (n) ISO_HIP_CHECK(copy_d2h(best_tmp.data(), J.d_out + rp_bytes, (size_t)n * 4));
             best_src = best_tmp.data();
         }
     }
+    for (uint32_t i = 0; i < n; ++i) out_best[i] = out_row_ptr[i + 1] > out_row_ptr[i] ? best_src[i] : -1;
+    return ISOCON_OK;
+}
+
+int csr_fetch(CsrJob &J, int32_t *out_best, uint64_t *out_row_ptr, uint32_t *out_cols, uint64_t cols_cap, uint64_t *n_cols_needed)
+{
+    const uint32_t n = J.n;
+    ++g_host_waits;
+    const hipError_t e = hipEventSynchronize(J.ev_rec);
+    J.drop();
+    ISO_HIP_CHECK(e);
+    unsigned long long rec[2];
+    memcpy(rec, J.pin + CsrJob::PIN_REC, sizeof(rec));
+    if (rec[0]) return ISOCON_E_UNSUPPORTED;
+    const uint64_t total = rec[1];
+    if (n_cols_needed) *n_cols_needed = total;
+    if (total > cols_cap) return ISOCON_E_CAPACITY;
+    if (total) ISO_HIP_CHECK(copy_d2h(out_cols, J.d_out + J.cols_off, (size_t)total * 4));
+    else { ++g_host_waits; ISO_HIP_CHECK(hipStreamSynchronize(0)); }
+    g_csr_stage_busy = false;
+    memcpy(out_row_ptr, J.pin + CsrJob::PIN_FIXED, ((size_t)n + 1) * 8);
+    const int32_t *best_src = reinterpret_cast<const int32_t *>(J.pin + CsrJob::PIN_FIXED + J.rp_bytes);
     for (uint32_t i = 0; i < n; ++i) out_best[i] = out_row_ptr[i + 1] > out_row_ptr[i] ? best_src[i] : -1;
     return ISOCON_OK;
 }
@@ -218,7 +218,7 @@
                    ~Total() { if (getenv("ISOCON_DEBUG")) fprintf(stderr, "[isocon] %-28s %8.2f ms\n", "isocon_nn_graph total", std::chrono::duration<double, std::milli>(std::chrono::steady_clock::now() - t).count()); } } total;
     WaitScope waits(s);
     NNContext C;
-    int rc = nn_setup(C, s, is_converged, is_target, depth, nullptr, true);
+    int rc = nn_setup(C, s, is_converged, is_target, depth, nullptr, true, true);
     if (rc) return rc;
     clk0.lap("setup");
     if (getenv("ISOCON_DEBUG")) { (void)hipDeviceSynchronize(); clk0.lap("sync after setup"); }
@@ -242,7 +242,9 @@
         if (C.hits.empty()) {
             C.stats.kernel_ms = C.tm.total; C.stats.narrow_kernel_ms = C.tm.marked_total;
             if (stats) *stats = C.stats;
-            rc = nn_finalize_device_core(&s->pool, n, C.d_best.as<int32_t>(), C.best_on_host ? C.best.data() : nullptr, C.dev_hits, C.dev_hit_count, out_best, out_row_ptr, out_cols, cols_cap, n_cols_needed);
+            if (C.csr.live && !C.best_on_host) rc = csr_fetch(C.csr, out_best, out_row_ptr, out_cols, cols_cap, n_cols_needed);
+            else rc = nn_finalize_device_core(&s->pool, n, C.d_best.as<int32_t>(), C.best_on_host ? C.best.data() : nullptr, C.dev_hits, C.dev_hit_count, out_best, out_row_ptr, out_cols, cols_cap, n_cols_needed, C.fin_zeroed);
+            C.fin_zeroed = false;
             clk.lap("finalize (device hits)");
             if (rc != ISOCON_E_UNSUPPORTED && rc != ISOCON_E_HIP) return rc;
         }
diff --git a/isocon_amd/csrc/nn_finalize.hpp b/isocon_amd/csrc/nn_finalize.hpp
--- a/isocon_amd/csrc/nn_finalize.hpp
+++ b/isocon_amd/csrc/nn_finalize.hpp
@@ -14,20 +14,34 @@
     return true;
 }
 
-__global__ __launch_bounds__(256) void k_fin_count(const int32_t *__restrict__ hits, unsigned long long n_hits, const int32_t *__restrict__ best, uint32_t n,
-                                                    uint32_t *__restrict__ cnt)
+static constexpr uint32_t NN_FIN_GRID = 2048;
+
+__device__ __forceinline__ unsigned long long nn_fin_rows_held(const unsigned long long *__restrict__ hit_count, unsigned long long n_hits)
 {
-    const unsigned long long h = (unsigned long long)blockIdx.x * 256u + threadIdx.x;
-    uint32_t e, o;
-    if (h < n_hits && nn_fin_valid(hits, h, best, n, e, o)) atomicAdd(cnt + e, 1u);
+    if (hit_count == nullptr) return n_hits;
+    const unsigned long long c = *hit_count;
+    return c < n_hits ? c : n_hits;
 }
 
-__global__ __launch_bounds__(256) void k_fin_scatter(const int32_t *__restrict__ hits, unsigned long long n_hits, const int32_t *__restrict__ best, uint32_t n,
-                                                      const unsigned long long *__restrict__ start, uint32_t *__restrict__ cursor, uint32_t *__restrict__ nb)
+__global__ __launch_bounds__(256) void k_fin_count(const int32_t *__restrict__ hits, const unsigned long long *__restrict__ hit_count, unsigned long long n_hits,
+                                                    const int32_t *__restrict__ best, uint32_t n, uint32_t *__restrict__ cnt)
 {
-    const unsigned long long h = (unsigned long long)blockIdx.x * 256u + threadIdx.x;
-    uint32_t e, o;
-    if (h < n_hits && nn_fin_valid(hits, h, best, n, e, o)) nb[start[e] + atomicAdd(cursor + e, 1u)] = o;
+    const unsigned long long rows = nn_fin_rows_held(hit_count, n_hits);
+    for (unsigned long long h = (unsigned long long)blockIdx.x * 256u + threadIdx.x; h < rows; h += (unsigned long long)gridDim.x * 256u) {
+        uint32_t e, o;
+        if (nn_fin_valid(hits, h, best, n, e, o)) atomicAdd(cnt + e, 1u);
+    }
+}
+
+__global__ __launch_bounds__(256) void k_fin_scatter(const int32_t *__restrict__ hits, const unsigned long long *__restrict__ hit_count, unsigned long long n_hits,
+                                                      const int32_t *__restrict__ best, uint32_t n, const unsigned long long *__restrict__ start,
+                                                      uint32_t *__restrict__ cursor, uint32_t *__restrict__ nb)
+{
+    const unsigned long long rows = nn_fin_rows_held(hit_count, n_hits);
+    for (unsigned long long h = (unsigned long long)blockIdx.x * 256u + threadIdx.x; h < rows; h += (unsigned long long)gridDim.x * 256u) {
+        uint32_t e, o;
+        if (nn_fin_valid(hits, h, best, n, e, o)) nb[start[e] + atomicAdd(cursor + e, 1u)] = o;
+    }
 }
 
 __global__ __launch_bounds__(256) void k_fin_rows(uint32_t n, const unsigned long long *__restrict__ start, uint32_t *__restrict__ nb, uint32_t *__restrict__ len2,
@@ -55,22 +69,38 @@
 }
 
 __global__ __launch_bounds__(256) void k_fin_gather(uint32_t n, const unsigned long long *__restrict__ start, const uint32_t *__restrict__ nb,
-                                                     const unsigned long long *__restrict__ row_ptr, uint32_t *__restrict__ cols)
+                                                     const unsigned long long *__restrict__ row_ptr, uint32_t *__restrict__ cols,
+                                                     unsigned long long *__restrict__ rec, const int32_t *__restrict__ best, int32_t *__restrict__ best_out)
 {
     const uint32_t i = blockIdx.x * 256u + threadIdx.x;
+    if (i == 0) rec[1] = row_ptr[n];
     if (i >= n) return;
+    if (best_out != nullptr) best_out[i] = best[i];
     const uint32_t len = (uint32_t)(row_ptr[i + 1] - row_ptr[i]);
     const uint32_t *src = nb + start[i];
     uint32_t *dst = cols + row_ptr[i];
     for (uint32_t a = 0; a < len; ++a) dst[a] = src[a];
 }
 
-__global__ __launch_bounds__(256) void k_fin_pack(uint32_t n, const unsigned long long *__restrict__ row_ptr, unsigned long long *__restrict__ rec,
-                                                   const int32_t *__restrict__ best, int32_t *__restrict__ best_out)
+__global__ __launch_bounds__(256) void k_nn_step_reset(uint32_t n, int32_t *__restrict__ best, uint8_t *__restrict__ qflag, uint8_t *__restrict__ tflag,
+                                                        unsigned long long *__restrict__ hit_count, unsigned long long *__restrict__ stats, uint32_t n_stats,
+                                                        uint32_t *__restrict__ fin_cnt, uint32_t *__restrict__ fin_cur, unsigned long long *__restrict__ step_rec,
+                                                        unsigned long long *__restrict__ fin_rec)
 {
     const uint32_t i = blockIdx.x * 256u + threadIdx.x;
-    if (i == 0) rec[1] = row_ptr[n];
-    if (best_out != nullptr && i < n) best_out[i] = best[i];
+    if (i < n) {
+        best[i] = NN_INF;
+        qflag[i] = 1;
+        tflag[i] = 1;
+        if (fin_cnt != nullptr) { fin_cnt[i] = 0; fin_cur[i] = 0; }
+    }
+    if (blockIdx.x == 0) {
+        if (threadIdx.x == 0) {
+            *hit_count = 0;
+            if (fin_cnt != nullptr) { step_rec[0] = step_rec[1] = 0; fin_rec[0] = fin_rec[1] = 0; }
+        }
+        for (uint32_t k = threadIdx.x; k < n_stats; k += 256u) stats[k] = 0;
+    }
 }
 
 __global__ __launch_bounds__(256) void k_nn_step_record(const unsigned long long *__restrict__ hit_count, const unsigned long long *__restrict__ stats, uint32_t n_stats,
diff --git a/isocon_amd/csrc/nn_lists.inc b/isocon_amd/csrc/nn_lists.inc
--- a/isocon_amd/csrc/nn_lists.inc
+++ b/isocon_amd/csrc/nn_lists.inc
@@ -4,6 +4,7 @@
 int NNContext::plan_lists(const QMap &Q, uint32_t nq, const NNParams &PR, ListPlan &L)
 {
     L = ListPlan();
+    if (g_side.open) ISO_HIP_CHECK(g_side.join());
     if (PR.lb == nullptr || nq == 0 || variant("nn_no_list") || st->pool.slots[SLOT_NN_LBT].p == nullptr || st->maxlen >= 16384) return ISOCON_OK;
     unsigned long long pairs_cap = std::min<unsigned long long>(lb_total, std::max<unsigned long long>(1ull << 22, lb_total / 8));
     if (const char *e = variant_value("nn_list_cap")) pairs_cap = std::max<unsigned long long>(1, strtoull(e, nullptr, 10));
@@ -29,7 +30,8 @@
     L.b = L.a + cap_out;
     L.sorted_a = L.b + cap_out;
     L.sorted_b = L.sorted_a + cap_out;
-    ISO_HIP_CHECK(hipMemsetAsync(d_ltot.p, 0, sizeof(NNPlanTotals), 0));
+    if (!ltot_zeroed) ISO_HIP_CHECK(hipMemsetAsync(d_ltot.p, 0, sizeof(NNPlanTotals), 0));
+    ltot_zeroed = false;
     NNBoundRows B;
     B.lb = PR.lb; B.row_off = PR.lb_row; B.row_len = static_cast<const uint32_t *>(st->pool.slots[SLOT_NN_LBLEN].p);
     B.lbT = static_cast<const uint8_t *>(st->pool.slots[SLOT_NN_LBT].p);
diff --git a/isocon_amd/csrc/nn_main.inc b/isocon_amd/csrc/nn_main.inc
--- a/isocon_amd/csrc/nn_main.inc
+++ b/isocon_amd/csrc/nn_main.inc
@@ -330,14 +330,17 @@
                               (size_t)std::count(C.tflag.begin(), C.tflag.end(), (uint8_t)1) > 512;
     const bool two_set_lists = two_set_many && !variant("nn_no_qgram");
     const bool whole_set = Q.begin == 0 && Q.end == n && Q.stride == 1 && Q.block_log2 == 0 && C.depth >= n;
+    SideJoinGuard join_guard;
     for (;;) {
         int rc;
-        if ((rc = C.upload_best()) || (rc = C.reset_counters())) return rc;
+        if ((rc = C.begin_pass())) return rc;
         clk.lap("phaseA: upload/reset");
         PhaseAPass P(do_seed, do_main, seeded_before);
+        C.lists_follow = false;
         if (!C.two_set || two_set_lists) {
             P.refill_main = !variant("nn_tiles") && fits;
             P.bounds_wanted = P.refill_main && !variant("nn_no_qgram");
+            C.lists_follow = do_main && P.bounds_wanted;
             P.PR = C.params(63);
             if (do_seed && (rc = phase_a_seeds(C, Q, P, clk))) return rc;
             if (allow_regroup && !P.refill_main && do_seed && do_main && whole_set && n > 128 && (rc = regroup_by_seed_hits(C, best0, P.G, clk))) return rc;
@@ -348,6 +351,7 @@
             if ((rc = phase_a_two_set_unbounded(C, Q))) return rc;
         } else if ((rc = phase_a_two_set_tiles(C, Q, do_main))) return rc;
         bool again = false;
+        if (g_side.open) ISO_HIP_CHECK(g_side.join());
         if ((rc = nn_end_pass(C, 63, P.no_markers, P.G, &clk, again))) return rc;
         if (!again) return ISOCON_OK;
     }
```
